# olga24912/lodestar

Measured on AMD Instinct MI355X. Metric: verified signature sets/sec (node), higher is better.
Workload: dtype u32/u64 (28-bit-limb Montgomery integer arithmetic); 1 GPU; C2 gossip attestation flood: 16384 single-pubkey sets per GPU, 1 set per batchable job; pk_mode=device table, sig_encoding=compressed 96 B, distinct_messages=16384, group_sets=1024, group_policy=0, inflight=32, slots=3, hw_queues=4, merge_sets=131072, pipeline_depth=3, parallelism=shard-by-job x1 (in-process devices), no collective

## Files before the change

lodestar_amd/build.py:

```python
import hashlib
import os
import subprocess
import sys
import time

PKG = os.path.dirname(os.path.abspath(__file__))
ROOT = os.path.dirname(PKG)
CSRC = os.path.join(PKG, "csrc")
LIB = os.environ.get("BLSGPU_LIB") or os.path.join(PKG, "libblsgpu.so")
ARCH = os.environ.get("BLSGPU_ARCH", "gfx950")
HIPCC = os.environ.get("HIPCC", "/opt/rocm/bin/hipcc")
SOURCES = ["k_sig.hip", "k_msm.hip", "k_hash.hip", "k_hmap.hip", "k_pk.hip", "k_sigagg.hip", "k_awr.hip", "k_same.hip", "k_miller.hip", "k_group.hip", "k_inv.hip", "k_ssz.hip", "k_debug.hip",
           "runtime.cpp", "helpers.cpp"]


OBJ_DIR = os.path.join(PKG, "build")


TU_DEFINES = {"k_sig.hip": ["BLS_INLINE_BIG=1"]}


def tu_defines():
    env = os.environ.get("BLSGPU_TU_DEFINES")
    if env is None:
        return TU_DEFINES
    out = {}
    for part in filter(None, env.split(";")):
        tu, _, defs = part.partition("=")
        out[tu] = [d for d in defs.split("+") if d]
    return out


_ILP = ["-mllvm", "-amdgpu-sched-strategy=max-ilp"]
_MINREG = ["-mllvm", "-amdgpu-sched-strategy=iterative-minreg"]
TU_CFLAGS = {"k_hash.hip": _MINREG, "k_pk.hip": _ILP}


def tu_cflags():
    env = os.environ.get("BLSGPU_TU_CFLAGS")
    if env is None:
        return TU_CFLAGS
    out = {}
    for part in filter(None, env.split(";")):
        tu, _, flags = part.partition("=")
        out[tu] = flags.split()
    return out


def _headers():
    out = [os.path.join(ROOT, "include", "blsgpu.h")]
    for f in os.listdir(CSRC):
        if f.endswith((".hpp", ".h")):
            out.append(os.path.join(CSRC, f))
    return out


def _tu_deps(src):
    if src.endswith(".cpp"):
        return [os.path.join(CSRC, f) for f in (src, "kernels.h", "batch_rand.hpp", "runtime_internal.hpp",
                                                "helper_layout.hpp")] + [os.path.join(ROOT, "include", "blsgpu.h")]
    return [os.path.join(CSRC, src)] + _headers()


def _deps():
    return _headers() + [os.path.join(CSRC, s) for s in SOURCES] + [os.path.abspath(__file__)]


def up_to_date():
    if not os.path.exists(LIB):
        return False
    t = os.path.getmtime(LIB)
    return all(os.path.getmtime(d) <= t for d in _deps())


def build(force=False, verbose=True):
    if not force and up_to_date():
        build_node_addon(verbose=verbose)
        return LIB
    objs = []
    common = ["-O3", "-std=c++17", "-fPIC", f"--offload-arch={ARCH}", "-I", os.path.join(ROOT, "include")]
    defines = os.environ.get("BLSGPU_DEFINES", "").split()
    common += ["-D" + d for d in defines]
    cflags = os.environ.get("BLSGPU_CFLAGS", "").split()
    common += cflags
    tu_defs = tu_defines()
    os.makedirs(OBJ_DIR, exist_ok=True)
    key = os.path.splitext(os.path.basename(LIB))[0] + ("." + "_".join(defines).replace("=", "-") if defines else "")
    if cflags:
        key += ".cf" + hashlib.md5(" ".join(cflags).encode()).hexdigest()[:8]
    procs = []
    t0 = time.time()
    for src in SOURCES:
        tdefs = tu_defs.get(src, [])
        tflags = tu_cflags().get(src, [])
        obj = os.path.join(OBJ_DIR, key + "." + os.path.splitext(src)[0] +
                           ("." + "_".join(tdefs).replace("=", "-") if tdefs else "") +
                           (".cf" + hashlib.md5(" ".join(tflags).encode()).hexdigest()[:8] if tflags else "") + ".o")
        objs.append(obj)
        if not force and os.path.exists(obj) and all(os.path.getmtime(d) <= os.path.getmtime(obj) for d in _tu_deps(src)):
            continue
        cmd = [HIPCC] + common + ["-D" + d for d in tdefs] + tflags + ["-c", os.path.join(CSRC, src), "-o", obj]
        if verbose:
            print(" ".join(cmd), flush=True)
        procs.append((src, subprocess.Popen(cmd)))
    for src, p in procs:
        if p.wait() != 0:
            raise RuntimeError(f"hipcc failed on {src}")
        if verbose:
            print(f"  {src}: done at {time.time() - t0:.0f} s", flush=True)
    cmd = [HIPCC, f"--offload-arch={ARCH}", "-shared", "-o", LIB] + objs + ["-lpthread"]
    if verbose:
        print(" ".join(cmd), flush=True)
    subprocess.check_call(cmd)
    build_node_addon(verbose=verbose)
    return LIB


NODE_DIR = os.path.join(PKG, "node")
ADDON = os.path.join(NODE_DIR, "blsgpu_napi.node")
NODE_INC = "/usr/include/node"


def build_node_addon(force=False, verbose=True):
    src = os.path.join(NODE_DIR, "blsgpu_napi.c")
    if not os.path.exists(os.path.join(NODE_INC, "node_api.h")):
        if verbose:
            print("node headers not found: N-API addon not built", flush=True)
        return None
    if not force and os.path.exists(ADDON) and os.path.getmtime(ADDON) >= max(
            os.path.getmtime(src), os.path.getmtime(LIB), os.path.getmtime(os.path.join(ROOT, "include", "blsgpu.h"))):
        return ADDON
    cmd = ["gcc", "-O2", "-std=c11", "-Wall", "-Wno-unused-parameter", "-shared", "-fPIC",
           "-DNODE_GYP_MODULE_NAME=blsgpu_napi", "-I", NODE_INC, "-I", os.path.join(ROOT, "include"), src,
           "-o", ADDON, "-L", PKG, "-l:libblsgpu.so", "-Wl,-rpath,$ORIGIN/.."]
    if verbose:
        print(" ".join(cmd), flush=True)
    subprocess.check_call(cmd)
    return ADDON


if __name__ == "__main__":
    build(force="--force" in sys.argv)
```

lodestar_amd/csrc/k_group.hip:

```cpp
#include "k_common.hpp"
#include "gt_wave.hpp"
#include "gt6.hpp"

__global__ __launch_bounds__(WAVE) void k_job_mask(PipelineBuffers b) {
  uint32_t j = blockIdx.x * WAVE + threadIdx.x;
  if (j >= b.n_jobs) return;
  const uint32_t a = b.job_first_set[j], e = b.job_first_set[j + 1];
  const int8_t* pk_st = b.status + b.n;
  int err = 0;
  for (uint32_t i = a; i < e && !err; i++) err = pk_st[i];
  for (uint32_t i = a; i < e && !err; i++) err = b.status[i];
  if (a == e) err = BLS_EMPTY_SET;
  b.job_err[j] = (int8_t)err;
  for (uint32_t i = a; i < e; i++) b.include[i] = err == 0 ? 1 : 0;
}

__global__ __launch_bounds__(WAVE) void k_group_reduce(PipelineBuffers b, const uint32_t* f_ranges, uint32_t ng,
                                                       uint32_t* F_out) {
  __shared__ uint32_t red[WAVE * W_FP12];
  const uint32_t g = blockIdx.x, lane = threadIdx.x;
  if (g >= ng) return;
  const uint32_t first = f_ranges[2 * g], last = f_ranges[2 * g + 1];
  fp12 F = fp12_one();
  bool any = false;
  for (uint32_t i = first + lane; i < last; i += WAVE) {
    F = any ? fp12_mul(F, ld_fp12(b.f_chunk, b.n, i)) : ld_fp12(b.f_chunk, b.n, i);
    any = true;
  }
#pragma unroll 1
  for (int s = WAVE / 2; s >= 1; s >>= 1) {
    if (lane >= (uint32_t)s && lane < (uint32_t)(2 * s)) st_fp12(red, WAVE, lane - s, F);
    __syncthreads();
    if (lane < (uint32_t)s) F = fp12_mul(F, ld_fp12(red, WAVE, lane));
    __syncthreads();
  }
  if (lane == 0) st_fp12(F_out, ng, g, F);
}

STAGE_KERNEL_W(BLSGPU_WPE_GRP) void k_f_runs(PipelineBuffers b, const uint32_t* runs, uint32_t n_runs) {
  const uint32_t q = blockIdx.x * WAVE + threadIdx.x;
  if (q >= n_runs) return;
  const uint32_t a = runs[2 * q], e = runs[2 * q + 1];
  fp12 F = ld_fp12(b.f_chunk, b.n, a);
#pragma unroll 1
  for (uint32_t i = a + 1; i < e; i++) F = fp12_mul(F, ld_fp12(b.f_chunk, b.n, i));
  st_fp12(b.f_chunk, b.n, a, F);
}

__global__ __launch_bounds__(GTW_LANES) void k_f_pairs(PipelineBuffers b, const uint32_t* pairs) {
  __shared__ uint32_t A[GTW_FP12], B[GTW_FP12], S[108 * BLS_NL];
  const uint32_t t = threadIdx.x, i = pairs[2 * blockIdx.x], j = pairs[2 * blockIdx.x + 1];
  for (uint32_t w = t; w < W_FP12; w += GTW_LANES) {
    A[gtw_lds_word(w)] = b.f_chunk[(size_t)w * b.n + i];
    B[gtw_lds_word(w)] = b.f_chunk[(size_t)w * b.n + j];
  }
  gtw_sync();
  gtw_mul<false>(A, A, B, S, t);
  for (uint32_t w = t; w < W_FP12; w += GTW_LANES) b.f_chunk[(size_t)w * b.n + i] = A[gtw_lds_word(w)];
}

STAGE_KERNEL void k_f_gather(PipelineBuffers b, const uint32_t* f_ranges, uint32_t ng, uint32_t* F_out) {
  const uint32_t q = blockIdx.x * WAVE + threadIdx.x;
  if (q >= ng * W_FP12) return;
  const uint32_t g = q % ng, w = q / ng, a = f_ranges[2 * g], e = f_ranges[2 * g + 1];
  F_out[q] = a < e ? b.f_chunk[(size_t)w * b.n + a] : (w < BLS_NL ? FP_ONE.l[w] : 0u);
}

__device__ __forceinline__ void gtw_load_S(GtwLds& sh, const uint32_t* S_in, uint32_t ng, uint32_t g, uint32_t t) {
  if (t == 0) {
    g2a Sa;
    const bool fin = jac_to_aff(ld_g2j(S_in, ng, g), Sa);
    if (fin) {
      lds_st(sh.QA, 0, Sa.x.c0);
      lds_st(sh.QA, 1, Sa.x.c1);
      lds_st(sh.QA, 2, Sa.y.c0);
      lds_st(sh.QA, 3, Sa.y.c1);
    }
    sh.flag = fin ? 1u : 0u;
  }
}

__global__ __launch_bounds__(GTW_MILLER_LANES) void k_group_sig_miller(const uint32_t* S_in, uint32_t ng, uint32_t* G_out) {
  __shared__ GtwLds sh;
  const uint32_t g = blockIdx.x, t = threadIdx.x;
  gtw_load_S(sh, S_in, ng, g, t);
  gtw_sync();
  if (sh.flag)
    gtw_miller_loop(sh.G, sh.QA, G1_GEN_X, G1_NEG_GEN_Y, sh.TB, sh.L, sh.L1, sh.S, sh.S2, t);
  else
    gtw_set_one(sh.G, t);
  gtw_sync();
  for (uint32_t w = t; w < W_FP12; w += GTW_MILLER_LANES) G_out[(size_t)w * ng + g] = sh.G[gtw_lds_word(w)];
}

STAGE_KERNEL_W(BLSGPU_WPE_GRP) void k_group_sig_miller_lane(const uint32_t* S_in, uint32_t ng, uint32_t* G_out) {
  const uint32_t g = blockIdx.x * WAVE + threadIdx.x;
  if (g >= ng) return;
  g2a Sa;
  g1a P;
  P.x = G1_GEN_X;
  P.y = G1_NEG_GEN_Y;
  const fp12 G = jac_to_aff(ld_g2j(S_in, ng, g), Sa) ? miller_loop(P, Sa) : fp12_one();
  st_fp12(G_out, ng, g, G);
}

STAGE_KERNEL_W(BLSGPU_WPE_LINES) void k_check_lines(const uint32_t* S_in, uint32_t ng, const uint32_t* sel, uint32_t n,
                                                   uint32_t* lines, uint8_t* flags) {
  const uint32_t q = blockIdx.x * WAVE + threadIdx.x;
  if (q >= n) return;
  const uint32_t g = sel ? sel[q] : q;
  g2a Sa;
  const bool fin = jac_to_aff(ld_g2j(S_in, ng, g), Sa);
  flags[g] = fin ? 0 : 1;
  if (fin) miller_lines_store(Sa, lines, ng, g);
}

STAGE_KERNEL_W(BLSGPU_WPE_GRP) void k_group_sig_miller_lane_sel(const uint32_t* S_in, uint32_t ng, const uint32_t* sel,
                                                               uint32_t n, uint32_t* G_out) {
  const uint32_t q = blockIdx.x * WAVE + threadIdx.x;
  if (q >= n) return;
  const uint32_t g = sel ? sel[q] : q;
  g2a Sa;
  g1a P;
  P.x = G1_GEN_X;
  P.y = G1_NEG_GEN_Y;
  const fp12 G = jac_to_aff(ld_g2j(S_in, ng, g), Sa) ? miller_loop(P, Sa) : fp12_one();
  st_fp12(G_out, ng, g, G);
}

template <bool MILLER>
__global__ __launch_bounds__(MILLER ? GTW_MILLER_LANES : GTW_LANES) void k_group_check(
    const uint32_t* S_in, const uint32_t* F_in, uint32_t ng, const uint32_t* G_in, const uint32_t* sel, uint8_t* ok) {
  constexpr uint32_t NT = MILLER ? GTW_MILLER_LANES : GTW_LANES;
  __shared__ GtwLds sh;
  const uint32_t t = threadIdx.x;
  const uint32_t g = sel ? sel[blockIdx.x] : blockIdx.x;
  for (uint32_t w = t; w < W_FP12; w += NT) {
    sh.F[gtw_lds_word(w)] = F_in[(size_t)w * ng + g];
    if (!MILLER) sh.G[gtw_lds_word(w)] = G_in[(size_t)w * ng + g];
  }
  if (MILLER) gtw_load_S(sh, S_in, ng, g, t);
  gtw_sync();
  if (!MILLER) {
    gtw_mul<false>(sh.F, sh.F, sh.G, sh.S, t);
  } else if (sh.flag) {
    gtw_miller_loop(sh.G, sh.QA, G1_GEN_X, G1_NEG_GEN_Y, sh.TB, sh.L, sh.L1, sh.S, sh.S2, t);
    gtw_mul<false>(sh.F, sh.F, sh.G, sh.S, t);
  }
  gtw_final_exp(sh.F, sh.W, sh.S, t);
  if (t == 0) ok[blockIdx.x] = fp12_is_one(gtw_to_reg(sh.F)) ? 1 : 0;
}

STAGE_KERNEL_W(BLSGPU_WPE_GRP) void k_group_check_lane(const uint32_t* S_in, const uint32_t* F_in, uint32_t ng,
                                                      const uint32_t* sel, uint32_t n, uint8_t* ok) {
  const uint32_t q = blockIdx.x * WAVE + threadIdx.x;
  if (q >= n) return;
  const uint32_t g = sel ? sel[q] : q;
  fp12 F = ld_fp12(F_in, ng, g);
  g2a Sa;
  if (jac_to_aff(ld_g2j(S_in, ng, g), Sa)) {
    g1a P;
    P.x = G1_GEN_X;
    P.y = G1_NEG_GEN_Y;
    F = fp12_mul(F, miller_loop(P, Sa));
  }
  ok[q] = fp12_is_one(final_exponentiation(F)) ? 1 : 0;
}

template <bool MILLER>
STAGE_KERNEL_W(BLSGPU_WPE_GRP) void k_group_check6(const uint32_t* F_in, const uint32_t* G_in, uint32_t ng,
                                                  const uint32_t* sel, uint32_t n, uint8_t* ok, const uint32_t* lines,
                                                  const uint8_t* flags) {
  const uint32_t lane = threadIdx.x, grp = lane / 6, k = lane % 6;
  const uint32_t q = blockIdx.x * ACC6_GROUPS + grp;
  if (grp >= ACC6_GROUPS || q >= n) return;
  const uint32_t gi = sel ? sel[q] : q;
  const G6 g{(int)(grp * 6), k};
  const int w0 = ((k & 1) ? 3 : 0) * 2 * W_FP + (int)(k >> 1) * 2 * W_FP;
  const fp2 F = ld_fp2(F_in, ng, gi, w0);
  fp2 G;
  if (MILLER)
    G = flags[gi] ? (k == 0 ? fp2_one() : fp2_zero()) : g6_miller(lines, ng, gi, G1_GEN_X, G1_NEG_GEN_Y, g);
  else
    G = ld_fp2(G_in, ng, gi, w0);
  const bool one = g6_is_one(g6_final_exp(g6_mul(F, G, g), g), g);
  if (k == 0) ok[q] = one ? 1 : 0;
}

__global__ __launch_bounds__(WAVE) void k_range_combine(const uint32_t* S_in, const uint32_t* F_in, uint32_t n_in,
                                                        const uint32_t* ranges, uint32_t n_out, uint32_t* S_out,
                                                        uint32_t* F_out) {
  __shared__ uint32_t red[WAVE * (W_G2J + W_FP12)];
  const uint32_t r = blockIdx.x, lane = threadIdx.x;
  if (r >= n_out) return;
  const uint32_t first = ranges[2 * r], last = ranges[2 * r + 1];
  g2j S = jac_infinity<fp2>();
  fp12 F = fp12_one();
  for (uint32_t e = first + lane; e < last; e += WAVE) {
    S = jac_add(S, ld_g2j(S_in, n_in, e));
    F = fp12_mul(F, ld_fp12(F_in, n_in, e));
  }
#pragma unroll 1
  for (int h = WAVE / 2; h >= 1; h >>= 1) {
    if (lane >= (uint32_t)h && lane < (uint32_t)(2 * h)) {
      st_g2j(red, WAVE, lane - h, S);
      st_fp12(red + WAVE * W_G2J, WAVE, lane - h, F);
    }
    __syncthreads();
    if (lane < (uint32_t)h) {
      S = jac_add(S, ld_g2j(red, WAVE, lane));
      F = fp12_mul(F, ld_fp12(red + WAVE * W_G2J, WAVE, lane));
    }
    __syncthreads();
  }
  if (lane == 0) {
    st_g2j(S_out, n_out, r, S);
    st_fp12(F_out, n_out, r, F);
  }
}


STAGE_KERNEL_W(BLSGPU_WPE_GRP) void k_group_reduce_lane(PipelineBuffers b, const uint32_t* set_ranges, const uint32_t* f_ranges,
                                      uint32_t ng, uint32_t* S_out, uint32_t* F_out) {
  const uint32_t g = blockIdx.x * WAVE + threadIdx.x;
  if (g >= ng) return;
  g2j S = jac_infinity<fp2>();
  for (uint32_t i = set_ranges[2 * g]; i < set_ranges[2 * g + 1]; i++)
    if (b.include[i]) S = jac_add(S, ld_g2j(b.rsig, b.n, i));
  fp12 F = fp12_one();
  for (uint32_t c = f_ranges[2 * g]; c < f_ranges[2 * g + 1]; c++) F = fp12_mul(F, ld_fp12(b.f_chunk, b.n, c));
  st_g2j(S_out, ng, g, S);
  st_fp12(F_out, ng, g, F);
}

STAGE_KERNEL_W(BLSGPU_WPE_GRP) void k_range_combine_lane(const uint32_t* S_in, const uint32_t* F_in, uint32_t n_in, const uint32_t* ranges,
                                       uint32_t n_out, uint32_t* S_out, uint32_t* F_out) {
  const uint32_t r = blockIdx.x * WAVE + threadIdx.x;
  if (r >= n_out) return;
  g2j S = jac_infinity<fp2>();
  fp12 F = fp12_one();
  for (uint32_t e = ranges[2 * r]; e < ranges[2 * r + 1]; e++) {
    S = jac_add(S, ld_g2j(S_in, n_in, e));
    F = fp12_mul(F, ld_fp12(F_in, n_in, e));
  }
  st_g2j(S_out, n_out, r, S);
  st_fp12(F_out, n_out, r, F);
}

static inline dim3 grid_for(uint32_t n) { return dim3((n + WAVE - 1) / WAVE); }

__global__ __launch_bounds__(256) void k_copy_words(uint32_t* __restrict__ dst, const uint32_t* __restrict__ src,
                                                    size_t n) {
  for (size_t i = (size_t)blockIdx.x * 256 + threadIdx.x; i < n; i += (size_t)gridDim.x * 256) dst[i] = src[i];
}
void launch_copy_words(uint32_t* dst, const uint32_t* src, size_t n, hipStream_t s) {
  if (n) hipLaunchKernelGGL(k_copy_words, dim3((unsigned)std::min<size_t>((n + 255) / 256, 8192)), dim3(256), 0, s, dst, src, n);
}

void launch_group_reduce_lane(const PipelineBuffers& b, const uint32_t* set_ranges, const uint32_t* f_ranges,
                              uint32_t ng, uint32_t* S, uint32_t* F, hipStream_t s) {
  if (ng) hipLaunchKernelGGL(k_group_reduce_lane, grid_for(ng), dim3(WAVE), 0, s, b, set_ranges, f_ranges, ng, S, F);
}
void launch_range_combine_lane(const uint32_t* S_in, const uint32_t* F_in, uint32_t n_in, const uint32_t* ranges,
                               uint32_t n_out, uint32_t* S_out, uint32_t* F_out, hipStream_t s) {
  if (n_out)
    hipLaunchKernelGGL(k_range_combine_lane, grid_for(n_out), dim3(WAVE), 0, s, S_in, F_in, n_in, ranges, n_out, S_out,
                       F_out);
}

void launch_job_mask(const PipelineBuffers& b, hipStream_t s) {
  if (b.n_jobs) hipLaunchKernelGGL(k_job_mask, grid_for(b.n_jobs), dim3(WAVE), 0, s, b);
}
void launch_group_reduce(const PipelineBuffers& b, const uint32_t* f_ranges, uint32_t ng, uint32_t* F, hipStream_t s) {
  if (ng) hipLaunchKernelGGL(k_group_reduce, dim3(ng), dim3(WAVE), 0, s, b, f_ranges, ng, F);
}
void launch_group_tree(const PipelineBuffers& b, const uint32_t* f_ranges, uint32_t ng, const uint32_t* runs,
                       uint32_t n_runs, const uint32_t* pairs, const std::vector<uint32_t>& level_end, uint32_t* F,
                       hipStream_t s) {
  if (!ng) return;
  if (n_runs) hipLaunchKernelGGL(k_f_runs, grid_for(n_runs), dim3(WAVE), 0, s, b, runs, n_runs);
  uint32_t p0 = 0;
  for (const uint32_t p1 : level_end) {
    if (p1 > p0) hipLaunchKernelGGL(k_f_pairs, dim3(p1 - p0), dim3(GTW_LANES), 0, s, b, pairs + 2 * (size_t)p0);
    p0 = p1;
  }
  hipLaunchKernelGGL(k_f_gather, grid_for(ng * W_FP12), dim3(WAVE), 0, s, b, f_ranges, ng, F);
}
void launch_group_sig_miller_sel(const uint32_t* S, uint32_t ng, const uint32_t* sel, uint32_t n_sel, uint32_t* G,
                                 hipStream_t s) {
  const uint32_t n = sel ? n_sel : ng;
  if (n) hipLaunchKernelGGL(k_group_sig_miller_lane_sel, grid_for(n), dim3(WAVE), 0, s, S, ng, sel, n, G);
}
void launch_group_check6(const uint32_t* F, const uint32_t* G, uint32_t ng, uint8_t* ok, hipStream_t s,
                         const uint32_t* sel, uint32_t n_sel) {
  const uint32_t n = sel ? n_sel : ng;
  if (n)
    hipLaunchKernelGGL(k_group_check6<false>, dim3((n + ACC6_GROUPS - 1) / ACC6_GROUPS), dim3(WAVE), 0, s, F, G, ng,
                       sel, n, ok, nullptr, nullptr);
}
void launch_check6_miller(const uint32_t* S, const uint32_t* F, uint32_t ng, uint8_t* ok, hipStream_t s,
                          const uint32_t* sel, uint32_t n_sel, uint32_t* lines, uint8_t* flags) {
  const uint32_t n = sel ? n_sel : ng;
  if (!n) return;
  hipLaunchKernelGGL(k_check_lines, grid_for(n), dim3(WAVE), 0, s, S, ng, sel, n, lines, flags);
  hipLaunchKernelGGL(k_group_check6<true>, dim3((n + ACC6_GROUPS - 1) / ACC6_GROUPS), dim3(WAVE), 0, s, F, nullptr, ng,
                     sel, n, ok, lines, flags);
}
void launch_group_check(const uint32_t* S, const uint32_t* F, uint32_t ng, uint8_t* ok, hipStream_t s,
                        const uint32_t* sel, uint32_t n_sel, const uint32_t* G, bool exclusive, bool lane) {
  const uint32_t n = sel ? n_sel : ng;
  if (!n) return;
  if (lane && !G)
    hipLaunchKernelGGL(k_group_check_lane, grid_for(n), dim3(WAVE), 0, s, S, F, ng, sel, n, ok);
  else if (G)
    hipLaunchKernelGGL(k_group_check<false>, dim3(n), dim3(GTW_LANES),
                       exclusive ? exclusive_cu_lds<k_group_check<false>>() : 0, s, S, F, ng, G, sel, ok);
  else
    hipLaunchKernelGGL(k_group_check<true>, dim3(n), dim3(GTW_MILLER_LANES),
                       exclusive ? exclusive_cu_lds<k_group_check<true>>() : 0, s, S, F, ng, G, sel, ok);
}
void launch_group_sig_miller(const uint32_t* S, uint32_t ng, uint32_t* G, hipStream_t s, bool exclusive, bool lane) {
  if (ng && lane)
    hipLaunchKernelGGL(k_group_sig_miller_lane, grid_for(ng), dim3(WAVE), 0, s, S, ng, G);
  else if (ng)
    hipLaunchKernelGGL(k_group_sig_miller, dim3(ng), dim3(GTW_MILLER_LANES),
                       exclusive ? exclusive_cu_lds<k_group_sig_miller>() : 0,
                       s, S, ng, G);
}
void launch_range_combine(const uint32_t* S_in, const uint32_t* F_in, uint32_t n_in, const uint32_t* ranges,
                          uint32_t n_out, uint32_t* S_out, uint32_t* F_out, hipStream_t s) {
  if (n_out)
    hipLaunchKernelGGL(k_range_combine, dim3(n_out), dim3(WAVE), 0, s, S_in, F_in, n_in, ranges, n_out, S_out, F_out);
}
```

lodestar_amd/csrc/k_miller.hip:

```cpp
#include "k_common.hpp"
#include "gt_wave.hpp"
#include "gt6.hpp"
#include "gtx.hpp"

#ifndef BLS_LINE_PAIRS
#define BLS_LINE_PAIRS 0
#endif
#ifndef BLS_ACC2_PAIRS
#define BLS_ACC2_PAIRS 0
#endif

BLS_INL fp fp_add_n(const fp& a, const fp& b) { return fp_add_norm(a, b); }

#ifndef BLS_ACC_PREFETCH
#define BLS_ACC_PREFETCH 0
#endif
#if BLS_ACC_PREFETCH && defined(__HIP_DEVICE_COMPILE__)
#define LDS_AS __attribute__((address_space(3)))
__device__ __forceinline__ void line_prefetch(uint32_t* pre, const uint32_t* o, uint32_t nm, uint32_t m) {
  const uint32_t* a = o + opaque_u32(m);
#pragma unroll 1
  for (int w = 0; w < W_LINE; w++) {
    __builtin_amdgcn_global_load_lds((const void*)a, (LDS_AS void*)(pre + w * WAVE), 4, 0, 0);
    a += nm;
  }
}
__device__ __forceinline__ void line_wait() {
  asm volatile("" ::: "memory");
  __builtin_amdgcn_s_waitcnt(0x0F70);
  asm volatile("" ::: "memory");
}
__device__ __forceinline__ void line_read_done() {
  asm volatile("" ::: "memory");
  __builtin_amdgcn_s_waitcnt(0xC07F);
  asm volatile("" ::: "memory");
}
__device__ __forceinline__ fp ld_fp_pre(const uint32_t* pre, int w0) {
  fp r;
#pragma unroll
  for (int l = 0; l < BLS_NL; l++) r.l[l] = pre[(w0 + l) * WAVE + threadIdx.x];
  return r;
}
__device__ __forceinline__ fp2 ld_fp2_pre(const uint32_t* pre, int w0) {
  return fp2_make(ld_fp_pre(pre, w0), ld_fp_pre(pre, w0 + W_FP));
}
#define ACC_PREFETCH 1
#else
#define ACC_PREFETCH 0
#endif

STAGE_KERNEL_W(BLSGPU_WPE_LINES) void k_miller_lines(PipelineBuffers b) {
  uint32_t u = blockIdx.x * WAVE + threadIdx.x;
  if (u >= b.n_umsg || (b.mflags[u] & MF_H_INF)) return;
  miller_lines_store(ld_g2a(b.h_aff, b.nm, u), b.lines, b.nm, u);
}

#ifndef BLSGPU_WPE_LINES2
#define BLSGPU_WPE_LINES2 2
#endif
STAGE_KERNEL_W(BLSGPU_WPE_LINES2) void k_miller_lines2(PipelineBuffers b) {
  const uint32_t q = blockIdx.x * WAVE + threadIdx.x;
  const uint32_t u = q >> 1, k = q & 1;
  if (u >= b.n_umsg || (b.mflags[u] & MF_H_INF)) return;
  auto ldQ = [&] {
    const uint32_t uu = opaque_u32(u);
    aff<fp2x> Q;
    Q.x.v = ld_fp(b.h_aff, b.nm, uu, (int)(k * W_FP));
    Q.y.v = ld_fp(b.h_aff, b.nm, uu, (int)((2 + k) * W_FP));
    return Q;
  };
  g2projx Tp;
  {
    const aff<fp2x> Q = ldQ();
    Tp.x = Q.x;
    Tp.y = Q.y;
    Tp.z = F_one((const fp2x*)0);
  }
  int bit = 62;
  bool add_next = false;
#pragma unroll 1
  for (int s = 0; s < MILLER_STEPS; s++) {
    line3x Ln;
    if (!add_next) {
      miller_dbl_line(Tp, Ln);
      add_next = (BLS_Z_ABS >> bit) & 1ull;
      bit--;
    } else {
      miller_add_line(Tp, ldQ(), Ln);
      add_next = false;
    }
    uint32_t* o = b.lines + (size_t)s * W_LINE * b.nm;
    st_fp(o, b.nm, u, (int)(k * W_FP), Ln.l0.v);
    st_fp(o, b.nm, u, (int)((2 + k) * W_FP), Ln.c1.v);
    st_fp(o, b.nm, u, (int)((4 + k) * W_FP), Ln.c4.v);
  }
}

template <bool UNITS>
STAGE_KERNEL_W(BLSGPU_WPE_ACC) void k_miller_acc(PipelineBuffers b) {
  const uint32_t c = blockIdx.x * WAVE + threadIdx.x;
  if (c >= b.n_chunks) return;
  const uint32_t k0 = b.chunk_first[c], k1 = b.chunk_first[c + 1];
#if ACC_PREFETCH
  __shared__ uint32_t pre[W_LINE * WAVE];
  auto msg_of = [&](uint32_t k) {
    const uint32_t i = b.chunk_items[k];
    return UNITS ? b.unit_msg[i] : b.msg_idx[i];
  };
  if (k1 > k0) line_prefetch(pre, b.lines, b.nm, msg_of(k0));
#endif
  fp12 f = fp12_one();
  int bit = 62;
  bool add_next = false;
#pragma unroll 1
  for (int s = 0; s < MILLER_STEPS; s++) {
    if (!add_next && s != 0) f = fp12_sqr(f);
    const uint32_t* o = b.lines + (size_t)s * W_LINE * b.nm;
#if BLS_LINE_PAIRS
    bool pend = false;
    fp2 q0, q1, q4;
#endif
#pragma unroll 1
    for (uint32_t k = k0; k < k1; k++) {
      const uint32_t i = b.chunk_items[k];
      uint32_t m;
      bool active;
      if (UNITS) {
        m = b.unit_msg[i];
        active = b.unit_ok[i] != 0;
      } else {
        m = b.msg_idx[i];
        active = b.include[i] != 0;
      }
#if ACC_PREFETCH
      line_wait();
      line3 L;
      L.l0 = ld_fp2_pre(pre, 0);
      L.c1 = ld_fp2_pre(pre, 2 * W_FP);
      L.c4 = ld_fp2_pre(pre, 4 * W_FP);
      line_read_done();
      if (k + 1 < k1)
        line_prefetch(pre, o, b.nm, msg_of(k + 1));
      else if (s + 1 < MILLER_STEPS)
        line_prefetch(pre, o + (size_t)W_LINE * b.nm, b.nm, msg_of(k0));
      if (!active || (b.mflags[m] & MF_H_INF)) continue;
      const g1a P = ld_g1a(UNITS ? b.unit_p : b.pk_aff, b.n, i);
#else
      if (!active || (b.mflags[m] & MF_H_INF)) continue;
      const g1a P = ld_g1a(UNITS ? b.unit_p : b.pk_aff, b.n, i);
      line3 L;
      L.l0 = ld_fp2(o, b.nm, m, 0);
      L.c1 = ld_fp2(o, b.nm, m, 2 * W_FP);
      L.c4 = ld_fp2(o, b.nm, m, 4 * W_FP);
#endif
#if BLS_LINE_PAIRS
      const fp2 l1 = fp2_mul_fp(L.c1, P.x), l4 = fp2_mul_fp(L.c4, P.y);
      if (pend) {
        f = fp12_mul_by_line2(f, line_pair(q0, q1, q4, L.l0, l1, l4));
        pend = false;
      } else {
        q0 = L.l0;
        q1 = l1;
        q4 = l4;
        pend = true;
      }
#else
      f = fp12_mul_by_014(f, L.l0, fp2_mul_fp(L.c1, P.x), fp2_mul_fp(L.c4, P.y));
#endif
    }
#if BLS_LINE_PAIRS
    if (pend) f = fp12_mul_by_014(f, q0, q1, q4);
#endif
    if (!add_next) {
      add_next = (BLS_Z_ABS >> bit) & 1ull;
      bit--;
    } else {
      add_next = false;
    }
  }
  st_fp12(b.f_chunk, b.n, c, fp12_conj(f));
}

template <bool UNITS>
STAGE_KERNEL_W(BLSGPU_WPE_ACC) void k_miller_acc2(PipelineBuffers b) {
  const uint32_t q = blockIdx.x * WAVE + threadIdx.x;
  const uint32_t c = q >> 1, h = q & 1;
  if (c >= b.n_chunks) return;
  const uint32_t k0 = b.chunk_first[c], k1 = b.chunk_first[c + 1];
#if ACC_PREFETCH
  __shared__ uint32_t pre[W_LINE * WAVE];
  auto msg_of = [&](uint32_t k) {
    const uint32_t i = b.chunk_items[k];
    return UNITS ? b.unit_msg[i] : b.msg_idx[i];
  };
  if (k1 > k0) line_prefetch(pre, b.lines, b.nm, msg_of(k0));
#endif
  fp6 mine = h ? fp6_zero() : fp6_one();
  int bit = 62;
  bool add_next = false;
#pragma unroll 1
  for (int s = 0; s < MILLER_STEPS; s++) {
    if (!add_next && s != 0) {
      const fp6 other = fp6_xlane(mine);
      const fp6 a0 = h ? other : mine, a1 = h ? mine : other;
      fp6 X, Y;
      if (h) {
        X.c0 = fp2_make(fp_add_n(a0.c0.c0, a1.c0.c0), fp_add_n(a0.c0.c1, a1.c0.c1));
        X.c1 = fp2_make(fp_add_n(a0.c1.c0, a1.c1.c0), fp_add_n(a0.c1.c1, a1.c1.c1));
        X.c2 = fp2_make(fp_add_n(a0.c2.c0, a1.c2.c0), fp_add_n(a0.c2.c1, a1.c2.c1));
        Y.c0 = fp2_make(fp_lc(T<1>(a0.c0.c0), T<1>(a1.c2.c0), T<-1>(a1.c2.c1)),
                        fp_lc(T<1>(a0.c0.c1), T<1>(a1.c2.c0), T<1>(a1.c2.c1)));
        Y.c1 = fp2_make(fp_add_n(a0.c1.c0, a1.c0.c0), fp_add_n(a0.c1.c1, a1.c0.c1));
        Y.c2 = fp2_make(fp_add_n(a0.c2.c0, a1.c1.c0), fp_add_n(a0.c2.c1, a1.c1.c1));
      } else {
        X = a0;
        Y = a1;
      }
      const fp6 pr = fp6_mul(X, Y);
      const fp6 t = fp6_xlane(pr);
      fp6 r;
      if (h) {
        r.c0.c0 = fp_lc(T<1>(pr.c0.c0), T<-1>(t.c0.c0), T<-1>(t.c2.c0), T<1>(t.c2.c1));
        r.c0.c1 = fp_lc(T<1>(pr.c0.c1), T<-1>(t.c0.c1), T<-1>(t.c2.c0), T<-1>(t.c2.c1));
        r.c1.c0 = fp_lc(T<1>(pr.c1.c0), T<-1>(t.c1.c0), T<-1>(t.c0.c0));
        r.c1.c1 = fp_lc(T<1>(pr.c1.c1), T<-1>(t.c1.c1), T<-1>(t.c0.c1));
        r.c2.c0 = fp_lc(T<1>(pr.c2.c0), T<-1>(t.c2.c0), T<-1>(t.c1.c0));
        r.c2.c1 = fp_lc(T<1>(pr.c2.c1), T<-1>(t.c2.c1), T<-1>(t.c1.c1));
      } else {
        r.c0 = fp2_make(fp_lc(T<2>(pr.c0.c0)), fp_lc(T<2>(pr.c0.c1)));
        r.c1 = fp2_make(fp_lc(T<2>(pr.c1.c0)), fp_lc(T<2>(pr.c1.c1)));
        r.c2 = fp2_make(fp_lc(T<2>(pr.c2.c0)), fp_lc(T<2>(pr.c2.c1)));
      }
      mine = fp6_xlane(r);
    }
    const uint32_t* o = b.lines + (size_t)s * W_LINE * b.nm;
    auto fold = [&](const fp6& T0, const fp6& T1) {
      const fp6 T1v = h ? T1 : fp6_mul_v(T1);
      fp6 r;
      r.c0 = fp2_make(fp_lc(T<1>(T0.c0.c0), T<1>(T1v.c0.c0)), fp_lc(T<1>(T0.c0.c1), T<1>(T1v.c0.c1)));
      r.c1 = fp2_make(fp_lc(T<1>(T0.c1.c0), T<1>(T1v.c1.c0)), fp_lc(T<1>(T0.c1.c1), T<1>(T1v.c1.c1)));
      r.c2 = fp2_make(fp_lc(T<1>(T0.c2.c0), T<1>(T1v.c2.c0)), fp_lc(T<1>(T0.c2.c1), T<1>(T1v.c2.c1)));
      mine = r;
    };
#if BLS_ACC2_PAIRS
    bool pend = false;
    fp2 q0, q1, q4;
#endif
#pragma unroll 1
    for (uint32_t k = k0; k < k1; k++) {
      const uint32_t i = b.chunk_items[k];
      uint32_t m;
      bool active;
      if (UNITS) {
        m = b.unit_msg[i];
        active = b.unit_ok[i] != 0;
      } else {
        m = b.msg_idx[i];
        active = b.include[i] != 0;
      }
#if ACC_PREFETCH
      line_wait();
      fp2 l0 = ld_fp2_pre(pre, 0), l1 = ld_fp2_pre(pre, 2 * W_FP), l4 = ld_fp2_pre(pre, 4 * W_FP);
      line_read_done();
      if (k + 1 < k1)
        line_prefetch(pre, o, b.nm, msg_of(k + 1));
      else if (s + 1 < MILLER_STEPS)
        line_prefetch(pre, o + (size_t)W_LINE * b.nm, b.nm, msg_of(k0));
      if (!active || (b.mflags[m] & MF_H_INF)) continue;
      const g1a P = ld_g1a(UNITS ? b.unit_p : b.pk_aff, b.n, i);
      l1 = fp2_mul_fp(l1, P.x);
      l4 = fp2_mul_fp(l4, P.y);
#else
      if (!active || (b.mflags[m] & MF_H_INF)) continue;
      const g1a P = ld_g1a(UNITS ? b.unit_p : b.pk_aff, b.n, i);
      const fp2 l0 = ld_fp2(o, b.nm, m, 0);
      const fp2 l1 = fp2_mul_fp(ld_fp2(o, b.nm, m, 2 * W_FP), P.x);
      const fp2 l4 = fp2_mul_fp(ld_fp2(o, b.nm, m, 4 * W_FP), P.y);
#endif
#if BLS_ACC2_PAIRS
      if (!pend) {
        q0 = l0;
        q1 = l1;
        q4 = l4;
        pend = true;
        continue;
      }
      pend = false;
      const fp2 R1 = fp2_mul(h ? q4 : q0, h ? l4 : l0);
      const fp2 R2 = fp2_mul(h ? fp2_add_nr(q0, q4) : q1, h ? fp2_add_nr(l0, l4) : l1);
      const fp2 R3 = fp2_mul(h ? fp2_add_nr(q1, q4) : fp2_add_nr(q0, q1), h ? fp2_add_nr(l1, l4) : fp2_add_nr(l0, l1));
      const fp2 O1 = fp2_xlane(R1), O2 = fp2_xlane(R2), O3 = fp2_xlane(R3);
      const fp2 P00 = h ? O1 : R1, P44 = h ? R1 : O1, P11 = h ? O2 : R2, X04 = h ? R2 : O2, X01 = h ? O3 : R3,
                X14 = h ? R3 : O3;
      fp6 M0;
      M0.c0 = fp2_make(fp_lc(T<1>(P00.c0), T<1>(P44.c0), T<-1>(P44.c1)), fp_lc(T<1>(P00.c1), T<1>(P44.c0), T<1>(P44.c1)));
      M0.c1 = F2_LC3(X01, P00, P11);
      M0.c2 = P11;
      const fp2 m11 = F2_LC3(X04, P00, P44), m12 = F2_LC3(X14, P11, P44);
      const fp6 other = fp6_xlane(mine);
      fold(fp6_mul(mine, M0), fp6_mul_by_12(other, m11, m12));
#else
      const fp6 other = fp6_xlane(mine);
      fold(fp6_mul_by_01(mine, l0, l1), fp6_mul_by_1(other, l4));
#endif
    }
#if BLS_ACC2_PAIRS
    if (pend) {
      const fp6 other = fp6_xlane(mine);
      fold(fp6_mul_by_01(mine, q0, q1), fp6_mul_by_1(other, q4));
    }
#endif
    if (!add_next) {
      add_next = (BLS_Z_ABS >> bit) & 1ull;
      bit--;
    } else {
      add_next = false;
    }
  }
  const fp6 out = h ? fp6_neg(mine) : mine;
  st_fp2(b.f_chunk, b.n, c, 6 * (int)h * W_FP, out.c0);
  st_fp2(b.f_chunk, b.n, c, (6 * (int)h + 2) * W_FP, out.c1);
  st_fp2(b.f_chunk, b.n, c, (6 * (int)h + 4) * W_FP, out.c2);
}

#ifndef BLSGPU_WPE_ACCX
#define BLSGPU_WPE_ACCX 2
#endif
template <bool UNITS>
STAGE_KERNEL_W(BLSGPU_WPE_ACCX) void k_miller_accx(PipelineBuffers b) {
  const uint32_t q = blockIdx.x * WAVE + threadIdx.x;
  const uint32_t c = q >> 1, k = q & 1;
  if (c >= b.n_chunks) return;
  const uint32_t k0 = b.chunk_first[c], k1 = b.chunk_first[c + 1];
  fp12x f;
  f.c0.c0 = F_one((const fp2x*)0);
  f.c0.c1 = f.c0.c2 = f.c1.c0 = f.c1.c1 = f.c1.c2 = F_zero((const fp2x*)0);
  int bit = 62;
  bool add_next = false;
#pragma unroll 1
  for (int s = 0; s < MILLER_STEPS; s++) {
    if (!add_next && s != 0) f = fp12x_sqr(f);
    const uint32_t* o = b.lines + (size_t)s * W_LINE * b.nm;
#pragma unroll 1
    for (uint32_t it = k0; it < k1; it++) {
      const uint32_t i = b.chunk_items[it];
      uint32_t m;
      bool active;
      if (UNITS) {
        m = b.unit_msg[i];
        active = b.unit_ok[i] != 0;
      } else {
        m = b.msg_idx[i];
        active = b.include[i] != 0;
      }
      if (!active || (b.mflags[m] & MF_H_INF)) continue;
      const g1a P = ld_g1a(UNITS ? b.unit_p : b.pk_aff, b.n, i);
      const fp2x l0{ld_fp(o, b.nm, m, (int)(k * W_FP))};
      const fp2x l1{fp_mul(ld_fp(o, b.nm, m, (int)((2 + k) * W_FP)), P.x)};
      const fp2x l4{fp_mul(ld_fp(o, b.nm, m, (int)((4 + k) * W_FP)), P.y)};
      f = fp12x_mul_by_014(f, l0, l1, l4);
    }
    if (!add_next) {
      add_next = (BLS_Z_ABS >> bit) & 1ull;
      bit--;
    } else {
      add_next = false;
    }
  }
  st_fp(b.f_chunk, b.n, c, (int)((0 + k) * W_FP), f.c0.c0.v);
  st_fp(b.f_chunk, b.n, c, (int)((2 + k) * W_FP), f.c0.c1.v);
  st_fp(b.f_chunk, b.n, c, (int)((4 + k) * W_FP), f.c0.c2.v);
  st_fp(b.f_chunk, b.n, c, (int)((6 + k) * W_FP), fp_neg(f.c1.c0.v));
  st_fp(b.f_chunk, b.n, c, (int)((8 + k) * W_FP), fp_neg(f.c1.c1.v));
  st_fp(b.f_chunk, b.n, c, (int)((10 + k) * W_FP), fp_neg(f.c1.c2.v));
}

template <bool UNITS, int WPE>
__global__ __launch_bounds__(WAVE) __attribute__((amdgpu_waves_per_eu(WPE, WPE))) void k_miller_acc6(PipelineBuffers b) {
  const uint32_t lane = threadIdx.x, grp = lane / 6, k = lane % 6;
  const uint32_t c = blockIdx.x * ACC6_GROUPS + grp;
  if (grp >= ACC6_GROUPS || c >= b.n_chunks) return;
  const int base = (int)(grp * 6);
  const uint32_t k0 = b.chunk_first[c], k1 = b.chunk_first[c + 1];
  fp2 f = k == 0 ? fp2_one() : fp2_zero();
  int bit = 62;
  bool add_next = false;
#pragma unroll 1
  for (int s = 0; s < MILLER_STEPS; s++) {
    if (!add_next && s != 0) {
      f = g6_sqr(f, G6{base, k});
    }
    const uint32_t* o = b.lines + (size_t)s * W_LINE * b.nm;
#pragma unroll 1
    for (uint32_t it = k0; it < k1; it++) {
      const uint32_t i = b.chunk_items[it];
      uint32_t m;
      bool active;
      if (UNITS) {
        m = b.unit_msg[i];
        active = b.unit_ok[i] != 0;
      } else {
        m = b.msg_idx[i];
        active = b.include[i] != 0;
      }
      if (!active || (b.mflags[m] & MF_H_INF)) continue;
      const g1a Pa = ld_g1a(UNITS ? b.unit_p : b.pk_aff, b.n, i);
      f = g6_line_mul(f, o, b.nm, m, Pa.x, Pa.y, G6{base, k});
    }
    if (!add_next) {
      add_next = (BLS_Z_ABS >> bit) & 1ull;
      bit--;
    } else {
      add_next = false;
    }
  }
  const int slot = (k & 1 ? 3 : 0) + (int)(k >> 1);
  st_fp2(b.f_chunk, b.n, c, slot * 2 * W_FP, (k & 1) ? fp2_neg(f) : f);
}

template <bool UNITS>
__global__ __launch_bounds__(GTW_MILLER_LANES) void k_miller_coop(PipelineBuffers b) {
  __shared__ GtwLds sh;
  const uint32_t c = blockIdx.x, t = threadIdx.x;
  if (c >= b.n_chunks) return;
  const uint32_t i = b.chunk_items[b.chunk_first[c]];
  uint32_t m;
  bool active;
  if (UNITS) {
    m = b.unit_msg[i];
    active = b.unit_ok[i] != 0;
  } else {
    m = b.msg_idx[i];
    active = b.include[i] != 0;
  }
  active = active && !(b.mflags[m] & MF_H_INF);
  if (active) {
    if (t < 4) lds_st(sh.QA, (int)t, ld_fp(b.h_aff, b.nm, m, (int)t * W_FP));
    const g1a P = ld_g1a(UNITS ? b.unit_p : b.pk_aff, b.n, i);
    gtw_sync();
    gtw_miller_loop(sh.G, sh.QA, P.x, P.y, sh.TB, sh.L, sh.L1, sh.S, sh.S2, t);
  } else {
    gtw_set_one(sh.G, t);
  }
  gtw_sync();
  for (uint32_t w = t; w < W_FP12; w += GTW_MILLER_LANES) b.f_chunk[(size_t)w * b.n + c] = sh.G[gtw_lds_word(w)];
}

static inline dim3 grid_for(uint32_t n) { return dim3((n + WAVE - 1) / WAVE); }

void launch_miller_coop(const PipelineBuffers& b, bool units, hipStream_t s, bool exclusive) {
  if (!b.n_chunks) return;
  if (units)
    hipLaunchKernelGGL(k_miller_coop<true>, dim3(b.n_chunks), dim3(GTW_MILLER_LANES),
                       exclusive ? exclusive_cu_lds<k_miller_coop<true>>() : 0, s, b);
  else
    hipLaunchKernelGGL(k_miller_coop<false>, dim3(b.n_chunks), dim3(GTW_MILLER_LANES),
                       exclusive ? exclusive_cu_lds<k_miller_coop<false>>() : 0, s, b);
}

void launch_miller_lines(const PipelineBuffers& b, hipStream_t s) {
  if (b.n_umsg) hipLaunchKernelGGL(k_miller_lines, grid_for(b.n_umsg), dim3(WAVE), 0, s, b);
}
void launch_miller_lines2(const PipelineBuffers& b, hipStream_t s) {
  if (b.n_umsg) hipLaunchKernelGGL(k_miller_lines2, grid_for(2 * b.n_umsg), dim3(WAVE), 0, s, b);
}
void launch_miller_acc2(const PipelineBuffers& b, bool units, hipStream_t s) {
  if (!b.n_chunks) return;
  if (units)
    hipLaunchKernelGGL(k_miller_acc2<true>, grid_for(2 * b.n_chunks), dim3(WAVE), 0, s, b);
  else
    hipLaunchKernelGGL(k_miller_acc2<false>, grid_for(2 * b.n_chunks), dim3(WAVE), 0, s, b);
}
#define ACC6_W1_MAX_CHUNKS (1024 * ACC6_GROUPS)
void launch_miller_acc6(const PipelineBuffers& b, bool units, hipStream_t s) {
  if (!b.n_chunks) return;
  const dim3 grid((b.n_chunks + ACC6_GROUPS - 1) / ACC6_GROUPS);
  const bool w2 = b.n_chunks > ACC6_W1_MAX_CHUNKS;
  if (units && w2)
    hipLaunchKernelGGL((k_miller_acc6<true, 2>), grid, dim3(WAVE), 0, s, b);
  else if (units)
    hipLaunchKernelGGL((k_miller_acc6<true, 1>), grid, dim3(WAVE), 0, s, b);
  else if (w2)
    hipLaunchKernelGGL((k_miller_acc6<false, 2>), grid, dim3(WAVE), 0, s, b);
  else
    hipLaunchKernelGGL((k_miller_acc6<false, 1>), grid, dim3(WAVE), 0, s, b);
}
void launch_miller_accx(const PipelineBuffers& b, bool units, hipStream_t s) {
  if (!b.n_chunks) return;
  if (units)
    hipLaunchKernelGGL(k_miller_accx<true>, grid_for(2 * b.n_chunks), dim3(WAVE), 0, s, b);
  else
    hipLaunchKernelGGL(k_miller_accx<false>, grid_for(2 * b.n_chunks), dim3(WAVE), 0, s, b);
}
void launch_miller_acc(const PipelineBuffers& b, bool units, hipStream_t s) {
  if (!b.n_chunks) return;
  if (units)
    hipLaunchKernelGGL(k_miller_acc<true>, grid_for(b.n_chunks), dim3(WAVE), 0, s, b);
  else
    hipLaunchKernelGGL(k_miller_acc<false>, grid_for(b.n_chunks), dim3(WAVE), 0, s, b);
}
```

lodestar_amd/csrc/kernels.h:

```cpp
#pragma once
#include <hip/hip_runtime.h>
#include <stdint.h>
#include <vector>

#define W_FP 14
#define W_G1A (2 * W_FP)
#define W_G1J (3 * W_FP)
#define W_G2A (4 * W_FP)
#define W_G2J (6 * W_FP)
#define W_FP12 (12 * W_FP)
#define W_PKTAB 32
#define MILLER_STEPS 68
#define W_LINE (3 * 2 * W_FP)

#define SF_SIG_INF 1u
#define MF_H_INF 1u

struct PipelineBuffers {
  uint32_t n;
  const uint8_t* sigs;
  const uint32_t* sig_len;
  uint32_t sig_stride;
  const uint8_t* pk_bytes;
  const uint32_t* set_pk_first;
  const uint32_t* pk_index;
  const uint32_t* pk_table;
  uint32_t pk_table_n;
  const uint32_t* agg_sets;
  uint32_t n_agg;
  uint32_t pk_direct1;
  const uint64_t* scalars;
  uint32_t* scal_tab;
  const uint32_t* job_first_set;
  uint32_t n_jobs;
  const uint8_t* umsgs;
  const uint32_t* msg_idx;
  uint32_t n_umsg;
  uint32_t nm;
  uint32_t n_units;
  const uint32_t* unit_set_first;
  const uint32_t* unit_sets;
  const uint32_t* unit_msg;
  uint32_t* sig_aff;
  uint32_t* h_aff;
  uint32_t* h_jac;
  uint32_t* h_norm;
  uint32_t* h_prep;
  uint32_t* h_q;
  uint32_t* inv_buf;
  uint32_t* inv_buf_pk;
  uint32_t* pk_jac;
  uint32_t* pk_aff;
  uint32_t* rsig;
  uint32_t* unit_p;
  uint32_t n_chunks;
  const uint32_t* chunk_first;
  const uint32_t* chunk_items;
  uint32_t* f_chunk;
  uint32_t* lines;
  uint8_t* flags;
  uint8_t* mflags;
  uint8_t* unit_ok;
  int8_t* status;
  int8_t* job_err;
  uint8_t* include;
};

void launch_sig_decode(const PipelineBuffers& b, uint32_t n_sets, hipStream_t s, bool coop = false,
                       hipEvent_t decoded = nullptr, bool exclusive = true, bool subgroup = true);
void launch_spec_mask(const PipelineBuffers& b, uint32_t n_sets, uint8_t* spec, hipStream_t s);
void launch_hash_prep(const PipelineBuffers& b, hipStream_t s);
void launch_hash_map(const PipelineBuffers& b, const uint32_t* inv, hipStream_t s);
void launch_hash_to_g2(const PipelineBuffers& b, hipStream_t s, bool coop = false,
                       bool exclusive = true);
void launch_pk_aggregate(const PipelineBuffers& b, uint32_t n_sets, hipStream_t s);
void launch_pk_finish(const PipelineBuffers& b, uint32_t n_sets, hipStream_t s);
void launch_batch_inv(const uint32_t* src, uint32_t src_stride, int w0, uint32_t* dst, uint32_t n, hipStream_t s);
void launch_pk_affine(const PipelineBuffers& b, uint32_t n_sets, hipStream_t s);
void launch_h_affine(const PipelineBuffers& b, hipStream_t s);
void launch_sig_scale(const PipelineBuffers& b, uint32_t n_sets, hipStream_t s, const uint32_t* list = nullptr);
#ifndef MSM_SLICE
#define MSM_SLICE 256
#endif
#define MSM_BUCKET_WORDS (128 * W_G2J)
#define MSM_WINDOW_WORDS (16 * W_G2J)
void launch_sig_msm(const PipelineBuffers& b, const uint32_t* slices, uint32_t n_slices, const uint32_t* range_slices,
                    uint32_t n_ranges, uint32_t* B, uint32_t* W, uint32_t* S, hipStream_t s, bool lane_tail = false,
                    uint32_t tree_slices = 0);
void launch_job_mask(const PipelineBuffers& b, hipStream_t s);
void launch_unit_aggregate(const PipelineBuffers& b, hipStream_t s);
void launch_miller_lines(const PipelineBuffers& b, hipStream_t s);
void launch_miller_lines2(const PipelineBuffers& b, hipStream_t s);
void launch_miller_accx(const PipelineBuffers& b, bool units, hipStream_t s);
void launch_miller_acc(const PipelineBuffers& b, bool units, hipStream_t s);
void launch_miller_acc2(const PipelineBuffers& b, bool units, hipStream_t s);
void launch_miller_acc6(const PipelineBuffers& b, bool units, hipStream_t s);
#ifndef BLSGPU_EXCLUSIVE_SMALL
#define BLSGPU_EXCLUSIVE_SMALL 1
#endif
void launch_miller_coop(const PipelineBuffers& b, bool units, hipStream_t s, bool exclusive = false);
void launch_group_reduce(const PipelineBuffers& b, const uint32_t* f_ranges, uint32_t n_groups, uint32_t* F,
                         hipStream_t s);
void launch_group_tree(const PipelineBuffers& b, const uint32_t* f_ranges, uint32_t n_groups, const uint32_t* runs,
                       uint32_t n_runs, const uint32_t* pairs, const std::vector<uint32_t>& level_end, uint32_t* F,
                       hipStream_t s);
void launch_group_check(const uint32_t* S, const uint32_t* F, uint32_t n_groups, uint8_t* ok, hipStream_t s,
                        const uint32_t* sel = nullptr, uint32_t n_sel = 0, const uint32_t* G = nullptr,
                        bool exclusive = false, bool lane = false);
void launch_group_check6(const uint32_t* F, const uint32_t* G, uint32_t n_groups, uint8_t* ok, hipStream_t s,
                         const uint32_t* sel = nullptr, uint32_t n_sel = 0);
void launch_check6_miller(const uint32_t* S, const uint32_t* F, uint32_t n_groups, uint8_t* ok, hipStream_t s,
                          const uint32_t* sel, uint32_t n_sel, uint32_t* lines, uint8_t* flags);
void launch_group_sig_miller_sel(const uint32_t* S, uint32_t n_groups, const uint32_t* sel, uint32_t n_sel, uint32_t* G,
                                 hipStream_t s);
void launch_group_sig_miller(const uint32_t* S, uint32_t n_groups, uint32_t* G, hipStream_t s, bool exclusive = false,
                             bool lane = false);
void launch_copy_words(uint32_t* dst, const uint32_t* src, size_t n, hipStream_t s);
void launch_group_reduce_lane(const PipelineBuffers& b, const uint32_t* set_ranges, const uint32_t* f_ranges,
                              uint32_t n_groups, uint32_t* S, uint32_t* F, hipStream_t s);
void launch_range_combine_lane(const uint32_t* S_in, const uint32_t* F_in, uint32_t n_in, const uint32_t* ranges,
                               uint32_t n_out, uint32_t* S_out, uint32_t* F_out, hipStream_t s);
void launch_range_combine(const uint32_t* S_in, const uint32_t* F_in, uint32_t n_in, const uint32_t* ranges,
                          uint32_t n_out, uint32_t* S_out, uint32_t* F_out, hipStream_t s);
void launch_pk_table_fill(const uint8_t* pk96, uint32_t n, uint32_t* table_dst, int8_t* status, hipStream_t s);
void launch_pk_serialize(const PipelineBuffers& b, uint32_t n_sets, uint8_t* out, uint32_t out_len, hipStream_t s);
void launch_key_validate(const uint8_t* pks, uint32_t n, uint32_t pk_len, uint32_t stride, uint8_t* out96,
                         int8_t* status, hipStream_t s);
inline uint32_t sig_agg_lanes(uint32_t n_groups, uint32_t n_sigs) {
  if (n_groups == 0) return 1;
  const uint64_t n = n_groups, lanes = 1024 * 64;
  const uint32_t by_count = n * 64 <= lanes ? 64 : n * 32 <= 2 * lanes ? 32 : n * 16 <= 2 * lanes ? 16
                            : n * 8 <= 2 * lanes ? 8 : 1;
  const uint64_t mean = ((uint64_t)n_sigs + n - 1) / n;
  const uint32_t by_size = mean <= 3 ? 1 : mean <= 8 ? 8 : mean <= 16 ? 16 : mean <= 32 ? 32 : 64;
  return by_count < by_size ? by_count : by_size;
}
void launch_sig_aggregate(const PipelineBuffers& b, const uint32_t* group_first, uint32_t n_groups, uint32_t n_sigs,
                          uint32_t* agg, int8_t* agg_status, uint32_t* first_bad, hipStream_t s);
void launch_sig_agg_serialize(const uint32_t* group_first, uint32_t n_groups, const uint32_t* agg, int8_t* agg_status,
                              uint8_t* out, uint32_t out_len, hipStream_t s);
struct AwrBuffers {
  uint32_t n;
  uint32_t n_groups;
  const uint32_t* group_first;
  const uint64_t* words;
  const uint8_t* pk_bytes;
  const uint32_t* pk_index;
  const uint32_t* pk_table;
  uint32_t pk_table_n;
  const uint32_t* sig_aff;
  const uint8_t* sig_flags;
  const int8_t* sig_status;
  uint32_t* tab;
  uint32_t tab_n;
  uint32_t* sum_pk;
  uint32_t* sum_sig;
  uint32_t* err_k;
  int8_t* err_c;
};
#define AWR_TAB_WORDS (9 * W_G2J)
inline uint32_t awr_lanes(uint32_t n_groups, uint32_t n_sets) {
  if (n_groups == 0) return 1;
  const uint64_t n = n_groups, lanes = 1024 * 64;
  const uint32_t by_count = n * 64 <= lanes ? 64 : n * 32 <= lanes ? 32 : n * 16 <= lanes ? 16 : n * 8 <= lanes ? 8 : 1;
  const uint64_t mean = ((uint64_t)n_sets + n - 1) / n;
  const uint32_t by_size = mean <= 1 ? 1 : mean <= 8 ? 8 : mean <= 16 ? 16 : mean <= 32 ? 32 : 64;
  return by_count < by_size ? by_count : by_size;
}
uint32_t awr_launch_lanes(uint32_t n_groups, uint32_t L);
void launch_awr_sums(const AwrBuffers& a, uint32_t L, hipStream_t s);
void launch_awr_sum_pk(const AwrBuffers& a, uint32_t L, hipStream_t s);
void launch_awr_sum_sig(const AwrBuffers& a, uint32_t L, hipStream_t s);
void launch_same_group_items(const AwrBuffers& a, const uint32_t* inv, uint32_t* pk_aff, uint8_t* include, int8_t* code,
                             hipStream_t s);
void launch_same_retry_items(const AwrBuffers& a, const uint32_t* list, uint32_t n_retry, uint32_t* pk_aff, uint32_t* S,
                             uint8_t* include, int8_t* code, hipStream_t s);
void launch_same_group_results(const uint32_t* group_first, uint32_t n_groups, uint32_t n_sets, const uint8_t* include,
                               const int8_t* code, const uint8_t* ok, int8_t* set_result, int8_t* group_result,
                               hipStream_t s);
void launch_same_retry_results(const uint32_t* list, uint32_t n_retry, const uint8_t* include, const int8_t* code,
                               const uint8_t* ok, int8_t* set_result, hipStream_t s);
void launch_awr_serialize(const AwrBuffers& a, uint8_t* out_pk, uint32_t out_pk_len, uint8_t* out_sig,
                          uint32_t out_sig_len, int8_t* status, uint32_t* first_bad, hipStream_t s);
void launch_signing_roots(int kind, const uint8_t* in, uint32_t n, uint32_t in_stride, const uint8_t* domain,
                          uint32_t domain_stride, uint8_t* out, hipStream_t s);
void launch_debug_op(int op, uint32_t n, const uint8_t* in, uint32_t in_stride, uint8_t* out, uint32_t out_stride,
                     int32_t* status, hipStream_t s);
```

lodestar_amd/csrc/pairing.hpp:

```cpp
#pragma once
#include "curve.hpp"

struct g2proj {
  fp2 x, y, z;
};

BLS_FN void miller_dbl_step(g2proj& T, const fp& xP, const fp& yP, fp2& l0, fp2& l1, fp2& l4) {
  fp2 A = fp2_half(fp2_mul(T.x, T.y));
  fp2 B = fp2_sqr(T.y);
  fp2 C = fp2_sqr(T.z);
  fp2 E = fp2_mul3(fp2_mul_xi(C));
  E = fp2_dbl(fp2_dbl(E));
  fp2 F = fp2_mul3(E);
  fp2 G = fp2_half(fp2_add(B, F));
  fp2 H = fp2_sub(fp2_sub(fp2_sqr(fp2_add(T.y, T.z)), B), C);
  fp2 J = fp2_sqr(T.x);
  fp2 E2 = fp2_sqr(E);
  T.x = fp2_mul(A, fp2_sub(B, F));
  T.y = fp2_sub(fp2_sqr(G), fp2_mul3(E2));
  T.z = fp2_mul(B, H);
  l0 = fp2_sub(E, B);
  l1 = fp2_mul_fp(fp2_mul3(J), xP);
  l4 = fp2_mul_fp(fp2_neg(H), yP);
}

BLS_FN void miller_add_step(g2proj& T, const g2a& Q, const fp& xP, const fp& yP, fp2& l0, fp2& l1, fp2& l4) {
  fp2 theta = fp2_sub(T.y, fp2_mul(Q.y, T.z));
  fp2 lam = fp2_sub(T.x, fp2_mul(Q.x, T.z));
  fp2 C = fp2_sqr(theta);
  fp2 D = fp2_sqr(lam);
  fp2 E = fp2_mul(lam, D);
  fp2 F = fp2_mul(T.z, C);
  fp2 G = fp2_mul(T.x, D);
  fp2 H = fp2_sub(fp2_add(E, F), fp2_dbl(G));
  fp2 X3 = fp2_mul(lam, H);
  fp2 Y3 = fp2_sub(fp2_mul(theta, fp2_sub(G, H)), fp2_mul(T.y, E));
  fp2 Z3 = fp2_mul(T.z, E);
  l0 = fp2_sub(fp2_mul(theta, Q.x), fp2_mul(lam, Q.y));
  l1 = fp2_mul_fp(fp2_neg(theta), xP);
  l4 = fp2_mul_fp(lam, yP);
  T.x = X3;
  T.y = Y3;
  T.z = Z3;
}

#define MILLER_STEPS 68
struct line3 {
  fp2 l0, c1, c4;
};
BLS_HD bool miller_step_is_add(int s) {
  int bit = 62;
  bool add_next = false;
  for (int k = 0; k < s; k++) {
    if (!add_next) {
      add_next = (BLS_Z_ABS >> bit) & 1ull;
      bit--;
    } else {
      add_next = false;
    }
  }
  return add_next;
}
#if BLS_LAZY_CURVE
BLS_FN void miller_dbl_line(g2proj& R, line3& Ln) {
  const fp2 A = fp2_half(fp2_mul(R.x, R.y));
  const fp2 B = fp2_sqr(R.y);
  const fp2 C = fp2_sqr(R.z);
  const fp2 xC = fp2_make(fp_lc(T<1>(C.c0), T<-1>(C.c1)), fp_lc(T<1>(C.c0), T<1>(C.c1)));
  const fp2 E = F_lc(L<12>(xC));
  const fp2 G = fp2_half(F_lc(L<1>(B), L<3>(E)));
  const fp2 H = F_lc(L<1>(fp2_sqr(fp2_add_norm(R.y, R.z))), L<-1>(B), L<-1>(C));
  const fp2 J = fp2_sqr(R.x);
  const fp2 E2 = fp2_sqr(E);
  R.x = fp2_mul(A, F_lc(L<1>(B), L<-3>(E)));
  R.y = F_lc(L<1>(fp2_sqr(G)), L<-3>(E2));
  R.z = fp2_mul(B, H);
  Ln.l0 = F_lc(L<1>(E), L<-1>(B));
  Ln.c1 = F_lc(L<3>(J));
  Ln.c4 = F_lc(L<-1>(H));
}
BLS_FN void miller_add_line(g2proj& R, const g2a& Q, line3& Ln) {
  const fp2 theta = F_lc(L<1>(R.y), L<-1>(fp2_mul(Q.y, R.z)));
  const fp2 lam = F_lc(L<1>(R.x), L<-1>(fp2_mul(Q.x, R.z)));
  const fp2 C = fp2_sqr(theta);
  const fp2 D = fp2_sqr(lam);
  const fp2 E = fp2_mul(lam, D);
  const fp2 F = fp2_mul(R.z, C);
  const fp2 G = fp2_mul(R.x, D);
  const fp2 H = F_lc(L<1>(E), L<1>(F), L<-2>(G));
  const fp2 X3 = fp2_mul(lam, H);
  const fp2 Y3 = F_lc(L<1>(fp2_mul(theta, F_lc(L<1>(G), L<-1>(H)))), L<-1>(fp2_mul(R.y, E)));
  const fp2 Z3 = fp2_mul(R.z, E);
  Ln.l0 = F_lc(L<1>(fp2_mul(theta, Q.x)), L<-1>(fp2_mul(lam, Q.y)));
  Ln.c1 = F_lc(L<-1>(theta));
  Ln.c4 = lam;
  R.x = X3;
  R.y = Y3;
  R.z = Z3;
}
#else
BLS_FN void miller_dbl_line(g2proj& T, line3& L) {
  fp2 A = fp2_half(fp2_mul(T.x, T.y));
  fp2 B = fp2_sqr(T.y);
  fp2 C = fp2_sqr(T.z);
  fp2 E = fp2_mul3(fp2_mul_xi(C));
  E = fp2_dbl(fp2_dbl(E));
  fp2 F = fp2_mul3(E);
  fp2 G = fp2_half(fp2_add(B, F));
  fp2 H = fp2_sub(fp2_sub(fp2_sqr(fp2_add(T.y, T.z)), B), C);
  fp2 J = fp2_sqr(T.x);
  fp2 E2 = fp2_sqr(E);
  T.x = fp2_mul(A, fp2_sub(B, F));
  T.y = fp2_sub(fp2_sqr(G), fp2_mul3(E2));
  T.z = fp2_mul(B, H);
  L.l0 = fp2_sub(E, B);
  L.c1 = fp2_mul3(J);
  L.c4 = fp2_neg(H);
}
BLS_FN void miller_add_line(g2proj& T, const g2a& Q, line3& L) {
  fp2 theta = fp2_sub(T.y, fp2_mul(Q.y, T.z));
  fp2 lam = fp2_sub(T.x, fp2_mul(Q.x, T.z));
  fp2 C = fp2_sqr(theta);
  fp2 D = fp2_sqr(lam);
  fp2 E = fp2_mul(lam, D);
  fp2 F = fp2_mul(T.z, C);
  fp2 G = fp2_mul(T.x, D);
  fp2 H = fp2_sub(fp2_add(E, F), fp2_dbl(G));
  fp2 X3 = fp2_mul(lam, H);
  fp2 Y3 = fp2_sub(fp2_mul(theta, fp2_sub(G, H)), fp2_mul(T.y, E));
  fp2 Z3 = fp2_mul(T.z, E);
  L.l0 = fp2_sub(fp2_mul(theta, Q.x), fp2_mul(lam, Q.y));
  L.c1 = fp2_neg(theta);
  L.c4 = lam;
  T.x = X3;
  T.y = Y3;
  T.z = Z3;
}
#endif
BLS_FN fp12 miller_acc_step(const fp12& f, int s, bool is_add, const line3& L, const fp& xP, const fp& yP) {
  fp12 g = (!is_add && s != 0) ? fp12_sqr(f) : f;
  return fp12_mul_by_014(g, L.l0, fp2_mul_fp(L.c1, xP), fp2_mul_fp(L.c4, yP));
}

BLS_HDNI fp12 miller_loop(const g1a& P, const g2a& Q) {
  g2proj T;
  T.x = Q.x;
  T.y = Q.y;
  T.z = fp2_one();
  fp12 f = fp12_one();
  int bit = 62;
  bool add_next = false;
#pragma unroll 1
  for (int s = 0; s < 68; s++) {
    fp2 l0, l1, l4;
    if (!add_next) {
      if (s != 0) f = fp12_sqr(f);
      miller_dbl_step(T, P.x, P.y, l0, l1, l4);
      add_next = (BLS_Z_ABS >> bit) & 1ull;
      bit--;
    } else {
      miller_add_step(T, Q, P.x, P.y, l0, l1, l4);
      add_next = false;
    }
    f = fp12_mul_by_014(f, l0, l1, l4);
  }
  return fp12_conj(f);
}

BLS_HDNI fp12 fp12_pow_zabs(const fp12& f) {
  fp12 r = f;
  for (int i = 62; i >= 0; i--) {
    r = fp12_cyclotomic_sqr(r);
    if ((BLS_Z_ABS >> i) & 1ull) r = fp12_mul(r, f);
  }
  return r;
}
BLS_HD fp12 fp12_pow_z(const fp12& f) { return fp12_conj(fp12_pow_zabs(f)); }

BLS_BIG fp12 fp12_mul_c(const fp12& a, const fp12& b) { return fp12_mul(a, b); }

BLS_HDNI fp12 final_exponentiation(const fp12& f) {
  fp12 f1 = fp12_mul_c(fp12_conj(f), fp12_inv(f));
  fp12 m = fp12_mul_c(fp12_frob2(f1), f1);
  fp12 t = fp12_mul_c(fp12_pow_z(m), fp12_conj(m));
  t = fp12_mul_c(fp12_pow_z(t), fp12_conj(t));
  t = fp12_mul_c(fp12_pow_z(t), fp12_frob1(t));
  t = fp12_mul_c(fp12_mul_c(fp12_pow_z(fp12_pow_z(t)), fp12_frob2(t)), fp12_conj(t));
  return fp12_mul_c(t, fp12_mul_c(fp12_sqr(m), m));
}
```

lodestar_amd/csrc/runtime.cpp:

```cpp
#include <pthread.h>
#include <stdio.h>
#include <sys/random.h>

#include <cmath>
#include <string>
#include <system_error>

#include "runtime_internal.hpp"

using namespace blsgpu_rt;

namespace {

std::atomic<int64_t> g_fail_run_skip{0}, g_fail_run_count{0};
thread_local bool tl_dispatcher = false;

inline uint32_t chunk_size(uint32_t len, uint32_t min_per_chunk) {
  const uint32_t count = min_per_chunk ? len / min_per_chunk : 0;
  return count <= 1 ? len : (len + count - 1) / count;
}

struct GroupPlanEntry {
  uint32_t first, end;
  bool batchable;
};

inline uint32_t miller_k_auto(uint32_t n_items) {
  uint32_t k = 1;
  while (k < 4 && n_items / (2 * k) >= 65536) k *= 2;
  return k;
}

void launch_miller_acc_auto(const PipelineBuffers& pb, bool units, hipStream_t st, uint32_t mk, int64_t lanes_opt,
                            int64_t acc6_max, bool pairs) {
  if (lanes_opt == 6 || (lanes_opt == 0 && mk == 1 && (int64_t)pb.n_chunks <= acc6_max)) {
    launch_miller_acc6(pb, units, st);
    return;
  }
  if (lanes_opt == 3 || (lanes_opt == 0 && pairs)) {
    launch_miller_accx(pb, units, st);
    return;
  }
  const bool two = lanes_opt == 2 || (lanes_opt == 0 && mk == 1);
  if (two)
    launch_miller_acc2(pb, units, st);
  else
    launch_miller_acc(pb, units, st);
}

inline std::pair<uint32_t, uint32_t> add_chunks(std::vector<uint32_t>& first, std::vector<uint32_t>& items,
                                                uint32_t a, uint32_t e, uint32_t k, const uint32_t* map = nullptr) {
  const uint32_t c0 = (uint32_t)first.size() - 1;
  for (uint32_t x = a; x < e; x += k) {
    for (uint32_t y = x; y < std::min(e, x + k); y++) items.push_back(map ? map[y] : y);
    first.push_back((uint32_t)items.size());
  }
  return {c0, (uint32_t)first.size() - 1};
}

inline void add_slices(std::vector<uint32_t>& slices, std::vector<uint32_t>& range_slices, uint32_t a, uint32_t e,
                       uint32_t len = MSM_SLICE) {
  for (uint32_t x = a; x < e; x += len) {
    slices.push_back(x);
    slices.push_back(std::min<uint32_t>(e, x + len));
  }
  range_slices.push_back((uint32_t)(slices.size() / 2));
}

}

namespace blsgpu_rt __attribute__((visibility("hidden"))) {

struct Shard {
  uint32_t job_begin, job_end;
  uint32_t set_begin, set_end;
  uint32_t dev = 0;
  int64_t cost = 0;
};

struct Owned {
  std::vector<uint32_t> jfs, siglen, pkfirst, pkidx;
  std::vector<uint8_t> jflags, pkb, msgs, sigs;
};

struct Call {
  blsgpu_ctx* ctx = nullptr;
  blsgpu_batch b{};
  Owned* owned = nullptr;
  int8_t* job_result = nullptr;
  blsgpu_stats* stats = nullptr;
  uint64_t seed = 0;
  batch_rand::Key key{};
  uint32_t max_index = 0;
  Options opt;
  std::vector<Shard> shards;
  std::vector<blsgpu_stats> sst;
  std::vector<int> rc;
  std::atomic<uint32_t> remaining{0};
  std::chrono::steady_clock::time_point t0;
  blsgpu_done_cb done = nullptr;
  void* user = nullptr;
  bool sync = false;
  std::mutex m;
  std::condition_variable cv;
  bool finished = false;
  int status = BLSGPU_OK;
};

}

namespace {

void shard_rule(const uint32_t* jfs, const uint32_t* spf, uint32_t n_jobs, uint32_t n_parts, uint32_t* out) {
  const uint32_t n_sets = n_jobs ? jfs[n_jobs] : 0;
  std::vector<double> set_prefix(n_sets + 1, 0.0);
  for (uint32_t i = 0; i < n_sets; i++)
    set_prefix[i + 1] = set_prefix[i] + 1.0 + (spf ? (double)(spf[i + 1] - spf[i]) / 256.0 : 0.0);
  std::vector<double> cost(n_jobs + 1);
  for (uint32_t j = 0; j <= n_jobs; j++) cost[j] = set_prefix[n_jobs ? jfs[j] : 0];
  uint32_t j0 = 0;
  out[0] = 0;
  for (uint32_t k = 0; k < n_parts; k++) {
    uint32_t j1;
    if (k + 1 == n_parts) {
      j1 = n_jobs;
    } else {
      const double target = cost[n_jobs] * (k + 1) / n_parts;
      j1 = (uint32_t)(std::upper_bound(cost.begin(), cost.end(), target) - cost.begin());
      j1 = j1 ? j1 - 1 : 0;
      j1 = std::max(j0, j1);
    }
    out[k + 1] = j1;
    j0 = j1;
  }
}

uint32_t route_rule(uint32_t n_sets, uint32_t n_dev, const int64_t* load, int64_t split_sets, uint32_t start,
                    uint32_t* out) {
  if (n_dev == 0) return 0;
  const uint64_t per = (uint64_t)std::max<int64_t>(1, split_sets);
  const uint32_t k = (uint32_t)std::max<uint64_t>(1, std::min<uint64_t>(n_dev, n_sets / per));
  std::vector<uint32_t> order(n_dev);
  for (uint32_t d = 0; d < n_dev; d++) order[d] = d;
  std::stable_sort(order.begin(), order.end(), [&](uint32_t a, uint32_t b) {
    if (load[a] != load[b]) return load[a] < load[b];
    return (a + n_dev - start % n_dev) % n_dev < (b + n_dev - start % n_dev) % n_dev;
  });
  std::sort(order.begin(), order.begin() + k);
  for (uint32_t i = 0; i < k; i++) out[i] = order[i];
  return k;
}


uint32_t adapt_group_sets(Device& d, int64_t group_sets, double sets_per_job) {
  double f;
  {
    std::lock_guard<std::mutex> lk(d.fail_mu);
    f = d.fail_rate;
  }
  const uint32_t gmax = (uint32_t)std::max<int64_t>(1, group_sets);
  if (f <= 0 || gmax <= 8) return gmax;
  const double retry = 13600.0 / (16.0 * std::max(1.0, sets_per_job)) + 1300.0, fixed = 14700.0;
  uint32_t best = gmax;
  double best_c = fixed / gmax + (1.0 - std::pow(1.0 - f, (double)gmax)) * retry;
  for (uint32_t g = 8; g < gmax; g *= 2) {
    const double c = fixed / g + (1.0 - std::pow(1.0 - f, (double)g)) * retry;
    if (c < best_c) best_c = c, best = g;
  }
  return best;
}

static bool host_trace() {
  static const bool on = [] {
    const char* v = getenv("BLSGPU_HOST_TRACE");
    return v && v[0] == '1';
  }();
  return on;
}
thread_local std::chrono::steady_clock::time_point tl_run_t0;
thread_local double tl_merge_ms = 0;

void release_inflight(Device& d, Slot& sl) {
  {
    std::lock_guard<std::mutex> lk(d.q_mu);
    if (!sl.in_flight) return;
    sl.in_flight = false;
    d.runs_inflight--;
  }
  d.q_cv.notify_all();
}

int run_shard(Device& d, Slot& sl, const blsgpu_batch& b, const Shard& sh, int8_t* job_result, uint64_t seed,
              const Options& opt, uint32_t max_index, blsgpu_stats& st, const uint64_t* scal_words,
              const std::vector<GroupPlanEntry>* plan = nullptr) {
  const uint32_t n = sh.set_end - sh.set_begin;
  const uint32_t nj = sh.job_end - sh.job_begin;
  if (nj == 0) return BLSGPU_OK;
  HIPCHK(hipSetDevice(d.id));
  const auto t_prep0 = std::chrono::steady_clock::now();
  const uint64_t grow0 = tl_async_grow;
  const uint32_t s0 = sh.set_begin;
  const uint32_t stride = std::max<uint32_t>(n, 1);
  const bool table_mode = b.pk_bytes == nullptr;
  const bool bytes_agg = b.pk_bytes && b.set_pk_first;
  const uint32_t pk_base = b.set_pk_first ? b.set_pk_first[s0] : 0;
  const uint32_t npk = b.set_pk_first ? b.set_pk_first[sh.set_end] - pk_base : 0;
  if (table_mode && npk && max_index >= d.table_n) return BLSGPU_ERR_ARGS;

  std::vector<uint64_t> scal(n);
  std::vector<std::pair<uint32_t, uint32_t>> group_jobs;
  std::vector<uint8_t> group_batchable;
  if (plan) {
    for (const GroupPlanEntry& g : *plan) {
      uint32_t sets = 0;
      for (uint32_t j = g.first; j < g.end; j++)
        sets += b.job_first_set[sh.job_begin + j + 1] - b.job_first_set[sh.job_begin + j];
      if (!sets) continue;
      group_jobs.push_back({g.first, g.end});
      group_batchable.push_back(g.batchable);
    }
  } else {
    const uint32_t gs = opt.group_adapt ? adapt_group_sets(d, opt.group_sets, (double)n / std::max(nj, 1u))
                                        : (uint32_t)opt.group_sets;
    uint32_t cur_sets = 0;
    bool open = false;
    for (uint32_t j = 0; j < nj; j++) {
      const uint32_t gj = sh.job_begin + j;
      const uint32_t a = b.job_first_set[gj] - s0, e = b.job_first_set[gj + 1] - s0;
      const bool batchable = b.job_flags && (b.job_flags[gj] & 1u);
      if (e == a) {
        open = false;
        continue;
      }
      if (!batchable) {
        group_jobs.push_back({j, j + 1});
        open = false;
        continue;
      }
      if (!open || cur_sets >= gs) {
        group_jobs.push_back({j, j});
        cur_sets = 0;
        open = true;
      }
      group_jobs.back().second = j + 1;
      cur_sets += e - a;
    }
  }
  memcpy(scal.data(), scal_words, (size_t)n * 8);
  auto job_sets = [&](uint32_t j) {
    const uint32_t gj = sh.job_begin + j;
    return std::make_pair(b.job_first_set[gj] - s0, b.job_first_set[gj + 1] - s0);
  };
  const uint32_t ng0 = (uint32_t)group_jobs.size();

  std::vector<uint32_t> msg_idx(n), uniq;
  if (opt.dedupe) {
    MsgIndex mi(n, seed ^ 0x6a09e667f3bcc908ull);
    uniq.reserve(n);
    const uint8_t* ms = b.msgs + (size_t)s0 * 32;
    constexpr uint32_t kAhead = 16;
    size_t hq[kAhead];
    for (uint32_t i = 0; i < std::min(n, kAhead); i++) {
      hq[i] = mi.hash(ms, i);
      __builtin_prefetch(&mi.slot[hq[i]]);
    }
    for (uint32_t i = 0; i < n; i++) {
      const size_t h = hq[i % kAhead];
      if (i + kAhead < n) {
        hq[i % kAhead] = mi.hash(ms, i + kAhead);
        __builtin_prefetch(&mi.slot[hq[i % kAhead]]);
      }
      msg_idx[i] = mi.find_or_add_h(ms, i, h, uniq);
    }
  } else {
    uniq.resize(n);
    for (uint32_t i = 0; i < n; i++) msg_idx[i] = uniq[i] = i;
  }
  const uint32_t n_umsg = (uint32_t)uniq.size();
  const uint32_t nm = std::max<uint32_t>(n_umsg, 1);
  const double t_dedupe_ms = host_trace() ? ms_since(t_prep0) : 0;
  std::vector<uint32_t> unit_of_set(n, UINT32_MAX), unit_msg, unit_first, unit_sets, g_unit_first(ng0 + 1, 0);
  bool merged = false;
  if (opt.dedupe && n_umsg < n) {
    std::vector<uint32_t> stamp(n_umsg, UINT32_MAX), unit_of_msg(n_umsg, 0);
    for (uint32_t g = 0; g < ng0; g++) {
      g_unit_first[g] = (uint32_t)unit_msg.size();
      const uint32_t a = job_sets(group_jobs[g].first).first, e = job_sets(group_jobs[g].second - 1).second;
      for (uint32_t i = a; i < e; i++) {
        const uint32_t m = msg_idx[i];
        if (stamp[m] != g) {
          stamp[m] = g;
          unit_of_msg[m] = (uint32_t)unit_msg.size();
          unit_msg.push_back(m);
        }
        unit_of_set[i] = unit_of_msg[m];
      }
    }
    g_unit_first[ng0] = (uint32_t)unit_msg.size();
    merged = unit_msg.size() < (size_t)n;
    if (merged) {
      const uint32_t nu = (uint32_t)unit_msg.size();
      unit_first.assign(nu + 1, 0);
      for (uint32_t i = 0; i < n; i++)
        if (unit_of_set[i] != UINT32_MAX) unit_first[unit_of_set[i] + 1]++;
      for (uint32_t u = 0; u < nu; u++) unit_first[u + 1] += unit_first[u];
      unit_sets.resize(unit_first[nu]);
      std::vector<uint32_t> fill(unit_first.begin(), unit_first.end() - 1);
      for (uint32_t i = 0; i < n; i++)
        if (unit_of_set[i] != UINT32_MAX) unit_sets[fill[unit_of_set[i]]++] = i;
    }
  }
  const uint32_t n_units = merged ? (uint32_t)unit_msg.size() : 0;
  const uint32_t n_items = merged ? n_units : n;
  const bool coop = n_items <= (uint32_t)opt.coop_max && opt.miller_k <= 1;
  const bool coop_g2 = n <= (uint32_t)opt.coop_g2_max;
  const bool excl = BLSGPU_EXCLUSIVE_SMALL && n_items <= (uint32_t)opt.coop_excl_max && (!sl.urgent || opt.urgent_excl);
  const uint32_t mk = coop ? 1u : opt.miller_k > 0 ? (uint32_t)opt.miller_k : miller_k_auto(n_items);
  std::vector<uint32_t> chunk_first{0}, chunk_items, g_chunks(2 * (size_t)ng0);
  chunk_items.reserve(n);
  for (uint32_t g = 0; g < ng0; g++) {
    const uint32_t a = merged ? g_unit_first[g] : job_sets(group_jobs[g].first).first;
    const uint32_t e = merged ? g_unit_first[g + 1] : job_sets(group_jobs[g].second - 1).second;
    const auto cr = add_chunks(chunk_first, chunk_items, a, e, mk);
    g_chunks[2 * g] = cr.first;
    g_chunks[2 * g + 1] = cr.second;
  }
  const uint32_t n_chunks = (uint32_t)chunk_first.size() - 1;
  const bool keep_f = opt.keep_f && !merged && mk == 1 && n_chunks == n;
  const bool small = n <= (uint32_t)opt.small_max;
  const bool spec = BLSGPU_STREAM_PAIRS && (small || opt.spec_large) && sl.alone && !opt.serial;
  const bool rsig_spec = spec && small && opt.rsig_spec;
  constexpr uint32_t kMsmHalfSliceMaxSets = 32768, kMsmSmallSliceMaxSets = 1024;
  const uint32_t slice_len = n <= kMsmSmallSliceMaxSets  ? 32
                             : n <= kMsmHalfSliceMaxSets ? (uint32_t)opt.msm_slice_mid
                                                         : MSM_SLICE;
  std::vector<uint32_t> slices, range_slices{0};
  uint32_t msm_tree = 0;
  for (uint32_t g = 0; g < ng0; g++)
    add_slices(slices, range_slices, job_sets(group_jobs[g].first).first, job_sets(group_jobs[g].second - 1).second,
               slice_len);
  const uint32_t n_slices = (uint32_t)(slices.size() / 2);
  if (n <= kMsmHalfSliceMaxSets && opt.msm_tree) {
    for (uint32_t g = 0; g < ng0; g++) msm_tree = std::max(msm_tree, range_slices[g + 1] - range_slices[g]);
    if ((uint64_t)ng0 * msm_tree > 2ull * n_slices) msm_tree = 0;
  }
  std::vector<uint32_t> ftree, f_level_end;
  uint32_t f_k = 1, f_max = 0;
  if (n_chunks > 16384)
    for (const uint32_t heads = opt.f_run_max > 16 ? 256u : 8192u;
         n_chunks / f_k > heads && f_k < (uint32_t)opt.f_run_max;)
      f_k *= 2;
  for (uint32_t g = 0; g < ng0; g++) f_max = std::max(f_max, g_chunks[2 * g + 1] - g_chunks[2 * g]);
  if (f_k > 1)
    for (uint32_t g = 0; g < ng0; g++)
      for (uint32_t x = g_chunks[2 * g], e = g_chunks[2 * g + 1]; x < e; x += f_k)
        if (std::min(e, x + f_k) - x > 1) {
          ftree.push_back(x);
          ftree.push_back(std::min(e, x + f_k));
        }
  const uint32_t n_fruns = (uint32_t)(ftree.size() / 2);
  for (uint32_t st = f_k; st < f_max; st *= 2) {
    for (uint32_t g = 0; g < ng0; g++)
      for (uint32_t i = g_chunks[2 * g], e = g_chunks[2 * g + 1]; i + st < e; i += 2 * st) {
        ftree.push_back(i);
        ftree.push_back(i + st);
      }
    f_level_end.push_back((uint32_t)(ftree.size() / 2) - n_fruns);
  }
  std::vector<uint32_t> agg_sets;
  if (table_mode || bytes_agg)
    for (uint32_t i = 0; i < n; i++)
      if (b.set_pk_first[s0 + i + 1] - b.set_pk_first[s0 + i] >= 2) agg_sets.push_back(i);

  const double t_struct_ms = host_trace() ? ms_since(t_prep0) : 0;
  uint32_t sig_w = 96;
  for (uint32_t i = 0; i < n; i++)
    if (b.sig_len[s0 + i] == 192) {
      sig_w = 192;
      break;
    }
  const size_t o_scal = 0, o_jobs = al256(o_scal + (size_t)n * 8), o_sigs = al256(o_jobs + (size_t)(nj + 1) * 4),
               o_siglen = al256(o_sigs + (size_t)n * sig_w), o_umsg = al256(o_siglen + (size_t)n * 4),
               o_midx = al256(o_umsg + (size_t)n_umsg * 32), o_ranges = al256(o_midx + (size_t)n * 4),
               o_franges = al256(o_ranges + (size_t)std::max(ng0, 1u) * 8),
               o_ufirst = al256(o_franges + (size_t)std::max(ng0, 1u) * 8),
               o_usets = al256(o_ufirst + (size_t)(n_units + 1) * 4), o_umsgi = al256(o_usets + (size_t)unit_sets.size() * 4),
               o_cfirst = al256(o_umsgi + (size_t)n_units * 4), o_citems = al256(o_cfirst + (size_t)(n_chunks + 1) * 4),
               o_agg = al256(o_citems + chunk_items.size() * 4), o_slices = al256(o_agg + agg_sets.size() * 4),
               o_rslices = al256(o_slices + slices.size() * 4), o_ftree = al256(o_rslices + range_slices.size() * 4),
               o_pk = al256(o_ftree + ftree.size() * 4);
  size_t in_bytes;
  if (table_mode)
    in_bytes = al256(o_pk + (size_t)(n + 1) * 4) + (size_t)npk * 4;
  else if (bytes_agg)
    in_bytes = al256(o_pk + (size_t)(n + 1) * 4) + (size_t)npk * 96;
  else
    in_bytes = o_pk + (size_t)n * 96;
  const size_t o_pk2 = al256(o_pk + (size_t)(n + 1) * 4);
  hipStream_t* const dst = sl.urgent ? d.ust : d.st;
  const int npairs = sl.urgent ? 2 : d.npairs;
  const int par = sl.urgent ? 0 : BLSGPU_STREAM_PAIRS ? (int)(d.run_seq.fetch_add(1) % (uint32_t)npairs) : 0;
  const int other = (par + 1) % npairs;
  hipStream_t s = BLSGPU_STREAM_PAIRS ? dst[2 * par] : dst[kSig];
  sl.set_stream(s);
  sl.h_in.ensure(in_bytes);
  sl.d_in.ensure(in_bytes);
  uint8_t* const hin = sl.h_in.p;
  memcpy(hin + o_scal, scal.data(), (size_t)n * 8);
  uint32_t* hjobs = reinterpret_cast<uint32_t*>(hin + o_jobs);
  for (uint32_t j = 0; j < nj; j++) hjobs[j] = job_sets(j).first;
  hjobs[nj] = n;
  uint8_t* hsigs = hin + o_sigs;
  uint32_t* hsiglen = reinterpret_cast<uint32_t*>(hin + o_siglen);
  if (b.sig_stride == sig_w) {
    memcpy(hsigs, b.sigs + (size_t)s0 * sig_w, (size_t)n * sig_w);
    memcpy(hsiglen, b.sig_len + s0, (size_t)n * 4);
  } else {
    for (uint32_t i = 0; i < n; i++) {
      const uint32_t len = b.sig_len[s0 + i];
      const uint32_t cl = (len == 96 || len == 192) ? len : 0;
      memcpy(hsigs + (size_t)i * sig_w, b.sigs + (size_t)(s0 + i) * b.sig_stride, cl);
      hsiglen[i] = len;
    }
  }
  for (uint32_t u = 0; u < n_umsg; u++) memcpy(hin + o_umsg + (size_t)u * 32, b.msgs + (size_t)(s0 + uniq[u]) * 32, 32);
  memcpy(hin + o_midx, msg_idx.data(), (size_t)n * 4);
  uint32_t* hranges = reinterpret_cast<uint32_t*>(hin + o_ranges);
  uint32_t* hfranges = reinterpret_cast<uint32_t*>(hin + o_franges);
  for (uint32_t g = 0; g < ng0; g++) {
    hranges[2 * g] = job_sets(group_jobs[g].first).first;
    hranges[2 * g + 1] = job_sets(group_jobs[g].second - 1).second;
    hfranges[2 * g] = g_chunks[2 * g];
    hfranges[2 * g + 1] = g_chunks[2 * g + 1];
  }
  memcpy(hin + o_cfirst, chunk_first.data(), chunk_first.size() * 4);
  memcpy(hin + o_citems, chunk_items.data(), chunk_items.size() * 4);
  if (!agg_sets.empty()) memcpy(hin + o_agg, agg_sets.data(), agg_sets.size() * 4);
  if (!slices.empty()) memcpy(hin + o_slices, slices.data(), slices.size() * 4);
  memcpy(hin + o_rslices, range_slices.data(), range_slices.size() * 4);
  if (!ftree.empty()) memcpy(hin + o_ftree, ftree.data(), ftree.size() * 4);
  if (merged) {
    memcpy(hin + o_ufirst, unit_first.data(), (size_t)(n_units + 1) * 4);
    memcpy(hin + o_usets, unit_sets.data(), unit_sets.size() * 4);
    memcpy(hin + o_umsgi, unit_msg.data(), (size_t)n_units * 4);
  }
  if (table_mode || bytes_agg) {
    uint32_t* hpkfirst = reinterpret_cast<uint32_t*>(hin + o_pk);
    for (uint32_t i = 0; i <= n; i++) hpkfirst[i] = b.set_pk_first[s0 + i] - pk_base;
    if (table_mode)
      memcpy(hin + o_pk2, b.pk_index + pk_base, (size_t)npk * 4);
    else
      memcpy(hin + o_pk2, b.pk_bytes + (size_t)pk_base * 96, (size_t)npk * 96);
  } else {
    memcpy(hin + o_pk, b.pk_bytes + (size_t)s0 * 96, (size_t)n * 96);
  }

  const size_t ob_flags = 0, ob_mflags = al256(n), ob_unit = al256(ob_mflags + nm), ob_status = al256(ob_unit + n),
               ob_include = al256(ob_status + 3 * (size_t)stride), ob_spec = al256(ob_include + stride),
               bytes_total = al256(ob_spec + stride);
  sl.d_bytes.ensure(bytes_total);
  const uint32_t max_ranges = std::max<uint32_t>(std::max(ng0, nj), 1);
  const size_t o_ok = al256(nj), res_bytes = o_ok + max_ranges;
  sl.d_res.ensure(res_bytes);
  sl.h_res.ensure(res_bytes);
  sl.d_S.ensure((size_t)W_G2J * max_ranges);
  sl.d_F.ensure((size_t)W_FP12 * max_ranges);
  sl.d_G.ensure((size_t)W_FP12 * std::max<uint32_t>(ng0, 1));
  sl.d_msmB.ensure((size_t)MSM_BUCKET_WORDS * std::max<uint32_t>(n_slices, 1));
  sl.d_msmW.ensure((size_t)MSM_WINDOW_WORDS * max_ranges);
  const size_t per_set = W_G2A + W_G1J + W_G1A + W_FP12 + 8 * W_G1J + 2 * W_FP + (merged ? W_G1A : 0);
  sl.d_work.ensure((size_t)stride * per_set + (size_t)nm * (W_G2A + W_G2J + W_FP + 14 * W_FP + 2 * W_G2J));
  sl.d_lines.ensure((size_t)nm * kMillerLineWords);
  if (keep_f) sl.d_fkeep.ensure((size_t)stride * W_FP12);
  if (rsig_spec) sl.d_fb.ensure((size_t)stride * 9 * W_G2J);
  uint8_t* const din = sl.d_in.p;
  uint8_t* const d_ok0 = sl.d_res.p + o_ok;

  PipelineBuffers pb;
  memset(&pb, 0, sizeof pb);
  pb.n = stride;
  pb.sigs = din + o_sigs;
  pb.sig_len = reinterpret_cast<uint32_t*>(din + o_siglen);
  pb.sig_stride = sig_w;
  pb.pk_bytes = table_mode ? nullptr : din + (bytes_agg ? o_pk2 : o_pk);
  pb.set_pk_first = (table_mode || bytes_agg) ? reinterpret_cast<uint32_t*>(din + o_pk) : nullptr;
  pb.pk_index = table_mode ? reinterpret_cast<uint32_t*>(din + o_pk2) : nullptr;
  pb.pk_table = d.table.p;
  pb.pk_table_n = d.table_n;
  pb.agg_sets = reinterpret_cast<uint32_t*>(din + o_agg);
  pb.n_agg = (uint32_t)agg_sets.size();
  pb.pk_direct1 = 1;
  pb.scalars = reinterpret_cast<uint64_t*>(din + o_scal);
  pb.job_first_set = reinterpret_cast<uint32_t*>(din + o_jobs);
  pb.n_jobs = nj;
  pb.umsgs = din + o_umsg;
  pb.msg_idx = reinterpret_cast<uint32_t*>(din + o_midx);
  pb.n_umsg = n_umsg;
  pb.nm = nm;
  pb.n_units = n_units;
  pb.unit_set_first = reinterpret_cast<uint32_t*>(din + o_ufirst);
  pb.unit_sets = reinterpret_cast<uint32_t*>(din + o_usets);
  pb.unit_msg = reinterpret_cast<uint32_t*>(din + o_umsgi);
  uint32_t* w = sl.d_work.p;
  pb.sig_aff = w; w += (size_t)stride * W_G2A;
  pb.pk_jac = w; w += (size_t)stride * W_G1J;
  pb.pk_aff = w; w += (size_t)stride * W_G1A;
  pb.rsig = nullptr;
  pb.f_chunk = w; w += (size_t)stride * W_FP12;
  pb.scal_tab = w; w += (size_t)stride * 8 * W_G1J;
  if (merged) {
    pb.unit_p = w; w += (size_t)stride * W_G1A;
  }
  pb.n_chunks = n_chunks;
  pb.chunk_first = reinterpret_cast<uint32_t*>(din + o_cfirst);
  pb.chunk_items = reinterpret_cast<uint32_t*>(din + o_citems);
  pb.inv_buf = w; w += (size_t)stride * W_FP;
  pb.inv_buf_pk = w; w += (size_t)stride * W_FP;
  pb.h_aff = w; w += (size_t)nm * W_G2A;
  pb.h_jac = w; w += (size_t)nm * W_G2J;
  pb.h_norm = w; w += (size_t)nm * W_FP;
  pb.h_prep = w; w += (size_t)nm * 14 * W_FP;
  pb.h_q = w;
  pb.lines = sl.d_lines.p;
  uint8_t* const db = sl.d_bytes.p;
  pb.flags = db + ob_flags;
  pb.mflags = db + ob_mflags;
  pb.unit_ok = db + ob_unit;
  pb.status = reinterpret_cast<int8_t*>(db + ob_status);
  pb.include = db + ob_include;
  pb.job_err = reinterpret_cast<int8_t*>(sl.d_res.p);

  const bool prof = opt.profile;
  const bool lane_tail = opt.lane_tail_min > 0 && n >= (uint32_t)opt.lane_tail_min;
  hipStream_t sm = BLSGPU_STREAM_PAIRS ? dst[2 * par + 1] : dst[kMsg],
              sp = BLSGPU_STREAM_PAIRS ? (small && sl.alone ? dst[2 * other] : s) : dst[kPk],
              stl = BLSGPU_STREAM_PAIRS ? s : dst[kTail];
  if (opt.serial) sm = sp = stl = s;
  auto beg = [&](int k, hipStream_t st) {
    if (prof) HIPCHK(hipEventRecord(sl.ev[2 * k], st));
  };
  auto end = [&](int k, hipStream_t st) {
    if (prof) HIPCHK(hipEventRecord(sl.ev[2 * k + 1], st));
  };
  {
    std::unique_lock<std::mutex> enq(d.enq_mu, std::defer_lock);
    if (!sl.urgent) enq.lock();
    st.host_ms = ms_since(tl_run_t0);
    if (host_trace())
      fprintf(stderr,
              "[blsgpu host] run %u sets: merge %.2f ms, prep %.2f ms (dedupe %.2f, structure %.2f), pick-to-copy %.2f "
              "ms, %zu B in\n",
              n, tl_merge_ms, ms_since(t_prep0), t_dedupe_ms, t_struct_ms, ms_since(tl_run_t0), in_bytes);
    const bool own_copy = opt.copy_stream && !opt.serial && !sl.urgent && tl_async_grow == grow0;
    hipStream_t sc = own_copy ? d.table_stream : s;
    HIPCHK(hipMemcpyAsync(din, hin, in_bytes, hipMemcpyHostToDevice, sc));
    HIPCHK(hipEventRecord(sl.join_in, sc));
    if (own_copy) HIPCHK(hipStreamWaitEvent(s, sl.join_in, 0));
    HIPCHK(hipStreamWaitEvent(sm, sl.join_in, 0));
    HIPCHK(hipStreamWaitEvent(sp, sl.join_in, 0));
    beg(1, sm);
    launch_hash_to_g2(pb, sm, coop_g2, excl);
    launch_h_affine(pb, sm);
    end(1, sm);
    beg(kStages, sm);
    if (!coop) {
      const bool two = opt.lines_lanes == 2;
      if (two)
        launch_miller_lines2(pb, sm);
      else
        launch_miller_lines(pb, sm);
    }
    end(kStages, sm);
    beg(2, sp);
    if ((table_mode || bytes_agg) && pb.n_agg) launch_pk_aggregate(pb, n, sp);
    end(2, sp);
    beg(3, sp);
    launch_pk_finish(pb, n, sp);
    launch_pk_affine(pb, n, sp);
    end(3, sp);
    HIPCHK(hipEventRecord(sl.join_pk, sp));
    hipStream_t smsm = spec ? dst[2 * other + 1] : s;
    PipelineBuffers pbm = pb;
    if (spec) pbm.include = db + ob_spec;
    beg(0, s);
    launch_sig_decode(pb, n, s, coop_g2, spec ? sl.join_dec : nullptr, excl);
    end(0, s);
    const uint32_t* d_slices = reinterpret_cast<uint32_t*>(din + o_slices);
    const uint32_t* d_rslices = reinterpret_cast<uint32_t*>(din + o_rslices);
    if (rsig_spec) {
      HIPCHK(hipEventRecord(sl.join_rsig, s));
      HIPCHK(hipStreamWaitEvent(sp, sl.join_rsig, 0));
      PipelineBuffers pq = pb;
      pq.rsig = sl.d_fb.p;
      pq.scal_tab = sl.d_fb.p + (size_t)stride * W_G2J;
      launch_sig_scale(pq, n, sp);
      HIPCHK(hipEventRecord(sl.join_rsig, sp));
    }
    if (spec) {
      HIPCHK(hipStreamWaitEvent(smsm, sl.join_dec, 0));
      launch_spec_mask(pb, n, pbm.include, smsm);
      launch_sig_msm(pbm, d_slices, n_slices, d_rslices, ng0, sl.d_msmB.p, sl.d_msmW.p, sl.d_S.p, smsm, false,
                     msm_tree);
      HIPCHK(hipEventRecord(sl.join_msm, smsm));
    }
    HIPCHK(hipStreamWaitEvent(s, sl.join_pk, 0));
    beg(4, s);
    launch_job_mask(pb, s);
    HIPCHK(hipEventRecord(sl.join_mask, s));
    HIPCHK(hipStreamWaitEvent(sm, sl.join_mask, 0));
    beg(5, sm);
    if (merged) launch_unit_aggregate(pb, sm);
    if (coop)
      launch_miller_coop(pb, merged, sm, excl);
    else
      launch_miller_acc_auto(pb, merged, sm, mk, opt.miller_lanes, opt.acc6_max, opt.miller_pairs != 0);
    end(5, sm);
    if (keep_f && opt.keep_copy == 1)
      launch_copy_words(sl.d_fkeep.p, pb.f_chunk, (size_t)stride * W_FP12, sm);
    else if (keep_f)
      HIPCHK(hipMemcpyAsync(sl.d_fkeep.p, pb.f_chunk, (size_t)stride * W_FP12 * 4, hipMemcpyDeviceToDevice, sm));
    const uint32_t* d_franges = reinterpret_cast<uint32_t*>(din + o_franges);
    beg(6, sm);
    const uint32_t* d_ftree = reinterpret_cast<uint32_t*>(din + o_ftree);
    launch_group_tree(pb, d_franges, ng0, d_ftree, n_fruns, d_ftree + 2 * (size_t)n_fruns, f_level_end, sl.d_F.p, sm);
    end(6, sm);
    HIPCHK(hipEventRecord(sl.join_msg, sm));
    if (spec)
      HIPCHK(hipStreamWaitEvent(s, sl.join_msm, 0));
    else
      launch_sig_msm(pb, d_slices, n_slices, d_rslices, ng0, sl.d_msmB.p, sl.d_msmW.p, sl.d_S.p, s,
                     lane_tail && (opt.lane_tail_parts & 1), msm_tree);
    end(4, s);
    const bool tail_msg = opt.tail_on_msg && !opt.serial && BLSGPU_STREAM_PAIRS;
    hipStream_t sg = s;
    if (spec && opt.spec_gsm && !tail_msg) sg = smsm;
    if (tail_msg) {
      HIPCHK(hipEventRecord(sl.join_gsm, s));
      HIPCHK(hipStreamWaitEvent(sm, sl.join_gsm, 0));
      sg = stl = sm;
    }
    beg(kStages + 1, sg);
    launch_group_sig_miller(sl.d_S.p, ng0, sl.d_G.p, sg, excl && coop,
                            lane_tail && (opt.lane_tail_parts & 2));
    end(kStages + 1, sg);
    HIPCHK(hipEventRecord(sl.join_gsm, sg));
    HIPCHK(hipStreamWaitEvent(stl, sl.join_gsm, 0));
    HIPCHK(hipStreamWaitEvent(stl, sl.join_msg, 0));
    if (rsig_spec) HIPCHK(hipStreamWaitEvent(stl, sl.join_rsig, 0));
    beg(7, stl);
    launch_group_check(sl.d_S.p, sl.d_F.p, ng0, d_ok0, stl, nullptr, 0, sl.d_G.p, excl && coop);
    end(7, stl);
    HIPCHK(hipGetLastError());
    HIPCHK(hipMemcpyAsync(sl.h_res.p, sl.d_res.p, o_ok + ng0, hipMemcpyDeviceToHost, stl));
    HIPCHK(hipEventRecord(sl.done, stl));
  }
  if (opt.early_release && !opt.serial) {
    HIPCHK(hipEventSynchronize(sl.join_msg));
    release_inflight(d, sl);
  }
  HIPCHK(hipEventSynchronize(sl.done));
  if (batch_rand::take_injection(g_fail_run_skip, g_fail_run_count)) throw HipError{hipErrorLaunchFailure};
  release_inflight(d, sl);
  st.groups += ng0;
  st.unique_messages += n_umsg;
  st.pairing_units += merged ? n_units : n;
  st.miller_chunks += n_chunks;
  st.run_sets = n;
  if (prof) {
    for (int k = 0; k < kStages; k++) {
      float ms = 0;
      HIPCHK(hipEventElapsedTime(&ms, sl.ev[2 * k], sl.ev[2 * k + 1]));
      if (k == 5 || k == 7) {
        const int x = k == 5 ? kStages : kStages + 1;
        float ml = 0;
        HIPCHK(hipEventElapsedTime(&ml, sl.ev[2 * x], sl.ev[2 * x + 1]));
        ms += ml;
      }
      st.stage_ms[k] += ms;
    }
  }

  std::vector<int> jr(nj, 0);
  for (uint32_t j = 0; j < nj; j++) {
    const int err = (int8_t)sl.h_res.p[j];
    jr[j] = err ? -err : 2;
  }
  std::vector<uint32_t> retry;
  std::vector<uint32_t> failed_g;
  for (uint32_t g = 0; g < ng0; g++) {
    std::vector<uint32_t> clean;
    bool dropped = false;
    for (uint32_t j = group_jobs[g].first; j < group_jobs[g].second; j++) {
      if (jr[j] == 2)
        clean.push_back(j);
      else if (job_sets(j).second > job_sets(j).first)
        dropped = true;
    }
    if (spec && dropped && !clean.empty()) {
      if (plan && group_batchable[g]) st.batch_retries++;
      if (!plan && clean.size() > 1) st.batch_retries++;
      retry.insert(retry.end(), clean.begin(), clean.end());
      continue;
    }
    if (plan) {
      if (!group_batchable[g]) {
      } else if (clean.size() == group_jobs[g].second - group_jobs[g].first && sl.h_res.p[o_ok + g]) {
        st.batch_sigs_success += job_sets(group_jobs[g].second - 1).second - job_sets(group_jobs[g].first).first;
      } else {
        st.batch_retries++;
      }
    }
    if (clean.empty()) continue;
    if (plan) {
      if (sl.h_res.p[o_ok + g]) {
        for (uint32_t j : clean) jr[j] = 1;
      } else {
        retry.insert(retry.end(), clean.begin(), clean.end());
        failed_g.push_back(g);
      }
      continue;
    }
    if (sl.h_res.p[o_ok + g]) {
      for (uint32_t j : clean) jr[j] = 1;
      if (group_jobs[g].second - group_jobs[g].first > 1)
        for (uint32_t j : clean) st.batch_sigs_success += job_sets(j).second - job_sets(j).first;
    } else {
      if (clean.size() > 1) st.batch_retries++;
      retry.insert(retry.end(), clean.begin(), clean.end());
      failed_g.push_back(g);
    }
  }

  if (!retry.empty()) {
    constexpr uint32_t kFbSub = 16;
    constexpr uint32_t kFbLaneMin = 128;
    const uint32_t nr = (uint32_t)retry.size();
    const hipStream_t sfb = sl.fb ? sl.fb : stl;
    sl.set_stream(sfb);
    std::vector<uint32_t> rfirst{0}, ritems, rr(2 * (size_t)nr), rf(2 * (size_t)nr), rsl, rrs{0}, rset;
    for (uint32_t q = 0; q < nr; q++) {
      const auto js = job_sets(retry[q]);
      rr[2 * q] = js.first;
      rr[2 * q + 1] = js.second;
      add_slices(rsl, rrs, js.first, js.second);
      for (uint32_t i = js.first; i < js.second; i++) rset.push_back(i);
      if (keep_f) {
        rf[2 * q] = js.first;
        rf[2 * q + 1] = js.second;
        continue;
      }
      const auto cr = add_chunks(rfirst, ritems, js.first, js.second, mk);
      rf[2 * q] = cr.first;
      rf[2 * q + 1] = cr.second;
    }
    const bool small_jobs = rset.size() < (size_t)32 * nr;
    constexpr uint32_t kFbDirectMax = 640;
    const bool busy = (!small && !sl.alone) || opt.fb_force_busy;
    auto lane_checks = [&](uint32_t count) { return busy && opt.fb_lane_min > 0 && count >= (uint32_t)opt.fb_lane_min; };
    const bool direct = (small && nr <= kFbDirectMax) || (busy && opt.fb_direct_min > 0 && nr >= (uint32_t)opt.fb_direct_min);
    const uint32_t nsub = !direct && nr >= 2 * kFbSub ? (nr + kFbSub - 1) / kFbSub : 0;
    auto fb_check = [&](const uint32_t* S, const uint32_t* F, uint32_t ng, uint8_t* ok, const uint32_t* sel,
                        uint32_t count) {
      if (lane_checks(count) && opt.fb_check6 == 2) {
        sl.d_lines.ensure((size_t)ng * kMillerLineWords);
        sl.d_fbflags.ensure(ng);
        launch_check6_miller(S, F, ng, ok, sfb, sel, count, sl.d_lines.p, sl.d_fbflags.p);
      } else if (lane_checks(count) && opt.fb_check6) {
        sl.d_G.ensure((size_t)W_FP12 * ng);
        launch_group_sig_miller_sel(S, ng, sel, count, sl.d_G.p, sfb);
        launch_group_check6(F, sl.d_G.p, ng, ok, sfb, sel, count);
      } else {
        launch_group_check(S, F, ng, ok, sfb, sel, count, nullptr, false, lane_checks(count));
      }
    };
    std::vector<uint32_t> subr(2 * (size_t)nsub);
    for (uint32_t t = 0; t < nsub; t++) {
      subr[2 * t] = t * kFbSub;
      subr[2 * t + 1] = std::min(nr, (t + 1) * kFbSub);
    }
    const uint32_t nc = (uint32_t)rfirst.size() - 1;
    const uint32_t nrs = (uint32_t)(rsl.size() / 2);
    const size_t o_rsl = 4 * (size_t)nr + rfirst.size() + ritems.size(), o_rrs = o_rsl + rsl.size(),
                 o_rset = o_rrs + rrs.size(), o_sub = o_rset + rset.size(), o_sel = o_sub + subr.size();
    const size_t words = o_sel + nr;
    sl.h_list.ensure(words);
    sl.d_list.ensure(words);
    uint32_t* hl = sl.h_list.p;
    memcpy(hl, rr.data(), rr.size() * 4);
    memcpy(hl + 2 * (size_t)nr, rf.data(), rf.size() * 4);
    memcpy(hl + 4 * (size_t)nr, rfirst.data(), rfirst.size() * 4);
    memcpy(hl + 4 * (size_t)nr + rfirst.size(), ritems.data(), ritems.size() * 4);
    memcpy(hl + o_rsl, rsl.data(), rsl.size() * 4);
    memcpy(hl + o_rrs, rrs.data(), rrs.size() * 4);
    memcpy(hl + o_rset, rset.data(), rset.size() * 4);
    if (nsub) memcpy(hl + o_sub, subr.data(), subr.size() * 4);
    sl.d_ok.ensure(nr + nsub);
    sl.h_ok.ensure(nr + nsub);
    sl.d_S.ensure((size_t)W_G2J * (nr + nsub));
    sl.d_F.ensure((size_t)W_FP12 * (nr + nsub));
    uint32_t* const dS = sl.d_S.p;
    uint32_t* const dF = sl.d_F.p;
    uint32_t* const dS_sub = sl.d_S.p + (size_t)W_G2J * nr;
    uint32_t* const dF_sub = sl.d_F.p + (size_t)W_FP12 * nr;
    HIPCHK(hipMemcpyAsync(sl.d_list.p, hl, o_sel * 4, hipMemcpyHostToDevice, sfb));
    PipelineBuffers pr = pb;
    pr.n_chunks = nc;
    pr.chunk_first = sl.d_list.p + 4 * (size_t)nr;
    pr.chunk_items = sl.d_list.p + 4 * (size_t)nr + rfirst.size();
    if (keep_f) {
      pr.f_chunk = sl.d_fkeep.p;
    } else {
      st.fallback_miller += (uint32_t)ritems.size();
      if (coop)
        launch_miller_coop(pr, false, sfb);
      else
        launch_miller_acc_auto(pr, false, sfb, mk, opt.miller_lanes, opt.acc6_max, opt.miller_pairs != 0);
    }
    st.fallback_jobs += nr;
    if (small_jobs) {
      if (!rsig_spec) sl.d_fb.ensure((size_t)stride * 9 * W_G2J);
      pr.rsig = sl.d_fb.p;
      pr.scal_tab = sl.d_fb.p + (size_t)stride * W_G2J;
      if (!rsig_spec) launch_sig_scale(pr, (uint32_t)rset.size(), sfb, sl.d_list.p + o_rset);
      launch_group_reduce_lane(pr, sl.d_list.p, sl.d_list.p + 2 * (size_t)nr, nr, dS, dF, sfb);
    } else {
      sl.d_msmB.ensure((size_t)MSM_BUCKET_WORDS * std::max<uint32_t>(nrs, 1));
      sl.d_msmW.ensure((size_t)MSM_WINDOW_WORDS * nr);
      launch_sig_msm(pr, sl.d_list.p + o_rsl, nrs, sl.d_list.p + o_rrs, nr, sl.d_msmB.p, sl.d_msmW.p, dS, sfb);
      launch_group_reduce(pr, sl.d_list.p + 2 * (size_t)nr, nr, dF, sfb);
    }
    std::vector<uint32_t> sel;
    if (nsub) {
      if (nsub >= kFbLaneMin)
        launch_range_combine_lane(dS, dF, nr, sl.d_list.p + o_sub, nsub, dS_sub, dF_sub, sfb);
      else
        launch_range_combine(dS, dF, nr, sl.d_list.p + o_sub, nsub, dS_sub, dF_sub, sfb);
      fb_check(dS_sub, dF_sub, nsub, sl.d_ok.p + nr, nullptr, nsub);
      HIPCHK(hipGetLastError());
      HIPCHK(hipMemcpyAsync(sl.h_ok.p + nr, sl.d_ok.p + nr, nsub, hipMemcpyDeviceToHost, sfb));
      HIPCHK(hipEventRecord(sl.done, sfb));
      HIPCHK(hipEventSynchronize(sl.done));
      for (uint32_t t = 0; t < nsub; t++)
        for (uint32_t q = subr[2 * t]; q < subr[2 * t + 1]; q++) {
          if (sl.h_ok.p[nr + t]) jr[retry[q]] = 1;
          else sel.push_back(q);
        }
    } else {
      for (uint32_t q = 0; q < nr; q++) sel.push_back(q);
    }
    if (!sel.empty()) {
      const uint32_t ns = (uint32_t)sel.size();
      memcpy(hl + o_sel, sel.data(), (size_t)ns * 4);
      HIPCHK(hipMemcpyAsync(sl.d_list.p + o_sel, hl + o_sel, (size_t)ns * 4, hipMemcpyHostToDevice, sfb));
      fb_check(dS, dF, nr, sl.d_ok.p, sl.d_list.p + o_sel, ns);
      HIPCHK(hipGetLastError());
      HIPCHK(hipMemcpyAsync(sl.h_ok.p, sl.d_ok.p, ns, hipMemcpyDeviceToHost, sfb));
      HIPCHK(hipEventRecord(sl.done, sfb));
      HIPCHK(hipEventSynchronize(sl.done));
      for (uint32_t k = 0; k < ns; k++) jr[retry[sel[k]]] = sl.h_ok.p[k] ? 1 : 0;
    }
    if (fb_verify() && small_jobs) {
      HIPCHK(hipDeviceSynchronize());
      const size_t wS = (size_t)W_G2J * nr, wF = (size_t)W_FP12 * nr;
      std::vector<uint32_t> S1(wS), F1(wF), S2(wS), F2(wF), L(o_sel);
      std::vector<uint8_t> ok_now(sel.size() + 1), ok2(nr);
      HIPCHK(hipMemcpy(S1.data(), dS, wS * 4, hipMemcpyDeviceToHost));
      HIPCHK(hipMemcpy(F1.data(), dF, wF * 4, hipMemcpyDeviceToHost));
      HIPCHK(hipMemcpy(L.data(), sl.d_list.p, o_sel * 4, hipMemcpyDeviceToHost));
      if (!sel.empty()) HIPCHK(hipMemcpy(ok_now.data(), sl.d_ok.p, sel.size(), hipMemcpyDeviceToHost));
      uint32_t *t_rs = nullptr, *t_S = nullptr, *t_F = nullptr;
      uint8_t* t_ok = nullptr;
      HIPCHK(hipMalloc((void**)&t_rs, (size_t)stride * 9 * W_G2J * 4));
      HIPCHK(hipMalloc((void**)&t_S, wS * 4));
      HIPCHK(hipMalloc((void**)&t_F, wF * 4));
      HIPCHK(hipMalloc((void**)&t_ok, nr));
      PipelineBuffers pq = pr;
      pq.rsig = t_rs;
      pq.scal_tab = t_rs + (size_t)stride * W_G2J;
      launch_sig_scale(pq, (uint32_t)rset.size(), sfb, sl.d_list.p + o_rset);
      launch_group_reduce_lane(pq, sl.d_list.p, sl.d_list.p + 2 * (size_t)nr, nr, t_S, t_F, sfb);
      launch_group_check(t_S, t_F, nr, t_ok, sfb, nullptr, 0, nullptr, false, false);
      HIPCHK(hipStreamSynchronize(sfb));
      HIPCHK(hipMemcpy(S2.data(), t_S, wS * 4, hipMemcpyDeviceToHost));
      HIPCHK(hipMemcpy(F2.data(), t_F, wF * 4, hipMemcpyDeviceToHost));
      HIPCHK(hipMemcpy(ok2.data(), t_ok, nr, hipMemcpyDeviceToHost));
      (void)hipFree(t_rs), (void)hipFree(t_S), (void)hipFree(t_F), (void)hipFree(t_ok);
      uint32_t sdiff = 0, fdiff = 0, vdiff = 0, stale = 0, ldiff = 0, first_v = UINT32_MAX, last_v = 0;
      for (uint32_t q = 0; q < nr; q++) {
        bool ds = false, df = false;
        for (size_t w = 0; w < W_G2J && !ds; w++) ds = S1[w * nr + q] != S2[w * nr + q];
        for (size_t w = 0; w < W_FP12 && !df; w++) df = F1[w * nr + q] != F2[w * nr + q];
        sdiff += ds, fdiff += df;
        if ((jr[retry[q]] == 1) != (ok2[q] != 0)) {
          vdiff++;
          first_v = std::min(first_v, q);
          last_v = q;
        }
      }
      for (size_t k = 0; k < o_sel; k++) ldiff += L[k] != hl[k];
      for (size_t k = 0; k < sel.size(); k++) stale += (ok_now[k] != 0) != (sl.h_ok.p[k] != 0);
      if (vdiff || sdiff || fdiff || stale || ldiff)
        fprintf(stderr, "[blsgpu fbverify] %u-set run, %u retried jobs (nsub %u, direct %d, busy %d, keep_f %d, rsig_spec "
                "%d, spec %d, coop %d, lanes %d): answers that differ on re-check %u (q %u-%u), S_j differ %u, F_j differ "
                "%u, results read vs now %u, list words %zu\n", n, nr, nsub, (int)direct, (int)busy, (int)keep_f,
                (int)rsig_spec, (int)spec, (int)coop, (int)lane_checks((uint32_t)sel.size()), vdiff, first_v, last_v,
                sdiff, fdiff, stale, (size_t)ldiff);
      else
        fprintf(stderr, "[blsgpu fbverify] ok: %u-set run, %u retried jobs\n", n, nr);
    }
  }
  for (uint32_t g : failed_g) {
    bool all_ok = true;
    for (uint32_t j = group_jobs[g].first; j < group_jobs[g].second && all_ok; j++)
      if (jr[j] != 1 && jr[j] >= 0) all_ok = false;
    if (all_ok) {
      d.spurious_groups.fetch_add(1, std::memory_order_relaxed);
      fprintf(stderr, "[blsgpu] device %d: batch group %u (jobs %u-%u) of a %u-set run failed its equation while "
              "every job verifies on its own (spec %d, merged %d, coop %d, mk %u)\n", d.id, g, group_jobs[g].first,
              group_jobs[g].second - 1, n, (int)spec, (int)merged, (int)coop, mk);
    }
  }
  for (uint32_t j = 0; j < nj; j++) job_result[sh.job_begin + j] = (int8_t)jr[j];
  if (!plan && ng0) {
    uint32_t failed = 0;
    for (uint32_t g = 0; g < ng0; g++)
      for (uint32_t j = group_jobs[g].first; j < group_jobs[g].second; j++)
        if (jr[j] != 1 && job_sets(j).second > job_sets(j).first) {
          failed++;
          break;
        }
    const double pf = std::min((double)failed, ng0 - 0.5) / ng0;
    const double f = 1.0 - std::pow(1.0 - pf, (double)ng0 / std::max(n, 1u));
    std::lock_guard<std::mutex> lk(d.fail_mu);
    d.fail_rate = 0.5 * d.fail_rate + 0.5 * f;
  }
  return BLSGPU_OK;
}

uint32_t max_table_index(const blsgpu_batch* b) {
  uint32_t m = 0;
  if (!b->pk_bytes && b->n_sets)
    for (uint32_t k = 0; k < b->set_pk_first[b->n_sets]; k++) m = std::max(m, b->pk_index[k]);
  return m;
}

int validate_batch(const blsgpu_batch* b) {
  if (!b || !b->job_first_set) return BLSGPU_ERR_ARGS;
  if (b->n_jobs == 0) return b->n_sets == 0 ? BLSGPU_OK : BLSGPU_ERR_ARGS;
  if (b->job_first_set[0] != 0 || b->job_first_set[b->n_jobs] != b->n_sets) return BLSGPU_ERR_ARGS;
  for (uint32_t j = 0; j < b->n_jobs; j++)
    if (b->job_first_set[j + 1] < b->job_first_set[j]) return BLSGPU_ERR_ARGS;
  if (b->n_sets == 0) return BLSGPU_OK;
  if (!b->msgs || !b->sigs || !b->sig_len) return BLSGPU_ERR_ARGS;
  if (b->sig_stride < 96) return BLSGPU_ERR_ARGS;
  for (uint32_t i = 0; i < b->n_sets; i++)
    if (b->sig_len[i] > b->sig_stride && (b->sig_len[i] == 96 || b->sig_len[i] == 192)) return BLSGPU_ERR_ARGS;
  if (!b->pk_bytes && (!b->set_pk_first || !b->pk_index)) return BLSGPU_ERR_ARGS;
  if (b->set_pk_first) {
    if (b->set_pk_first[0] != 0) return BLSGPU_ERR_ARGS;
    for (uint32_t i = 0; i < b->n_sets; i++)
      if (b->set_pk_first[i + 1] < b->set_pk_first[i]) return BLSGPU_ERR_ARGS;
  }
  return BLSGPU_OK;
}


void finish_call(Call* c) {
  blsgpu_stats local{};
  int status = BLSGPU_OK;
  for (int k = 0; k < kStages; k++) local.stage_ms[k] = c->sst.empty() ? 0 : c->sst[0].stage_ms[k];
  for (size_t k = 0; k < c->shards.size(); k++) {
    local.groups += c->sst[k].groups;
    local.batch_retries += c->sst[k].batch_retries;
    local.batch_sigs_success += c->sst[k].batch_sigs_success;
    local.unique_messages += c->sst[k].unique_messages;
    local.pairing_units += c->sst[k].pairing_units;
    local.miller_chunks += c->sst[k].miller_chunks;
    local.fallback_jobs += c->sst[k].fallback_jobs;
    local.fallback_miller += c->sst[k].fallback_miller;
    local.urgent_lane |= c->sst[k].urgent_lane;
    local.host_ms = std::max(local.host_ms, c->sst[k].host_ms);
    if (c->rc[k] != BLSGPU_OK && c->rc[k] != BLSGPU_DEVICE_ERROR) status = c->rc[k];
  }
  local.run_sets = c->sst.empty() ? 0 : c->sst[0].run_sets;
  local.run_calls = c->sst.empty() ? 0 : c->sst[0].run_calls;
  local.devices_used = (uint32_t)c->shards.size();
  local.device_ms = std::chrono::duration<double, std::milli>(std::chrono::steady_clock::now() - c->t0).count();
  if (c->stats) *c->stats = local;
  blsgpu_ctx* ctx = c->ctx;
  if (c->sync) {
    std::lock_guard<std::mutex> lk(c->m);
    c->status = status;
    c->finished = true;
    c->cv.notify_all();
  } else {
    blsgpu_done_cb done = c->done;
    void* user = c->user;
    delete c->owned;
    delete c;
    if (done) try {
        done(user, status);
      } catch (...) {
      }
  }
  leave(ctx);
}

inline int pk_mode(const blsgpu_batch& b) { return !b.pk_bytes ? 0 : (b.set_pk_first ? 2 : 1); }

void shard_scalars(const blsgpu_batch& b, const Shard& sh, const batch_rand::Key& key, uint64_t* out) {
  if (sh.set_end > sh.set_begin) batch_rand::words(key, sh.set_begin, sh.set_end - sh.set_begin, out);
  for (uint32_t j = sh.job_begin; j < sh.job_end; j++) {
    const uint32_t a = b.job_first_set[j], e = b.job_first_set[j + 1];
    const bool batchable = b.job_flags && (b.job_flags[j] & 1u);
    if (!batchable && e - a == 1) out[a - sh.set_begin] = 0;
  }
}

int run_pool_policy(Device& d, Slot& sl, const blsgpu_batch& b, const Shard& sh, int8_t* job_result, uint64_t seed,
                    const Options& opt, uint32_t max_index, blsgpu_stats& st, const uint64_t* scal_words) {
  const uint32_t s0 = sh.set_begin, n = sh.set_end - sh.set_begin;
  std::vector<uint64_t> scal0(std::max<uint32_t>(n, 1));
  memcpy(scal0.data(), scal_words, (size_t)n * 8);
  struct Sub {
    uint32_t call, a, e;
    bool batchable;
  };
  std::vector<Sub> subs;
  for (uint32_t j = sh.job_begin; j < sh.job_end; j++) {
    const uint32_t a = b.job_first_set[j], e = b.job_first_set[j + 1];
    const bool bt = b.job_flags && (b.job_flags[j] & 1u);
    if (a == e) {
      subs.push_back({j, a, a, bt});
      continue;
    }
    const uint32_t per = chunk_size(e - a, 128);
    for (uint32_t k = a; k < e; k += per) subs.push_back({j, k, std::min(e, k + per), bt});
  }
  std::vector<uint32_t> order;
  std::vector<GroupPlanEntry> plan;
  for (size_t q = 0; q < subs.size();) {
    size_t q1 = q;
    uint32_t total = 0;
    while (q1 < subs.size() && total < 128) total += subs[q1].e - subs[q1].a, q1++;
    std::vector<uint32_t> bat, rest;
    for (size_t x = q; x < q1; x++) (subs[x].batchable && subs[x].e > subs[x].a ? bat : rest).push_back((uint32_t)x);
    if (!bat.empty()) {
      const uint32_t per = chunk_size((uint32_t)bat.size(), 16);
      for (size_t k = 0; k < bat.size(); k += per) {
        GroupPlanEntry g{(uint32_t)order.size(), 0, true};
        for (size_t x = k; x < std::min(bat.size(), k + per); x++) order.push_back(bat[x]);
        g.end = (uint32_t)order.size();
        plan.push_back(g);
      }
    }
    for (uint32_t x : rest) {
      plan.push_back({(uint32_t)order.size(), (uint32_t)order.size() + 1, false});
      order.push_back(x);
    }
    q = q1;
  }
  const int mode = pk_mode(b);
  const uint32_t ns = (uint32_t)subs.size();
  std::vector<uint32_t> jfs{0}, siglen, spf{0}, pki;
  std::vector<uint8_t> flags, msgs, sigs, pkb;
  std::vector<uint64_t> scal;
  jfs.reserve(ns + 1);
  siglen.reserve(n);
  scal.reserve(n);
  msgs.reserve((size_t)n * 32);
  sigs.reserve((size_t)n * b.sig_stride);
  for (uint32_t x : order) {
    const Sub& u = subs[x];
    jfs.push_back(jfs.back() + u.e - u.a);
    flags.push_back(u.batchable ? 1 : 0);
    for (uint32_t i = u.a; i < u.e; i++) {
      siglen.push_back(b.sig_len[i]);
      sigs.insert(sigs.end(), b.sigs + (size_t)i * b.sig_stride, b.sigs + (size_t)(i + 1) * b.sig_stride);
      msgs.insert(msgs.end(), b.msgs + (size_t)i * 32, b.msgs + (size_t)i * 32 + 32);
      scal.push_back(scal0[i - s0]);
      if (mode == 1) {
        pkb.insert(pkb.end(), b.pk_bytes + (size_t)i * 96, b.pk_bytes + (size_t)(i + 1) * 96);
      } else {
        const uint32_t k0 = b.set_pk_first[i], k1 = b.set_pk_first[i + 1];
        spf.push_back(spf.back() + k1 - k0);
        if (mode == 0)
          pki.insert(pki.end(), b.pk_index + k0, b.pk_index + k1);
        else
          pkb.insert(pkb.end(), b.pk_bytes + (size_t)k0 * 96, b.pk_bytes + (size_t)k1 * 96);
      }
    }
  }
  blsgpu_batch pb{};
  pb.n_sets = n;
  pb.n_jobs = ns;
  pb.job_first_set = jfs.data();
  pb.job_flags = flags.data();
  pb.pk_bytes = mode ? pkb.data() : nullptr;
  pb.set_pk_first = mode == 1 ? nullptr : spf.data();
  pb.pk_index = mode == 0 ? pki.data() : nullptr;
  pb.msgs = msgs.data();
  pb.sigs = sigs.data();
  pb.sig_len = siglen.data();
  pb.sig_stride = b.sig_stride;
  std::vector<int8_t> sub_res(std::max<uint32_t>(ns, 1), 0);
  const Shard all{0, ns, 0, n};
  const int rc = run_shard(d, sl, pb, all, sub_res.data(), seed, opt, max_index, st, scal.data(), &plan);
  if (rc != BLSGPU_OK) return rc;
  std::vector<uint32_t> pos(ns);
  for (uint32_t k = 0; k < ns; k++) pos[order[k]] = k;
  std::vector<uint8_t> seen(sh.job_end - sh.job_begin, 0);
  for (uint32_t j = sh.job_begin; j < sh.job_end; j++) job_result[j] = 1;
  for (uint32_t x = 0; x < ns; x++) {
    const uint32_t call = subs[x].call;
    const int8_t r = sub_res[pos[x]];
    if (seen[call - sh.job_begin]) continue;
    if (r < 0) {
      job_result[call] = r;
      seen[call - sh.job_begin] = 1;
// ... 380 lines not shown
  for (auto& e : s->ev)
    if (e) (void)hipEventDestroy(e);
  for (hipEvent_t e : {s->join_in, s->join_msg, s->join_pk, s->join_mask, s->join_gsm, s->join_dec, s->join_msm,
                       s->join_rsig, s->done})
    if (e) (void)hipEventDestroy(e);
  if (s->fb) (void)hipStreamSynchronize(s->fb), (void)hipStreamDestroy(s->fb);
  delete s;
}

hipStream_t make_stream(const std::vector<uint32_t>& mask, int prio) {
  hipStream_t st = nullptr;
  if (!mask.empty())
    HIPCHK(hipExtStreamCreateWithCUMask(&st, (uint32_t)mask.size(), mask.data()));
  else
    HIPCHK(hipStreamCreateWithPriority(&st, hipStreamNonBlocking, prio));
  return st;
}

void create_streams(blsgpu_ctx* ctx, Device* d) {
  HIPCHK(hipSetDevice(d->id));
  int prio_lo = 0, prio_hi = 0;
  HIPCHK(hipDeviceGetStreamPriorityRange(&prio_lo, &prio_hi));
  int n_cu = 0;
  HIPCHK(hipDeviceGetAttribute(&n_cu, hipDeviceAttributeMultiprocessorCount, d->id));
  const int part = (int)std::min<int64_t>(ctx->urgent_cus, n_cu / 2) & ~7;
  d->urgent_cus = part;
  const size_t words = (size_t)(n_cu + 31) / 32;
  std::vector<uint32_t> pmask(words, 0);
  d->main_mask.clear();
  for (int i = 0; i < n_cu; i++)
    if (part == 0 || i < part) pmask[i / 32] |= 1u << (i % 32);
  if (part > 0 && ctx->urgent_isolate == 1) {
    d->main_mask.assign(words, 0);
    for (int i = part; i < n_cu; i++) d->main_mask[i / 32] |= 1u << (i % 32);
  }
  if (ctx->urgent_isolate == 3) d->main_mask.assign(words, ~0u);
  if (ctx->urgent_isolate == 2) pmask.clear();
  d->npairs = ctx->hw_queues >= 6 ? kMaxPairs : 2;
  for (int k = 0; k < 2 * d->npairs; k++) {
    const bool high = ctx->pipeline_prio && ((BLSGPU_STREAM_PRIO & (1 << (k & 3))) != 0 || (k >= kStreams && (k & 1)));
    d->st[k] = make_stream(d->main_mask, high ? prio_hi : prio_lo);
  }
  d->umask = pmask;
  d->uprio = prio_hi;
#if BLSGPU_URGENT_EAGER
  for (int k = 0; k < 4; k++) d->ust[k] = make_stream(d->umask, d->uprio);
#endif
}

bool ensure_urgent_streams(Device* d, Slot* sl) {
  if (d->ust[0]) return true;
  try {
    HIPCHK(hipSetDevice(d->id));
    for (int k = 0; k < 4; k++) d->ust[k] = make_stream(d->umask, d->uprio);
  } catch (HipError&) {
    for (hipStream_t& st : d->ust)
      if (st) (void)hipStreamDestroy(st), st = nullptr;
    return false;
  }
  sl->set_stream(d->ust[0]);
  return true;
}

void create_slot_events(Device* d, Slot* s) {
  const unsigned wait_flags = hipEventDisableTiming | (d->blocking_sync ? hipEventBlockingSync : 0u);
  for (hipEvent_t* e : {&s->join_in, &s->join_pk, &s->join_mask, &s->join_gsm, &s->join_dec, &s->join_msm, &s->join_rsig})
    HIPCHK(hipEventCreateWithFlags(e, hipEventDisableTiming));
  for (hipEvent_t* e : {&s->join_msg, &s->done}) HIPCHK(hipEventCreateWithFlags(e, wait_flags));
  for (auto& e : s->ev) HIPCHK(hipEventCreate(&e));
}

void add_slot(Device* d) {
  Slot* s = new Slot();
  HIPCHK(hipSetDevice(d->id));
  try {
    s->set_stream(d->st[kSig]);
    create_slot_events(d, s);
    int prio_lo = 0, prio_hi = 0;
    HIPCHK(hipDeviceGetStreamPriorityRange(&prio_lo, &prio_hi));
    s->fb = make_stream(d->main_mask, prio_lo);
  } catch (HipError&) {
    free_slot(d, s);
    throw;
  }
  d->slots.push_back(s);
  d->workers.emplace_back(worker_loop, d, s);
}

void resize_slots(Device* d, int64_t want) {
  std::vector<std::thread> joins;
  std::vector<Slot*> gone;
  {
    std::lock_guard<std::mutex> lk(d->q_mu);
    while ((int64_t)d->slots.size() < want) add_slot(d);
    while ((int64_t)d->slots.size() > want) {
      Slot* s = d->slots.back();
      s->retire = true;
      gone.push_back(s);
      joins.push_back(std::move(d->workers.back()));
      d->slots.pop_back();
      d->workers.pop_back();
    }
  }
  d->q_cv.notify_all();
  for (size_t k = 0; k < joins.size(); k++) {
    try {
      joins[k].join();
      free_slot(d, gone[k]);
    } catch (std::system_error&) {
      joins[k].detach();
    }
  }
}

void destroy_device(Device* d) {
  {
    std::lock_guard<std::mutex> lk(d->q_mu);
    d->stop = true;
  }
  d->q_cv.notify_all();
  for (auto& t : d->workers) t.join();
  if (d->uworker.joinable()) d->uworker.join();
  for (Slot* s : d->slots) free_slot(d, s);
  if (d->uslot) free_slot(d, d->uslot);
  (void)hipSetDevice(d->id);
  for (hipStream_t st : d->st)
    if (st) (void)hipStreamSynchronize(st), (void)hipStreamDestroy(st);
  for (hipStream_t st : d->ust)
    if (st) (void)hipStreamSynchronize(st), (void)hipStreamDestroy(st);
  for (hipStream_t st : d->same_st)
    if (st) (void)hipStreamSynchronize(st), (void)hipStreamDestroy(st);
  for (hipEvent_t e : d->same_ev)
    if (e) (void)hipEventDestroy(e);
  d->helper.release_all();
  d->table.release();
  if (d->table_stream) (void)hipStreamDestroy(d->table_stream);
  delete d;
}

int64_t hw_queues_of_process() {
  const char* v = getenv("GPU_MAX_HW_QUEUES");
  const long q = v ? strtol(v, nullptr, 10) : 0;
  return q > 0 ? q : 4;
}

int64_t default_slots(int64_t) { return 3; }

int ensure_slots(blsgpu_ctx* ctx) {
  std::lock_guard<std::mutex> lk(ctx->slots_mu);
  if (ctx->slots_started) return BLSGPU_OK;
  try {
    for (Device* d : ctx->devs) {
      if (!d->st[0]) {
        d->blocking_sync = ctx->blocking_sync != 0;
        create_streams(ctx, d);
      }
      resize_slots(d, ctx->slots_per_device);
      if (!d->uslot) {
        Slot* u = new Slot();
        u->urgent = true;
        try {
          u->set_stream(d->ust[0]);
          create_slot_events(d, u);
        } catch (HipError&) {
          free_slot(d, u);
          throw;
        }
        d->uslot = u;
        try {
          d->uworker = std::thread(urgent_loop, d, u);
        } catch (std::system_error&) {
          d->uslot = nullptr;
          free_slot(d, u);
          return BLSGPU_DEVICE_ERROR;
        }
      }
    }
  } catch (HipError&) {
    return BLSGPU_DEVICE_ERROR;
  }
  ctx->slots_started = true;
  return BLSGPU_OK;
}

int64_t shard_cost(const blsgpu_batch& b, const Shard& sh) {
  int64_t c = 256 * (int64_t)(sh.set_end - sh.set_begin);
  if (b.set_pk_first) c += b.set_pk_first[sh.set_end] - b.set_pk_first[sh.set_begin];
  return c;
}

bool launch_urgent(blsgpu_ctx* ctx, Call* c) {
  const blsgpu_batch& b = c->b;
  const uint32_t nd = (uint32_t)std::min<int64_t>((int64_t)ctx->devs.size(), c->opt.max_devices);
  if (!c->opt.urgent_lane || (int64_t)b.n_sets > c->opt.urgent_max_sets || nd == 0) return false;
  const uint32_t start = ctx->route_seq.fetch_add(1, std::memory_order_relaxed) % nd;
  uint32_t best = start;
  for (uint32_t k = 1; k < nd; k++) {
    const uint32_t x = (start + k) % nd;
    if (ctx->devs[x]->upending.load(std::memory_order_relaxed) < ctx->devs[best]->upending.load(std::memory_order_relaxed))
      best = x;
  }
  Device* d = ctx->devs[best];
  if (!d->uslot) return false;
  Shard sh{0, b.n_jobs, 0, b.n_sets};
  sh.dev = best;
  sh.cost = 0;
  c->shards.push_back(sh);
  c->sst.assign(1, blsgpu_stats{});
  c->rc.assign(1, BLSGPU_OK);
  c->remaining = 1;
  c->t0 = std::chrono::steady_clock::now();
  d->upending.fetch_add(1, std::memory_order_relaxed);
  {
    std::lock_guard<std::mutex> lk(d->q_mu);
    d->uqueue.push_back({c, 0});
  }
  d->q_cv.notify_all();
  return true;
}

void launch_call(blsgpu_ctx* ctx, Call* c) {
  const blsgpu_batch& b = c->b;
  bool urgent = false;
  if (b.job_flags)
    for (uint32_t j = 0; j < b.n_jobs && !urgent; j++) urgent = (b.job_flags[j] & BLSGPU_JOB_URGENT) != 0;
  if (urgent && launch_urgent(ctx, c)) return;
  const uint32_t nd_all = (uint32_t)std::min<int64_t>((int64_t)ctx->devs.size(), c->opt.max_devices);
  std::vector<int64_t> load(nd_all);
  for (uint32_t d = 0; d < nd_all; d++) load[d] = ctx->devs[d]->load.load(std::memory_order_relaxed);
  std::vector<uint32_t> devs(std::max<uint32_t>(nd_all, 1));
  const uint32_t nd = route_rule(b.n_sets, nd_all, load.data(), c->opt.route_split_sets,
                                 ctx->route_seq.fetch_add(1, std::memory_order_relaxed), devs.data());
  std::vector<uint32_t> parts(nd + 1);
  shard_rule(b.job_first_set, b.set_pk_first, b.n_jobs, nd, parts.data());
  for (uint32_t k = 0; k < nd; k++) {
    Shard sh{parts[k], parts[k + 1], b.n_jobs ? b.job_first_set[parts[k]] : 0,
             b.n_jobs ? b.job_first_set[parts[k + 1]] : 0};
    sh.dev = devs[k];
    sh.cost = shard_cost(b, sh);
    c->shards.push_back(sh);
  }
  c->sst.assign(nd, blsgpu_stats{});
  c->rc.assign(nd, BLSGPU_OK);
  c->remaining = nd;
  c->t0 = std::chrono::steady_clock::now();
  for (uint32_t k = 0; k < nd; k++) {
    Device* d = ctx->devs[c->shards[k].dev];
    d->load.fetch_add(c->shards[k].cost, std::memory_order_relaxed);
    {
      std::lock_guard<std::mutex> lk(d->q_mu);
      if (urgent)
        d->queue.push_front({c, k});
      else
        d->queue.push_back({c, k});
    }
    d->q_cv.notify_all();
  }
}

}
bool blsgpu_rt::resolve_key(uint64_t seed, batch_rand::Key& key, uint64_t& hash_key) {
  if (seed == 0) {
    if (!batch_rand::os_key(key)) return false;
    hash_key = batch_rand::hash_key(key);
  } else {
    key = batch_rand::seed_key(seed);
    hash_key = batch_rand::hash_key(key);
  }
  return true;
}
namespace {

void reject_all(const blsgpu_batch* b, int8_t* job_result, int code) {
  if (job_result)
    for (uint32_t j = 0; j < b->n_jobs; j++) job_result[j] = (int8_t)-code;
}

Options snapshot(blsgpu_ctx* ctx) {
  std::lock_guard<std::mutex> lk(ctx->opt_mu);
  return ctx->opt;
}

}

extern "C" {

int blsgpu_init(const int* devices, int n_devices, blsgpu_ctx** out) {
  if (!out) return BLSGPU_ERR_ARGS;
  *out = nullptr;
  int count = 0;
  if (hipGetDeviceCount(&count) != hipSuccess || count <= 0) return BLSGPU_ERR_NO_DEVICE;
  std::vector<int> ids;
  if (devices && n_devices > 0) {
    for (int i = 0; i < n_devices; i++) {
      if (devices[i] < 0 || devices[i] >= count) return BLSGPU_ERR_ARGS;
      ids.push_back(devices[i]);
    }
  } else {
    for (int i = 0; i < count; i++) ids.push_back(i);
  }
  blsgpu_ctx* ctx = new blsgpu_ctx();
  ctx->hw_queues = hw_queues_of_process();
  ctx->slots_per_device = default_slots(ctx->hw_queues);
  try {
    for (int id : ids) {
      Device* d = new Device();
      d->id = id;
      ctx->devs.push_back(d);
      HIPCHK(hipSetDevice(id));
      HIPCHK(hipStreamCreateWithFlags(&d->table_stream, hipStreamNonBlocking));
    }
  } catch (HipError&) {
    blsgpu_destroy(ctx);
    return BLSGPU_ERR_NO_DEVICE;
  }
  *out = ctx;
  return BLSGPU_OK;
}

void blsgpu_destroy(blsgpu_ctx* ctx) {
  if (!ctx) return;
  {
    std::unique_lock<std::mutex> lk(ctx->active_mu);
    ctx->closed = true;
    ctx->active_cv.wait(lk, [&] { return ctx->active == 0; });
  }
  for (Device* d : ctx->devs) destroy_device(d);
  delete ctx;
}

int blsgpu_device_count(const blsgpu_ctx* ctx) { return ctx ? (int)ctx->devs.size() : 0; }

uint32_t blsgpu_pubkeys_count(const blsgpu_ctx* ctx) {
  if (!ctx || ctx->devs.empty()) return 0;
  uint32_t n = UINT32_MAX;
  for (Device* d : ctx->devs) {
    std::shared_lock<std::shared_mutex> lk(d->table_mu);
    n = std::min(n, d->table_n);
  }
  return n;
}

int blsgpu_pubkeys_upload(blsgpu_ctx* ctx, uint32_t first_index, const uint8_t* pk96, uint32_t n) {
  if (!ctx) return BLSGPU_ERR_ARGS;
  if (n == 0) return BLSGPU_OK;
  if (!pk96) return BLSGPU_ERR_ARGS;
  if (!enter(ctx)) return BLSGPU_ERR_CLOSED;
  std::lock_guard<std::mutex> tl(ctx->table_mu);
  int result = BLSGPU_OK;
  for (Device* d : ctx->devs) {
    std::shared_lock<std::shared_mutex> lk(d->table_mu);
    if (first_index > d->table_n) result = BLSGPU_ERR_ARGS;
  }
  auto upload_one = [&](Device* d) -> int {
    try {
      HIPCHK(hipSetDevice(d->id));
      hipStream_t ts = d->table_stream;
      const uint32_t need = first_index + n;
      uint8_t* dpk = nullptr;
      int8_t* dst = nullptr;
      uint32_t* tmp = nullptr;
      HIPCHK(hipMalloc((void**)&dpk, (size_t)n * 96));
      HIPCHK(hipMalloc((void**)&dst, n));
      HIPCHK(hipMalloc((void**)&tmp, (size_t)n * W_PKTAB * 4));
      HIPCHK(hipMemcpyAsync(dpk, pk96, (size_t)n * 96, hipMemcpyHostToDevice, ts));
      launch_pk_table_fill(dpk, n, tmp, dst, ts);
      HIPCHK(hipGetLastError());
      std::vector<int8_t> hst(n);
      HIPCHK(hipMemcpyAsync(hst.data(), dst, n, hipMemcpyDeviceToHost, ts));
      HIPCHK(hipStreamSynchronize(ts));
      int err = 0;
      for (uint32_t i = 0; i < n && !err; i++) err = hst[i];
      if (!err) {
        std::unique_lock<std::shared_mutex> lk(d->table_mu);
        if (need > d->table.cap / W_PKTAB) {
          DevBuf<uint32_t> nt;
          nt.ensure((size_t)std::max<uint32_t>(need, d->table_n + d->table_n / 2) * W_PKTAB);
          if (d->table_n)
            HIPCHK(hipMemcpyAsync(nt.p, d->table.p, (size_t)d->table_n * W_PKTAB * 4, hipMemcpyDeviceToDevice, ts));
          d->table.release();
          d->table = nt;
        }
        HIPCHK(hipMemcpyAsync(d->table.p + (size_t)first_index * W_PKTAB, tmp, (size_t)n * W_PKTAB * 4,
                              hipMemcpyDeviceToDevice, ts));
        HIPCHK(hipStreamSynchronize(ts));
        d->table_n = std::max(d->table_n, need);
      }
      (void)hipFree(dpk);
      (void)hipFree(dst);
      (void)hipFree(tmp);
      return err;
    } catch (HipError&) {
      return BLSGPU_DEVICE_ERROR;
    } catch (std::exception&) {
      return BLSGPU_DEVICE_ERROR;
    }
  };
  if (!result) {
    std::vector<int> rc(ctx->devs.size(), 0);
    if (ctx->devs.size() == 1) {
      rc[0] = upload_one(ctx->devs[0]);
    } else {
      std::vector<std::thread> th;
      for (size_t k = 0; k < ctx->devs.size(); k++) th.emplace_back([&, k] { rc[k] = upload_one(ctx->devs[k]); });
      for (auto& t : th) t.join();
    }
    for (int r : rc)
      if (r && !result) result = r;
  }
  leave(ctx);
  return result;
}

int blsgpu_set_option(blsgpu_ctx* ctx, const char* key, int64_t value) {
  if (!ctx || !key) return BLSGPU_ERR_ARGS;
  std::string k(key);
  if (k == "urgent_cus" || k == "urgent_isolate" || k == "blocking_sync" || k == "pipeline_prio") {
    std::lock_guard<std::mutex> sk(ctx->slots_mu);
    if (ctx->slots_started) return BLSGPU_ERR_ARGS;
    if (k == "blocking_sync" || k == "pipeline_prio") {
      if (value < 0 || value > 1) return BLSGPU_ERR_ARGS;
      (k == "blocking_sync" ? ctx->blocking_sync : ctx->pipeline_prio) = value;
    } else if (k == "urgent_cus") {
      if (value < 0 || value > 128 || (value & 7)) return BLSGPU_ERR_ARGS;
      ctx->urgent_cus = value;
    } else {
      if (value < 0 || value > 3) return BLSGPU_ERR_ARGS;
      ctx->urgent_isolate = value;
    }
    return BLSGPU_OK;
  }
  if (k == "slots") {
    if (value < 1 || value > 64 || tl_dispatcher) return BLSGPU_ERR_ARGS;
    std::lock_guard<std::mutex> sk(ctx->slots_mu);
    ctx->slots_per_device = value;
    if (ctx->slots_started) {
      try {
        for (Device* d : ctx->devs) resize_slots(d, value);
      } catch (HipError&) {
        return BLSGPU_DEVICE_ERROR;
      }
    }
    return BLSGPU_OK;
  }
  std::lock_guard<std::mutex> lk(ctx->opt_mu);
  if (k == "group_sets") {
    if (value < 1) return BLSGPU_ERR_ARGS;
    ctx->opt.group_sets = value;
  } else if (k == "profile") {
    ctx->opt.profile = value != 0;
  } else if (k == "max_devices") {
    if (value < 1) return BLSGPU_ERR_ARGS;
    ctx->opt.max_devices = value;
  } else if (k == "dedupe") {
    ctx->opt.dedupe = value != 0;
  } else if (k == "merge_sets") {
    if (value < 0) return BLSGPU_ERR_ARGS;
    ctx->opt.merge_sets = value;
  } else if (k == "miller_k") {
    if (value < 0 || value > 64) return BLSGPU_ERR_ARGS;
    ctx->opt.miller_k = value;
  } else if (k == "group_policy") {
    if (value < 0 || value > 1) return BLSGPU_ERR_ARGS;
    ctx->opt.group_policy = value;
  } else if (k == "merge_wait_us") {
    if (value < 0 || value > 1000000) return BLSGPU_ERR_ARGS;
    ctx->opt.merge_wait_us = value;
  } else if (k == "idle_wait_us") {
    if (value < 0 || value > 1000000) return BLSGPU_ERR_ARGS;
    ctx->opt.idle_wait_us = value;
  } else if (k == "pipeline_depth") {
    if (value < 1 || value > 64) return BLSGPU_ERR_ARGS;
    ctx->opt.pipeline_depth = value;
  } else if (k == "serial") {
    ctx->opt.serial = value != 0;
  } else if (k == "miller_lanes") {
    if (value < 0 || (value > 3 && value != 6)) return BLSGPU_ERR_ARGS;
    ctx->opt.miller_lanes = value;
  } else if (k == "msm_slice_mid") {
    if (value < 8 || value > MSM_SLICE) return BLSGPU_ERR_ARGS;
    ctx->opt.msm_slice_mid = value;
  } else if (k == "copy_stream") {
    ctx->opt.copy_stream = value != 0;
  } else if (k == "tail_on_msg") {
    ctx->opt.tail_on_msg = value != 0;
  } else if (k == "early_release") {
    ctx->opt.early_release = value != 0;
  } else if (k == "merge_balance") {
    ctx->opt.merge_balance = value != 0;
  } else if (k == "lines_lanes") {
    if (value < 1 || value > 2) return BLSGPU_ERR_ARGS;
    ctx->opt.lines_lanes = value;
  } else if (k == "msm_tree") {
    ctx->opt.msm_tree = value != 0;
  } else if (k == "coop_max") {
    if (value < 0 || value > (1 << 24)) return BLSGPU_ERR_ARGS;
    ctx->opt.coop_max = value;
  } else if (k == "coop_g2_max") {
    if (value < 0 || value > (1 << 24)) return BLSGPU_ERR_ARGS;
    ctx->opt.coop_g2_max = value;
  } else if (k == "coop_excl_max") {
    if (value < 0 || value > (1 << 24)) return BLSGPU_ERR_ARGS;
    ctx->opt.coop_excl_max = value;
  } else if (k == "rsig_spec") {
    ctx->opt.rsig_spec = value != 0;
  } else if (k == "spec_large") {
    ctx->opt.spec_large = value != 0;
  } else if (k == "spec_gsm") {
    ctx->opt.spec_gsm = value != 0;
  } else if (k == "fb_lane_min") {
    if (value < 0) return BLSGPU_ERR_ARGS;
    ctx->opt.fb_lane_min = value;
  } else if (k == "fb_force_busy") {
    ctx->opt.fb_force_busy = value != 0;
  } else if (k == "keep_f") {
    ctx->opt.keep_f = value != 0;
  } else if (k == "keep_copy") {
    ctx->opt.keep_copy = value != 0;
  } else if (k == "urgent_lane") {
    ctx->opt.urgent_lane = value != 0;
  } else if (k == "urgent_max_sets") {
    if (value < 0) return BLSGPU_ERR_ARGS;
    ctx->opt.urgent_max_sets = value;
  } else if (k == "urgent_excl") {
    ctx->opt.urgent_excl = value != 0;
  } else if (k == "group_adapt") {
    ctx->opt.group_adapt = value != 0;
  } else if (k == "urgent_wait_us") {
    if (value < 0 || value > 100000) return BLSGPU_ERR_ARGS;
    ctx->opt.urgent_wait_us = value;
  } else if (k == "fb_check6") {
    if (value < 0 || value > 2) return BLSGPU_ERR_ARGS;
    ctx->opt.fb_check6 = value;
  } else if (k == "fb_direct_min") {
    if (value < 0) return BLSGPU_ERR_ARGS;
    ctx->opt.fb_direct_min = value;
  } else if (k == "small_max") {
    if (value < 0) return BLSGPU_ERR_ARGS;
    ctx->opt.small_max = value;
  } else if (k == "miller_pairs") {
    if (value < 0 || value > 1) return BLSGPU_ERR_ARGS;
    ctx->opt.miller_pairs = value;
  } else if (k == "acc6_max") {
    if (value < 0) return BLSGPU_ERR_ARGS;
    ctx->opt.acc6_max = value;
  } else if (k == "route_split_sets") {
    if (value < 1) return BLSGPU_ERR_ARGS;
    ctx->opt.route_split_sets = value;
  } else if (k == "lane_tail_parts") {
    if (value < 0 || value > 3) return BLSGPU_ERR_ARGS;
    ctx->opt.lane_tail_parts = value;
  } else if (k == "lane_tail_min") {
    if (value < 0) return BLSGPU_ERR_ARGS;
    ctx->opt.lane_tail_min = value;
  } else if (k == "f_run_max") {
    if (value < 1 || value > 1024 || (value & (value - 1))) return BLSGPU_ERR_ARGS;
    ctx->opt.f_run_max = value;
  } else {
    return BLSGPU_ERR_ARGS;
  }
  return BLSGPU_OK;
}

int blsgpu_get_option(const blsgpu_ctx* cctx, const char* key, int64_t* value) {
  if (!cctx || !key || !value) return BLSGPU_ERR_ARGS;
  blsgpu_ctx* ctx = const_cast<blsgpu_ctx*>(cctx);
  const std::string k(key);
  if (k == "slots") {
    std::lock_guard<std::mutex> sk(ctx->slots_mu);
    if (ctx->slots_started && !ctx->devs.empty()) {
      std::lock_guard<std::mutex> lk(ctx->devs[0]->q_mu);
      *value = (int64_t)ctx->devs[0]->slots.size();
    } else {
      *value = ctx->slots_per_device;
    }
    return BLSGPU_OK;
  }
  if (k == "hw_queues") {
    *value = ctx->hw_queues;
    return BLSGPU_OK;
  }
  if (k == "blocking_sync" || k == "pipeline_prio") {
    std::lock_guard<std::mutex> sk(ctx->slots_mu);
    *value = k == "blocking_sync" ? ctx->blocking_sync : ctx->pipeline_prio;
    return BLSGPU_OK;
  }
  if (k == "urgent_cus" || k == "urgent_isolate") {
    std::lock_guard<std::mutex> sk(ctx->slots_mu);
    if (k == "urgent_cus")
      *value = ctx->slots_started && !ctx->devs.empty() ? ctx->devs[0]->urgent_cus : ctx->urgent_cus;
    else
      *value = ctx->urgent_isolate;
    return BLSGPU_OK;
  }
  if (k == "abi_version") {
    *value = BLSGPU_ABI_VERSION;
    return BLSGPU_OK;
  }
  if (k == "spurious_groups") {
    uint64_t c = 0;
    for (const Device* d : ctx->devs) c += d->spurious_groups.load(std::memory_order_relaxed);
    *value = (int64_t)c;
    return BLSGPU_OK;
  }
  std::lock_guard<std::mutex> lk(ctx->opt_mu);
  const Options& o = ctx->opt;
// ... 230 lines not shown
```

lodestar_amd/csrc/runtime_internal.hpp:

```cpp
#pragma once
#include <hip/hip_runtime.h>
#include <stdint.h>
#include <stdlib.h>
#include <string.h>

#include <algorithm>
#include <atomic>
#include <chrono>
#include <condition_variable>
#include <deque>
#include <mutex>
#include <shared_mutex>
#include <thread>
#include <vector>

#include "../../include/blsgpu.h"
#include "batch_rand.hpp"
#include "kernels.h"

namespace blsgpu_rt __attribute__((visibility("hidden"))) {

struct HipError {
  hipError_t e;
};
#define HIPCHK(x)                             \
  do {                                        \
    hipError_t _e = (x);                      \
    if (_e != hipSuccess) throw HipError{_e}; \
  } while (0)

inline thread_local uint64_t tl_async_grow = 0;
inline bool poison_buffers() {
  static const bool on = [] {
    const char* v = getenv("BLSGPU_POISON");
    return v && v[0] == '1';
  }();
  return on;
}
inline bool sync_grow() {
  static const bool on = [] {
    const char* v = getenv("BLSGPU_SYNC_GROW");
    return v && v[0] == '1';
  }();
  return on;
}
inline std::mutex g_grow_mu;
inline bool grow_unlocked() {
  static const bool on = [] {
    const char* v = getenv("BLSGPU_GROW_UNLOCKED");
    return v && v[0] == '1';
  }();
  return on;
}
inline bool fb_verify() {
  static const bool on = [] {
    const char* v = getenv("BLSGPU_FB_VERIFY");
    return v && v[0] == '1';
  }();
  return on;
}
inline bool grow_free() {
  static const bool on = [] {
    const char* v = getenv("BLSGPU_GROW_FREE");
    return v && v[0] == '1';
  }();
  return on;
}
template <class T>
struct DevBuf {
  T* p = nullptr;
  size_t cap = 0;
  hipStream_t st = nullptr;
  std::vector<T*> retired;
  void ensure(size_t n) {
    if (n <= cap) return;
    std::unique_lock<std::mutex> lk(g_grow_mu, std::defer_lock);
    if (!grow_unlocked()) lk.lock();
    const size_t c = std::max<size_t>(n, cap * 2);
    if (st && sync_grow()) {
      HIPCHK(hipDeviceSynchronize());
      if (p) HIPCHK(hipFree(p));
      p = nullptr;
      HIPCHK(hipMalloc((void**)&p, c * sizeof(T)));
      if (poison_buffers()) HIPCHK(hipMemset(p, 0xA5, c * sizeof(T)));
      HIPCHK(hipDeviceSynchronize());
      tl_async_grow++;
    } else if (st) {
      if (p && grow_free()) HIPCHK(hipFreeAsync(p, st));
      else if (p) retired.push_back(p);
      p = nullptr;
      HIPCHK(hipMallocAsync((void**)&p, c * sizeof(T), st));
      if (poison_buffers()) HIPCHK(hipMemsetAsync(p, 0xA5, c * sizeof(T), st));
      tl_async_grow++;
    } else {
      if (p) HIPCHK(hipFree(p));
      p = nullptr;
      HIPCHK(hipMalloc((void**)&p, c * sizeof(T)));
      if (poison_buffers()) {
        HIPCHK(hipMemset(p, 0xA5, c * sizeof(T)));
        HIPCHK(hipStreamSynchronize(nullptr));
      }
    }
    cap = c;
  }
  void release() {
    std::unique_lock<std::mutex> lk(g_grow_mu, std::defer_lock);
    if (!grow_unlocked()) lk.lock();
    if (p) (void)(st ? hipFreeAsync(p, st) : hipFree(p));
    for (T* q : retired) (void)(st ? hipFreeAsync(q, st) : hipFree(q));
    retired.clear();
    p = nullptr;
    cap = 0;
  }
};

template <class T>
struct HostBuf {
  T* p = nullptr;
  size_t cap = 0;
  void ensure(size_t n) {
    if (n <= cap) return;
    std::unique_lock<std::mutex> lk(g_grow_mu, std::defer_lock);
    if (!grow_unlocked()) lk.lock();
    if (p) HIPCHK(hipHostFree(p));
    p = nullptr;
    size_t c = std::max<size_t>(n, cap * 2);
    HIPCHK(hipHostMalloc((void**)&p, c * sizeof(T), hipHostMallocDefault));
    if (poison_buffers()) memset(p, 0x5A, c * sizeof(T));
    cap = c;
  }
  void release() {
    if (p) (void)hipHostFree(p);
    p = nullptr;
    cap = 0;
  }
};

constexpr int kStages = 8;
constexpr size_t kMillerLineWords = (size_t)MILLER_STEPS * W_LINE;

inline size_t al256(size_t x) { return (x + 255) & ~(size_t)255; }

struct Slot {
  hipEvent_t join_in = nullptr, join_msg = nullptr, join_pk = nullptr, join_mask = nullptr, join_gsm = nullptr,
             join_dec = nullptr, join_msm = nullptr, join_rsig = nullptr, done = nullptr;
  hipEvent_t ev[2 * (kStages + 2)] = {};
  DevBuf<uint8_t> d_in, d_res, d_bytes, d_ok, d_fbflags;
  DevBuf<uint32_t> d_work, d_lines, d_S, d_F, d_G, d_list, d_msmB, d_msmW, d_fb;
  DevBuf<uint32_t> d_fkeep;
  HostBuf<uint8_t> h_in, h_res, h_ok;
  HostBuf<uint32_t> h_list;
  hipStream_t fb = nullptr;
  bool retire = false;
  bool in_flight = false;
  bool alone = false;
  bool urgent = false;

  void set_stream(hipStream_t st) {
    for (auto* b : {&d_in, &d_res, &d_bytes, &d_ok, &d_fbflags}) b->st = st;
    for (auto* b : {&d_work, &d_lines, &d_S, &d_F, &d_G, &d_list, &d_msmB, &d_msmW, &d_fb, &d_fkeep}) b->st = st;
  }
  void release_all() {
    d_in.release(); d_res.release(); d_bytes.release(); d_ok.release(); d_fbflags.release();
    d_work.release(); d_lines.release(); d_S.release(); d_F.release(); d_list.release();
    d_msmB.release(); d_msmW.release(); d_fb.release(); d_G.release(); d_fkeep.release();
    h_in.release(); h_res.release(); h_ok.release(); h_list.release();
  }
};

struct Call;
struct Task {
  Call* call;
  uint32_t shard;
};

enum { kSig = 0, kMsg = 1, kPk = 2, kTail = 3, kStreams = 4, kMaxPairs = 3 };
#ifndef BLSGPU_STREAM_PRIO
#define BLSGPU_STREAM_PRIO ((1 << kMsg) | (1 << kTail))
#endif
#ifndef BLSGPU_STREAM_PAIRS
#define BLSGPU_STREAM_PAIRS 1
#endif


struct Device {
  int id = 0;
  hipStream_t table_stream = nullptr;
  hipStream_t st[2 * kMaxPairs] = {};
  int npairs = 2;
  std::mutex enq_mu;
  std::mutex helper_mu;
  Slot helper;
  hipStream_t same_st[2] = {};
  hipEvent_t same_ev[3] = {};
  std::shared_mutex table_mu;
  DevBuf<uint32_t> table;
  uint32_t table_n = 0;
  std::mutex q_mu;
  std::condition_variable q_cv;
  std::deque<Task> queue;
  bool stop = false;
  std::vector<Slot*> slots;
  std::vector<std::thread> workers;
  int runs_inflight = 0;
  std::atomic<uint32_t> run_seq{0};
  std::atomic<int64_t> load{0};
  hipStream_t ust[4] = {};
  std::vector<uint32_t> umask;
  int uprio = 0;
  std::deque<Task> uqueue;
  Slot* uslot = nullptr;
  std::thread uworker;
  std::atomic<int> upending{0};
  std::atomic<uint64_t> spurious_groups{0};
  int urgent_cus = 0;
  std::vector<uint32_t> main_mask;
  bool blocking_sync = true;
  std::mutex fail_mu;
  double fail_rate = 0;
};

struct Options {
  int64_t group_sets = 1024;
  int64_t max_devices = 64;
  bool profile = false;
  bool dedupe = true;
  int64_t miller_k = 0;
  int64_t merge_sets = 131072;
  int64_t merge_wait_us = 2000;
  int64_t idle_wait_us = 0;
  int64_t pipeline_depth = 3;
  int64_t group_policy = 0;
  bool serial = false;
  int64_t miller_lanes = 0;
  int64_t f_run_max = 16;
  int64_t lane_tail_min = 0;
  int64_t lane_tail_parts = 3;
  int64_t msm_slice_mid = 32;
  int64_t lines_lanes = 2;
  int64_t merge_balance = 0;
  int64_t early_release = 0;
  int64_t tail_on_msg = 0;
  int64_t copy_stream = 0;
  int64_t msm_tree = 1;
  int64_t coop_max = 512;
  int64_t coop_g2_max = 4096;
  int64_t coop_excl_max = 512;
  int64_t rsig_spec = 1;
  int64_t spec_large = 1;
  int64_t spec_gsm = 0;
  int64_t fb_lane_min = 256;
  int64_t route_split_sets = 16384;
  int64_t acc6_max = 16384;
  int64_t miller_pairs = 0;
  int64_t small_max = 4096;
  int64_t fb_direct_min = 1024;
  int64_t fb_check6 = 2;
  int64_t keep_f = 1;
  int64_t keep_copy = 0;
  int64_t fb_force_busy = 0;
  int64_t urgent_lane = 1;
  int64_t urgent_max_sets = 512;
  int64_t urgent_excl = 0;
  int64_t urgent_wait_us = 300;
  int64_t group_adapt = 1;
  bool same_run(const struct Options& o) const {
    return group_sets == o.group_sets && profile == o.profile && dedupe == o.dedupe && miller_k == o.miller_k &&
           group_policy == o.group_policy && serial == o.serial && miller_lanes == o.miller_lanes &&
           f_run_max == o.f_run_max && lane_tail_min == o.lane_tail_min &&
           lane_tail_parts == o.lane_tail_parts &&
           msm_slice_mid == o.msm_slice_mid && msm_tree == o.msm_tree &&
           lines_lanes == o.lines_lanes && merge_balance == o.merge_balance && early_release == o.early_release && tail_on_msg == o.tail_on_msg && copy_stream == o.copy_stream && coop_max == o.coop_max &&
           coop_g2_max == o.coop_g2_max && coop_excl_max == o.coop_excl_max && rsig_spec == o.rsig_spec && spec_large == o.spec_large && spec_gsm == o.spec_gsm &&
           fb_lane_min == o.fb_lane_min && acc6_max == o.acc6_max && miller_pairs == o.miller_pairs && small_max == o.small_max &&
           fb_direct_min == o.fb_direct_min && fb_check6 == o.fb_check6 && fb_force_busy == o.fb_force_busy &&
           group_adapt == o.group_adapt && keep_f == o.keep_f && keep_copy == o.keep_copy;
  }
};

struct MsgIndex {
  std::vector<uint32_t> slot;
  uint64_t key;
  explicit MsgIndex(uint32_t n, uint64_t k) : key(k) {
    size_t cap = 16;
    while (cap < (size_t)n * 2) cap <<= 1;
    slot.assign(cap, 0);
  }
  static uint64_t mix(uint64_t z) {
    z = (z ^ (z >> 30)) * 0xBF58476D1CE4E5B9ull;
    z = (z ^ (z >> 27)) * 0x94D049BB133111EBull;
    return z ^ (z >> 31);
  }
  size_t hash(const uint8_t* msgs, uint32_t i) const {
    uint64_t w[4];
    memcpy(w, msgs + (size_t)i * 32, 32);
    return (size_t)(mix(w[0] ^ key) ^ mix(w[1] + key) ^ w[2] ^ (w[3] << 1)) & (slot.size() - 1);
  }
  uint32_t find_or_add(const uint8_t* msgs, uint32_t i, std::vector<uint32_t>& uniq) {
    return find_or_add_h(msgs, i, hash(msgs, i), uniq);
  }
  uint32_t find_or_add_h(const uint8_t* msgs, uint32_t i, size_t h, std::vector<uint32_t>& uniq) {
    const size_t mask = slot.size() - 1;
    for (;;) {
      const uint32_t s = slot[h];
      if (!s) {
        uniq.push_back(i);
        slot[h] = (uint32_t)uniq.size();
        return (uint32_t)uniq.size() - 1;
      }
      if (memcmp(msgs + (size_t)uniq[s - 1] * 32, msgs + (size_t)i * 32, 32) == 0) return s - 1;
      h = (h + 1) & mask;
    }
  }
};

inline double ms_since(std::chrono::steady_clock::time_point t) {
  return std::chrono::duration<double, std::milli>(std::chrono::steady_clock::now() - t).count();
}

bool resolve_key(uint64_t seed, batch_rand::Key& key, uint64_t& hash_key);

}

struct blsgpu_ctx {
  std::vector<blsgpu_rt::Device*> devs;
  std::atomic<bool> closed{false};
  std::mutex active_mu;
  std::condition_variable active_cv;
  int active = 0;
  std::mutex table_mu;
  std::mutex opt_mu;
  blsgpu_rt::Options opt;
  int64_t slots_per_device = 2;
  int64_t hw_queues = 4;
  std::mutex slots_mu;
  bool slots_started = false;
  std::atomic<uint32_t> route_seq{0};
  int64_t urgent_cus = 0;
  int64_t urgent_isolate = 1;
  int64_t blocking_sync = 1;
  int64_t pipeline_prio = 1;
};

namespace blsgpu_rt __attribute__((visibility("hidden"))) {
inline bool enter(blsgpu_ctx* ctx) {
  std::lock_guard<std::mutex> lk(ctx->active_mu);
  if (ctx->closed) return false;
  ctx->active++;
  return true;
}
inline void leave(blsgpu_ctx* ctx) {
  {
    std::lock_guard<std::mutex> lk(ctx->active_mu);
    ctx->active--;
  }
  ctx->active_cv.notify_all();
}
}
```

Before: 3.916 million sets/s.

## Split Miller loop into step segments across lanes and fold partial results

Adds optional segmentation of the Miller accumulation loop. Each chunk's 68 steps are split into up to 8 segments run as separate grid rows, and the partial fp12 values are then combined with squarings and multiplies in a new fold kernel. A planner picks a larger chunk size k with several segments for big runs, so that items are batched into fewer, longer chunks while enough lanes stay busy. The cost is extra fold work, extra fp12 storage, and redundant bit-walking per segment.

Measured after the change: 4.275 million sets/s, median of 6. 1.09x the previous value.

```diff
diff --git a/lodestar_amd/build.py b/lodestar_amd/build.py
--- a/lodestar_amd/build.py
+++ b/lodestar_amd/build.py
@@ -58,7 +58,8 @@
 def _tu_deps(src):
     if src.endswith(".cpp"):
         return [os.path.join(CSRC, f) for f in (src, "kernels.h", "batch_rand.hpp", "runtime_internal.hpp",
-                                                "helper_layout.hpp")] + [os.path.join(ROOT, "include", "blsgpu.h")]
+                                                "helper_layout.hpp", "miller_plan.hpp")] + [
+            os.path.join(ROOT, "include", "blsgpu.h")]
     return [os.path.join(CSRC, src)] + _headers()
 
 
diff --git a/lodestar_amd/csrc/k_group.hip b/lodestar_amd/csrc/k_group.hip
--- a/lodestar_amd/csrc/k_group.hip
+++ b/lodestar_amd/csrc/k_group.hip
@@ -64,6 +64,13 @@
   if (q >= ng * W_FP12) return;
   const uint32_t g = q % ng, w = q / ng, a = f_ranges[2 * g], e = f_ranges[2 * g + 1];
   F_out[q] = a < e ? b.f_chunk[(size_t)w * b.n + a] : (w < BLS_NL ? FP_ONE.l[w] : 0u);
+}
+
+STAGE_KERNEL_W(BLSGPU_WPE_GRP) void k_f_fold(const uint32_t* H, uint32_t ng, MillerSegs sg, uint32_t* F_out) {
+  const uint32_t g = blockIdx.x * WAVE + threadIdx.x;
+  if (g >= ng) return;
+  const uint32_t stride = sg.n * ng;
+  st_fp12(F_out, ng, g, miller_seg_fold(sg.n, sg.dbl, [&](uint32_t j) { return ld_fp12(H, stride, j * ng + g); }));
 }
 
 __device__ __forceinline__ void gtw_load_S(GtwLds& sh, const uint32_t* S_in, uint32_t ng, uint32_t g, uint32_t t) {
@@ -276,13 +283,19 @@
 }
 void launch_group_tree(const PipelineBuffers& b, const uint32_t* f_ranges, uint32_t ng, const uint32_t* runs,
                        uint32_t n_runs, const uint32_t* pairs, const std::vector<uint32_t>& level_end, uint32_t* F,
-                       hipStream_t s) {
+                       hipStream_t s, const MillerSegs* segs, uint32_t* H) {
   if (!ng) return;
   if (n_runs) hipLaunchKernelGGL(k_f_runs, grid_for(n_runs), dim3(WAVE), 0, s, b, runs, n_runs);
   uint32_t p0 = 0;
   for (const uint32_t p1 : level_end) {
     if (p1 > p0) hipLaunchKernelGGL(k_f_pairs, dim3(p1 - p0), dim3(GTW_LANES), 0, s, b, pairs + 2 * (size_t)p0);
     p0 = p1;
+  }
+  if (segs && segs->n > 1) {
+    const uint32_t nh = segs->n * ng;
+    hipLaunchKernelGGL(k_f_gather, grid_for(nh * W_FP12), dim3(WAVE), 0, s, b, f_ranges, nh, H);
+    hipLaunchKernelGGL(k_f_fold, grid_for(ng), dim3(WAVE), 0, s, H, ng, *segs, F);
+    return;
   }
   hipLaunchKernelGGL(k_f_gather, grid_for(ng * W_FP12), dim3(WAVE), 0, s, b, f_ranges, ng, F);
 }
diff --git a/lodestar_amd/csrc/k_miller.hip b/lodestar_amd/csrc/k_miller.hip
--- a/lodestar_amd/csrc/k_miller.hip
+++ b/lodestar_amd/csrc/k_miller.hip
@@ -96,25 +96,38 @@
   }
 }
 
-template <bool UNITS>
-STAGE_KERNEL_W(BLSGPU_WPE_ACC) void k_miller_acc(PipelineBuffers b) {
+template <bool UNITS, bool SEG>
+STAGE_KERNEL_W(BLSGPU_WPE_ACC) void k_miller_acc(PipelineBuffers b, MillerSegs sg) {
   const uint32_t c = blockIdx.x * WAVE + threadIdx.x;
   if (c >= b.n_chunks) return;
   const uint32_t k0 = b.chunk_first[c], k1 = b.chunk_first[c + 1];
+  int s0 = 0, s1 = MILLER_STEPS, bit = 62;
+  bool add_next = false;
+  if (SEG) {
+    s0 = (int)sg.first[blockIdx.y];
+    s1 = (int)sg.first[blockIdx.y + 1];
+#pragma unroll 1
+    for (int s = 0; s < s0; s++) {
+      if (!add_next) {
+        add_next = (BLS_Z_ABS >> bit) & 1ull;
+        bit--;
+      } else {
+        add_next = false;
+      }
+    }
+  }
 #if ACC_PREFETCH
   __shared__ uint32_t pre[W_LINE * WAVE];
   auto msg_of = [&](uint32_t k) {
     const uint32_t i = b.chunk_items[k];
     return UNITS ? b.unit_msg[i] : b.msg_idx[i];
   };
-  if (k1 > k0) line_prefetch(pre, b.lines, b.nm, msg_of(k0));
+  if (k1 > k0) line_prefetch(pre, b.lines + (size_t)s0 * W_LINE * b.nm, b.nm, msg_of(k0));
 #endif
   fp12 f = fp12_one();
-  int bit = 62;
-  bool add_next = false;
-#pragma unroll 1
-  for (int s = 0; s < MILLER_STEPS; s++) {
-    if (!add_next && s != 0) f = fp12_sqr(f);
+#pragma unroll 1
+  for (int s = s0; s < s1; s++) {
+    if (!add_next && s != s0) f = fp12_sqr(f);
     const uint32_t* o = b.lines + (size_t)s * W_LINE * b.nm;
 #if BLS_LINE_PAIRS
     bool pend = false;
@@ -141,7 +154,7 @@
       line_read_done();
       if (k + 1 < k1)
         line_prefetch(pre, o, b.nm, msg_of(k + 1));
-      else if (s + 1 < MILLER_STEPS)
+      else if (s + 1 < s1)
         line_prefetch(pre, o + (size_t)W_LINE * b.nm, b.nm, msg_of(k0));
       if (!active || (b.mflags[m] & MF_H_INF)) continue;
       const g1a P = ld_g1a(UNITS ? b.unit_p : b.pk_aff, b.n, i);
@@ -178,7 +191,7 @@
       add_next = false;
     }
   }
-  st_fp12(b.f_chunk, b.n, c, fp12_conj(f));
+  st_fp12(b.f_chunk, b.n, SEG ? blockIdx.y * b.n_chunks + c : c, fp12_conj(f));
 }
 
 template <bool UNITS>
@@ -492,10 +505,19 @@
   else
     hipLaunchKernelGGL(k_miller_accx<false>, grid_for(2 * b.n_chunks), dim3(WAVE), 0, s, b);
 }
-void launch_miller_acc(const PipelineBuffers& b, bool units, hipStream_t s) {
+void launch_miller_acc(const PipelineBuffers& b, bool units, hipStream_t s, const MillerSegs* segs) {
   if (!b.n_chunks) return;
+  if (segs && segs->n > 1) {
+    const dim3 grid(grid_for(b.n_chunks).x, segs->n);
+    if (units)
+      hipLaunchKernelGGL((k_miller_acc<true, true>), grid, dim3(WAVE), 0, s, b, *segs);
+    else
+      hipLaunchKernelGGL((k_miller_acc<false, true>), grid, dim3(WAVE), 0, s, b, *segs);
+    return;
+  }
+  const MillerSegs one{};
   if (units)
-    hipLaunchKernelGGL(k_miller_acc<true>, grid_for(b.n_chunks), dim3(WAVE), 0, s, b);
+    hipLaunchKernelGGL((k_miller_acc<true, false>), grid_for(b.n_chunks), dim3(WAVE), 0, s, b, one);
   else
-    hipLaunchKernelGGL(k_miller_acc<false>, grid_for(b.n_chunks), dim3(WAVE), 0, s, b);
-}
+    hipLaunchKernelGGL((k_miller_acc<false, false>), grid_for(b.n_chunks), dim3(WAVE), 0, s, b, one);
+}
diff --git a/lodestar_amd/csrc/kernels.h b/lodestar_amd/csrc/kernels.h
--- a/lodestar_amd/csrc/kernels.h
+++ b/lodestar_amd/csrc/kernels.h
@@ -92,7 +92,13 @@
 void launch_miller_lines(const PipelineBuffers& b, hipStream_t s);
 void launch_miller_lines2(const PipelineBuffers& b, hipStream_t s);
 void launch_miller_accx(const PipelineBuffers& b, bool units, hipStream_t s);
-void launch_miller_acc(const PipelineBuffers& b, bool units, hipStream_t s);
+#define MILLER_MAX_SEGS 8
+struct MillerSegs {
+  uint32_t n;
+  uint32_t first[MILLER_MAX_SEGS + 1];
+  uint32_t dbl[MILLER_MAX_SEGS];
+};
+void launch_miller_acc(const PipelineBuffers& b, bool units, hipStream_t s, const MillerSegs* segs = nullptr);
 void launch_miller_acc2(const PipelineBuffers& b, bool units, hipStream_t s);
 void launch_miller_acc6(const PipelineBuffers& b, bool units, hipStream_t s);
 #ifndef BLSGPU_EXCLUSIVE_SMALL
@@ -103,7 +109,7 @@
                          hipStream_t s);
 void launch_group_tree(const PipelineBuffers& b, const uint32_t* f_ranges, uint32_t n_groups, const uint32_t* runs,
                        uint32_t n_runs, const uint32_t* pairs, const std::vector<uint32_t>& level_end, uint32_t* F,
-                       hipStream_t s);
+                       hipStream_t s, const MillerSegs* segs = nullptr, uint32_t* H = nullptr);
 void launch_group_check(const uint32_t* S, const uint32_t* F, uint32_t n_groups, uint8_t* ok, hipStream_t s,
                         const uint32_t* sel = nullptr, uint32_t n_sel = 0, const uint32_t* G = nullptr,
                         bool exclusive = false, bool lane = false);
diff --git a/lodestar_amd/csrc/miller_plan.hpp b/lodestar_amd/csrc/miller_plan.hpp
--- /dev/null
+++ b/lodestar_amd/csrc/miller_plan.hpp
@@ -0,0 +1,111 @@
+#pragma once
+#include <stdint.h>
+#include <algorithm>
+#include <utility>
+#include <vector>
+
+namespace miller_plan {
+
+constexpr uint32_t kSteps = 68;
+constexpr uint32_t kDoublings = 63;
+constexpr uint64_t kZAbs = 0xd201000000010000ull;
+constexpr uint32_t kMaxSegments = 8;
+constexpr uint32_t kFillLanes = 65536;
+
+inline bool is_doubling_step(uint32_t s) {
+  int bit = 62;
+  bool add_next = false, dbl = true;
+  for (uint32_t t = 0; t <= s; t++) {
+    dbl = !add_next;
+    if (!add_next) {
+      add_next = (kZAbs >> bit) & 1ull;
+      bit--;
+    } else {
+      add_next = false;
+    }
+  }
+  return dbl;
+}
+
+struct Segments {
+  uint32_t n;
+  uint32_t first[kMaxSegments + 1];
+  uint32_t dbl[kMaxSegments];
+};
+inline Segments segments(uint32_t J) {
+  Segments sg{};
+  sg.n = std::min(std::max(J, 1u), kMaxSegments);
+  for (uint32_t j = 0; j <= sg.n; j++) {
+    uint32_t s = (kSteps * j + sg.n / 2) / sg.n;
+    if (s < kSteps && !is_doubling_step(s)) s--;
+    sg.first[j] = s;
+  }
+  for (uint32_t j = 0; j < sg.n; j++) {
+    sg.dbl[j] = 0;
+    for (uint32_t s = sg.first[j]; s < sg.first[j + 1]; s++) sg.dbl[j] += is_doubling_step(s) ? 1 : 0;
+  }
+  return sg;
+}
+
+inline uint32_t group_chunks(uint32_t len, uint32_t k) { return (len + k - 1) / k; }
+inline uint64_t count_chunks(const uint32_t* group_len, size_t n_groups, uint32_t k) {
+  uint64_t c = 0;
+  for (size_t g = 0; g < n_groups; g++) c += group_chunks(group_len[g], k);
+  return c;
+}
+
+inline uint32_t fit_segments(uint64_t n_chunks, uint32_t want, uint64_t capacity) {
+  uint32_t J = std::min(std::max(want, 1u), kMaxSegments);
+  while (J > 1 && n_chunks * J > capacity) J--;
+  return J;
+}
+
+struct Plan {
+  uint32_t k, segs;
+};
+inline bool pair_allowed(uint64_t n_items, uint64_t n_chunks, uint32_t k, uint32_t J, uint64_t capacity) {
+  return J >= 1 && J <= k && J <= kMaxSegments && n_chunks * J <= capacity && 2 * n_items >= n_chunks * k;
+}
+inline Plan plan_auto(uint32_t n_items, const uint32_t* group_len, size_t n_groups, uint64_t capacity, bool explicit_k,
+                      uint32_t k_today) {
+  if (explicit_k || n_items < kFillLanes) return {k_today, 1};
+  for (uint32_t k : {8u, 4u}) {
+    const uint64_t nc = count_chunks(group_len, n_groups, k);
+    for (uint32_t J = 1; J <= k && J <= kMaxSegments; J++)
+      if (nc * J >= kFillLanes) {
+        if (pair_allowed(n_items, nc, k, J, capacity)) return {k, J};
+        break;
+      }
+  }
+  return {k_today, 1};
+}
+
+inline bool hold_kept_values(double fail_rate, double sets_per_group) {
+  if (!(fail_rate > 0)) return false;
+  double ok = 1.0;
+  double b = fail_rate >= 1 ? 0.0 : 1.0 - fail_rate;
+  for (uint64_t e = sets_per_group < 1 ? 1 : (uint64_t)sets_per_group; e; e >>= 1, b *= b)
+    if (e & 1) ok *= b;
+  return 1.0 - ok >= 0.2;
+}
+
+inline std::pair<uint32_t, uint32_t> add_chunks(std::vector<uint32_t>& first, std::vector<uint32_t>& items, uint32_t a,
+                                                uint32_t e, uint32_t k, bool interleave = false,
+                                                const uint32_t* map = nullptr) {
+  const uint32_t c0 = (uint32_t)first.size() - 1;
+  if (interleave) {
+    const uint32_t nc = group_chunks(e - a, k);
+    for (uint32_t c = 0; c < nc; c++) {
+      for (uint32_t y = a + c; y < e; y += nc) items.push_back(map ? map[y] : y);
+      first.push_back((uint32_t)items.size());
+    }
+  } else {
+    for (uint32_t x = a; x < e; x += k) {
+      for (uint32_t y = x; y < std::min(e, x + k); y++) items.push_back(map ? map[y] : y);
+      first.push_back((uint32_t)items.size());
+    }
+  }
+  return {c0, (uint32_t)first.size() - 1};
+}
+
+}
diff --git a/lodestar_amd/csrc/pairing.hpp b/lodestar_amd/csrc/pairing.hpp
--- a/lodestar_amd/csrc/pairing.hpp
+++ b/lodestar_amd/csrc/pairing.hpp
@@ -140,6 +140,18 @@
 BLS_FN fp12 miller_acc_step(const fp12& f, int s, bool is_add, const line3& L, const fp& xP, const fp& yP) {
   fp12 g = (!is_add && s != 0) ? fp12_sqr(f) : f;
   return fp12_mul_by_014(g, L.l0, fp2_mul_fp(L.c1, xP), fp2_mul_fp(L.c4, yP));
+}
+
+template <class Ld>
+BLS_FN fp12 miller_seg_fold(uint32_t n_segs, const uint32_t* dbl, Ld ld) {
+  fp12 R = ld(0u);
+#pragma unroll 1
+  for (uint32_t j = 1; j < n_segs; j++) {
+#pragma unroll 1
+    for (uint32_t t = 0; t < dbl[j]; t++) R = fp12_sqr(R);
+    R = fp12_mul(R, ld(j));
+  }
+  return R;
 }
 
 BLS_HDNI fp12 miller_loop(const g1a& P, const g2a& Q) {
diff --git a/lodestar_amd/csrc/runtime.cpp b/lodestar_amd/csrc/runtime.cpp
--- a/lodestar_amd/csrc/runtime.cpp
+++ b/lodestar_amd/csrc/runtime.cpp
@@ -7,6 +7,7 @@
 #include <system_error>
 
 #include "runtime_internal.hpp"
+#include "miller_plan.hpp"
 
 using namespace blsgpu_rt;
 
@@ -31,32 +32,24 @@
   return k;
 }
 
+enum class AccForm { six, pairs, two, one };
+inline AccForm acc_form(uint32_t mk, uint32_t n_chunks, int64_t lanes_opt, int64_t acc6_max, bool pairs) {
+  if (lanes_opt == 6 || (lanes_opt == 0 && mk == 1 && (int64_t)n_chunks <= acc6_max)) return AccForm::six;
+  if (lanes_opt == 3 || (lanes_opt == 0 && pairs)) return AccForm::pairs;
+  return lanes_opt == 2 || (lanes_opt == 0 && mk == 1) ? AccForm::two : AccForm::one;
+}
 void launch_miller_acc_auto(const PipelineBuffers& pb, bool units, hipStream_t st, uint32_t mk, int64_t lanes_opt,
-                            int64_t acc6_max, bool pairs) {
-  if (lanes_opt == 6 || (lanes_opt == 0 && mk == 1 && (int64_t)pb.n_chunks <= acc6_max)) {
-    launch_miller_acc6(pb, units, st);
-    return;
-  }
-  if (lanes_opt == 3 || (lanes_opt == 0 && pairs)) {
-    launch_miller_accx(pb, units, st);
-    return;
-  }
-  const bool two = lanes_opt == 2 || (lanes_opt == 0 && mk == 1);
-  if (two)
-    launch_miller_acc2(pb, units, st);
-  else
-    launch_miller_acc(pb, units, st);
-}
-
-inline std::pair<uint32_t, uint32_t> add_chunks(std::vector<uint32_t>& first, std::vector<uint32_t>& items,
-                                                uint32_t a, uint32_t e, uint32_t k, const uint32_t* map = nullptr) {
-  const uint32_t c0 = (uint32_t)first.size() - 1;
-  for (uint32_t x = a; x < e; x += k) {
-    for (uint32_t y = x; y < std::min(e, x + k); y++) items.push_back(map ? map[y] : y);
-    first.push_back((uint32_t)items.size());
-  }
-  return {c0, (uint32_t)first.size() - 1};
-}
+                            int64_t acc6_max, bool pairs, const MillerSegs* segs = nullptr) {
+  switch (acc_form(mk, pb.n_chunks, lanes_opt, acc6_max, pairs)) {
+    case AccForm::six: launch_miller_acc6(pb, units, st); break;
+    case AccForm::pairs: launch_miller_accx(pb, units, st); break;
+    case AccForm::two: launch_miller_acc2(pb, units, st); break;
+    case AccForm::one: launch_miller_acc(pb, units, st, segs); break;
+  }
+}
+
+using miller_plan::add_chunks;
+static_assert(miller_plan::kSteps == MILLER_STEPS && miller_plan::kMaxSegments == MILLER_MAX_SEGS, "miller_plan.hpp");
 
 inline void add_slices(std::vector<uint32_t>& slices, std::vector<uint32_t>& range_slices, uint32_t a, uint32_t e,
                        uint32_t len = MSM_SLICE) {
@@ -315,17 +308,47 @@
   const bool coop = n_items <= (uint32_t)opt.coop_max && opt.miller_k <= 1;
   const bool coop_g2 = n <= (uint32_t)opt.coop_g2_max;
   const bool excl = BLSGPU_EXCLUSIVE_SMALL && n_items <= (uint32_t)opt.coop_excl_max && (!sl.urgent || opt.urgent_excl);
-  const uint32_t mk = coop ? 1u : opt.miller_k > 0 ? (uint32_t)opt.miller_k : miller_k_auto(n_items);
+  const uint32_t mk_whole = coop ? 1u : opt.miller_k > 0 ? (uint32_t)opt.miller_k : miller_k_auto(n_items);
+  auto group_items = [&](uint32_t g) -> std::pair<uint32_t, uint32_t> {
+    if (merged) return {g_unit_first[g], g_unit_first[g + 1]};
+    return {job_sets(group_jobs[g].first).first, job_sets(group_jobs[g].second - 1).second};
+  };
+  const AccForm form_whole = acc_form(mk_whole, n_items, opt.miller_lanes, opt.acc6_max, opt.miller_pairs != 0);
+  uint32_t mk = mk_whole, segs = 1;
+  bool seg_plan = false;
+  if (opt.miller_segments > 0) {
+    if (!coop && form_whole == AccForm::one) segs = (uint32_t)std::min<int64_t>(opt.miller_segments, mk);
+  } else if (!coop && opt.miller_lanes == 0 && (form_whole == AccForm::one || form_whole == AccForm::two)) {
+    std::vector<uint32_t> g_len(ng0);
+    for (uint32_t g = 0; g < ng0; g++) g_len[g] = group_items(g).second - group_items(g).first;
+    bool hold = false;
+    if (opt.keep_f && !merged && mk_whole == 1 && ng0) {
+      std::lock_guard<std::mutex> lk(d.fail_mu);
+      hold = miller_plan::hold_kept_values(d.fail_rate, (double)n / ng0);
+    }
+    const miller_plan::Plan pl =
+        miller_plan::plan_auto(n_items, g_len.data(), ng0, stride, opt.miller_k > 0 || hold, mk_whole);
+    seg_plan = pl.k != mk_whole || pl.segs > 1;
+    mk = pl.k, segs = pl.segs;
+  }
+  const bool interleave = segs > 1 || seg_plan;
   std::vector<uint32_t> chunk_first{0}, chunk_items, g_chunks(2 * (size_t)ng0);
   chunk_items.reserve(n);
   for (uint32_t g = 0; g < ng0; g++) {
-    const uint32_t a = merged ? g_unit_first[g] : job_sets(group_jobs[g].first).first;
-    const uint32_t e = merged ? g_unit_first[g + 1] : job_sets(group_jobs[g].second - 1).second;
-    const auto cr = add_chunks(chunk_first, chunk_items, a, e, mk);
+    const auto ae = group_items(g);
+    const auto cr = add_chunks(chunk_first, chunk_items, ae.first, ae.second, mk, interleave);
     g_chunks[2 * g] = cr.first;
     g_chunks[2 * g + 1] = cr.second;
   }
   const uint32_t n_chunks = (uint32_t)chunk_first.size() - 1;
+  segs = miller_plan::fit_segments(n_chunks, segs, stride);
+  MillerSegs msegs{};
+  {
+    const miller_plan::Segments sg = miller_plan::segments(segs);
+    msegs.n = sg.n;
+    for (uint32_t j = 0; j <= sg.n; j++) msegs.first[j] = sg.first[j];
+    for (uint32_t j = 0; j < sg.n; j++) msegs.dbl[j] = sg.dbl[j];
+  }
   const bool keep_f = opt.keep_f && !merged && mk == 1 && n_chunks == n;
   const bool small = n <= (uint32_t)opt.small_max;
   const bool spec = BLSGPU_STREAM_PAIRS && (small || opt.spec_large) && sl.alone && !opt.serial;
@@ -346,22 +369,29 @@
   }
   std::vector<uint32_t> ftree, f_level_end;
   uint32_t f_k = 1, f_max = 0;
-  if (n_chunks > 16384)
+  const uint32_t n_slots = n_chunks * segs, n_franges = ng0 * segs;
+  std::vector<uint32_t> f_rng(2 * (size_t)n_franges);
+  for (uint32_t j = 0; j < segs; j++)
+    for (uint32_t g = 0; g < ng0; g++) {
+      f_rng[2 * ((size_t)j * ng0 + g)] = j * n_chunks + g_chunks[2 * g];
+      f_rng[2 * ((size_t)j * ng0 + g) + 1] = j * n_chunks + g_chunks[2 * g + 1];
+    }
+  if (n_slots > 16384)
     for (const uint32_t heads = opt.f_run_max > 16 ? 256u : 8192u;
-         n_chunks / f_k > heads && f_k < (uint32_t)opt.f_run_max;)
+         n_slots / f_k > heads && f_k < (uint32_t)opt.f_run_max;)
       f_k *= 2;
   for (uint32_t g = 0; g < ng0; g++) f_max = std::max(f_max, g_chunks[2 * g + 1] - g_chunks[2 * g]);
   if (f_k > 1)
-    for (uint32_t g = 0; g < ng0; g++)
-      for (uint32_t x = g_chunks[2 * g], e = g_chunks[2 * g + 1]; x < e; x += f_k)
+    for (uint32_t r = 0; r < n_franges; r++)
+      for (uint32_t x = f_rng[2 * r], e = f_rng[2 * r + 1]; x < e; x += f_k)
         if (std::min(e, x + f_k) - x > 1) {
           ftree.push_back(x);
           ftree.push_back(std::min(e, x + f_k));
         }
   const uint32_t n_fruns = (uint32_t)(ftree.size() / 2);
   for (uint32_t st = f_k; st < f_max; st *= 2) {
-    for (uint32_t g = 0; g < ng0; g++)
-      for (uint32_t i = g_chunks[2 * g], e = g_chunks[2 * g + 1]; i + st < e; i += 2 * st) {
+    for (uint32_t r = 0; r < n_franges; r++)
+      for (uint32_t i = f_rng[2 * r], e = f_rng[2 * r + 1]; i + st < e; i += 2 * st) {
         ftree.push_back(i);
         ftree.push_back(i + st);
       }
@@ -383,7 +413,7 @@
                o_siglen = al256(o_sigs + (size_t)n * sig_w), o_umsg = al256(o_siglen + (size_t)n * 4),
                o_midx = al256(o_umsg + (size_t)n_umsg * 32), o_ranges = al256(o_midx + (size_t)n * 4),
                o_franges = al256(o_ranges + (size_t)std::max(ng0, 1u) * 8),
-               o_ufirst = al256(o_franges + (size_t)std::max(ng0, 1u) * 8),
+               o_ufirst = al256(o_franges + (size_t)std::max(n_franges, 1u) * 8),
                o_usets = al256(o_ufirst + (size_t)(n_units + 1) * 4), o_umsgi = al256(o_usets + (size_t)unit_sets.size() * 4),
                o_cfirst = al256(o_umsgi + (size_t)n_units * 4), o_citems = al256(o_cfirst + (size_t)(n_chunks + 1) * 4),
                o_agg = al256(o_citems + chunk_items.size() * 4), o_slices = al256(o_agg + agg_sets.size() * 4),
@@ -430,9 +460,8 @@
   for (uint32_t g = 0; g < ng0; g++) {
     hranges[2 * g] = job_sets(group_jobs[g].first).first;
     hranges[2 * g + 1] = job_sets(group_jobs[g].second - 1).second;
-    hfranges[2 * g] = g_chunks[2 * g];
-    hfranges[2 * g + 1] = g_chunks[2 * g + 1];
-  }
+  }
+  memcpy(hfranges, f_rng.data(), f_rng.size() * 4);
   memcpy(hin + o_cfirst, chunk_first.data(), chunk_first.size() * 4);
   memcpy(hin + o_citems, chunk_items.data(), chunk_items.size() * 4);
   if (!agg_sets.empty()) memcpy(hin + o_agg, agg_sets.data(), agg_sets.size() * 4);
@@ -472,6 +501,7 @@
   sl.d_work.ensure((size_t)stride * per_set + (size_t)nm * (W_G2A + W_G2J + W_FP + 14 * W_FP + 2 * W_G2J));
   sl.d_lines.ensure((size_t)nm * kMillerLineWords);
   if (keep_f) sl.d_fkeep.ensure((size_t)stride * W_FP12);
+  if (segs > 1) sl.d_fseg.ensure((size_t)W_FP12 * n_franges);
   if (rsig_spec) sl.d_fb.ensure((size_t)stride * 9 * W_G2J);
   uint8_t* const din = sl.d_in.p;
   uint8_t* const d_ok0 = sl.d_res.p + o_ok;
@@ -549,8 +579,9 @@
     if (host_trace())
       fprintf(stderr,
               "[blsgpu host] run %u sets: merge %.2f ms, prep %.2f ms (dedupe %.2f, structure %.2f), pick-to-copy %.2f "
-              "ms, %zu B in\n",
-              n, tl_merge_ms, ms_since(t_prep0), t_dedupe_ms, t_struct_ms, ms_since(tl_run_t0), in_bytes);
+              "ms, %zu B in, %u Miller chunks of %u x %u segments\n",
+              n, tl_merge_ms, ms_since(t_prep0), t_dedupe_ms, t_struct_ms, ms_since(tl_run_t0), in_bytes, n_chunks, mk,
+              segs);
     const bool own_copy = opt.copy_stream && !opt.serial && !sl.urgent && tl_async_grow == grow0;
     hipStream_t sc = own_copy ? d.table_stream : s;
     HIPCHK(hipMemcpyAsync(din, hin, in_bytes, hipMemcpyHostToDevice, sc));
@@ -612,8 +643,10 @@
     if (merged) launch_unit_aggregate(pb, sm);
     if (coop)
       launch_miller_coop(pb, merged, sm, excl);
+    else if (seg_plan)
+      launch_miller_acc(pb, merged, sm, &msegs);
     else
-      launch_miller_acc_auto(pb, merged, sm, mk, opt.miller_lanes, opt.acc6_max, opt.miller_pairs != 0);
+      launch_miller_acc_auto(pb, merged, sm, mk, opt.miller_lanes, opt.acc6_max, opt.miller_pairs != 0, &msegs);
     end(5, sm);
     if (keep_f && opt.keep_copy == 1)
       launch_copy_words(sl.d_fkeep.p, pb.f_chunk, (size_t)stride * W_FP12, sm);
@@ -622,7 +655,8 @@
     const uint32_t* d_franges = reinterpret_cast<uint32_t*>(din + o_franges);
     beg(6, sm);
     const uint32_t* d_ftree = reinterpret_cast<uint32_t*>(din + o_ftree);
-    launch_group_tree(pb, d_franges, ng0, d_ftree, n_fruns, d_ftree + 2 * (size_t)n_fruns, f_level_end, sl.d_F.p, sm);
+    launch_group_tree(pb, d_franges, ng0, d_ftree, n_fruns, d_ftree + 2 * (size_t)n_fruns, f_level_end, sl.d_F.p, sm,
+                      &msegs, sl.d_fseg.p);
     end(6, sm);
     HIPCHK(hipEventRecord(sl.join_msg, sm));
     if (spec)
@@ -749,7 +783,7 @@
         rf[2 * q + 1] = js.second;
         continue;
       }
-      const auto cr = add_chunks(rfirst, ritems, js.first, js.second, mk);
+      const auto cr = add_chunks(rfirst, ritems, js.first, js.second, mk_whole);
       rf[2 * q] = cr.first;
       rf[2 * q + 1] = cr.second;
     }
@@ -814,7 +848,7 @@
       if (coop)
         launch_miller_coop(pr, false, sfb);
       else
-        launch_miller_acc_auto(pr, false, sfb, mk, opt.miller_lanes, opt.acc6_max, opt.miller_pairs != 0);
+        launch_miller_acc_auto(pr, false, sfb, mk_whole, opt.miller_lanes, opt.acc6_max, opt.miller_pairs != 0);
     }
     st.fallback_jobs += nr;
     if (small_jobs) {
@@ -1801,6 +1835,10 @@
   blsgpu_ctx* ctx = new blsgpu_ctx();
   ctx->hw_queues = hw_queues_of_process();
   ctx->slots_per_device = default_slots(ctx->hw_queues);
+  if (const char* v = getenv("BLSGPU_MILLER_SEGMENTS")) {
+    const long j = strtol(v, nullptr, 10);
+    if (j >= 1 && j <= MILLER_MAX_SEGS) ctx->opt.miller_segments = j;
+  }
   try {
     for (int id : ids) {
       Device* d = new Device();
diff --git a/lodestar_amd/csrc/runtime_internal.hpp b/lodestar_amd/csrc/runtime_internal.hpp
--- a/lodestar_amd/csrc/runtime_internal.hpp
+++ b/lodestar_amd/csrc/runtime_internal.hpp
@@ -148,6 +148,7 @@
   DevBuf<uint8_t> d_in, d_res, d_bytes, d_ok, d_fbflags;
   DevBuf<uint32_t> d_work, d_lines, d_S, d_F, d_G, d_list, d_msmB, d_msmW, d_fb;
   DevBuf<uint32_t> d_fkeep;
+  DevBuf<uint32_t> d_fseg;
   HostBuf<uint8_t> h_in, h_res, h_ok;
   HostBuf<uint32_t> h_list;
   hipStream_t fb = nullptr;
@@ -158,12 +159,12 @@
 
   void set_stream(hipStream_t st) {
     for (auto* b : {&d_in, &d_res, &d_bytes, &d_ok, &d_fbflags}) b->st = st;
-    for (auto* b : {&d_work, &d_lines, &d_S, &d_F, &d_G, &d_list, &d_msmB, &d_msmW, &d_fb, &d_fkeep}) b->st = st;
+    for (auto* b : {&d_work, &d_lines, &d_S, &d_F, &d_G, &d_list, &d_msmB, &d_msmW, &d_fb, &d_fkeep, &d_fseg}) b->st = st;
   }
   void release_all() {
     d_in.release(); d_res.release(); d_bytes.release(); d_ok.release(); d_fbflags.release();
     d_work.release(); d_lines.release(); d_S.release(); d_F.release(); d_list.release();
-    d_msmB.release(); d_msmW.release(); d_fb.release(); d_G.release(); d_fkeep.release();
+    d_msmB.release(); d_msmW.release(); d_fb.release(); d_G.release(); d_fkeep.release(); d_fseg.release();
     h_in.release(); h_res.release(); h_ok.release(); h_list.release();
   }
 };
@@ -232,6 +233,7 @@
   int64_t pipeline_depth = 3;
   int64_t group_policy = 0;
   bool serial = false;
+  int64_t miller_segments = 0;
   int64_t miller_lanes = 0;
   int64_t f_run_max = 16;
   int64_t lane_tail_min = 0;
@@ -266,7 +268,7 @@
   int64_t group_adapt = 1;
   bool same_run(const struct Options& o) const {
     return group_sets == o.group_sets && profile == o.profile && dedupe == o.dedupe && miller_k == o.miller_k &&
-           group_policy == o.group_policy && serial == o.serial && miller_lanes == o.miller_lanes &&
+           group_policy == o.group_policy && serial == o.serial && miller_lanes == o.miller_lanes && miller_segments == o.miller_segments &&
            f_run_max == o.f_run_max && lane_tail_min == o.lane_tail_min &&
            lane_tail_parts == o.lane_tail_parts &&
            msm_slice_mid == o.msm_slice_mid && msm_tree == o.msm_tree &&
```
